# fgcallari/skeres

Hardware: AMD Instinct MI355X
Metric: LM iterations/sec (higher is better)
Workload: dtype f64

## Files before the change

### skeres_amd/csrc/bal_kernels.hip

```cpp
#include <hip/hip_runtime.h>

#include <algorithm>

#include "functors.hpp"
#include "bal_kernels.hpp"

namespace sk {

static constexpr int kBlock = 256;

__device__ __forceinline__ double wave_sum(double v) {
#pragma unroll
  for (int off = 32; off > 0; off >>= 1) v += __shfl_xor(v, off, 64);
  return v;
}

__device__ __forceinline__ int bal_part(const BalDev& d, int i) { return i >= d.cam_b ? 2 : ((i >= d.seg_lo && i < d.cam_a) ? 0 : 1); }
__device__ __forceinline__ int bal_pos(const BalDev& d, int i, int part) { return 9 * (i - (part == 0 ? d.seg_lo : (part == 1 ? d.cam_a : d.cam_b))); }
__device__ __forceinline__ double* bal_block(const BalDev& d, int i, int j, int* ld) {
  const int pj = bal_part(d, j), pi = bal_part(d, i);
  const BalDev::Front& f = d.front[pj];
  const int row = pi == pj ? bal_pos(d, i, pi) : f.border_row[i - d.cam_b];
  *ld = f.ld;
  return f.S + (size_t)row * f.ld + bal_pos(d, j, pj);
// ... 218 lines not shown
    acc[1] += m0 * (d.r[o] + m0 / 2.0) + m1 * (d.r[(size_t)d.N + o] + m1 / 2.0);
  }
  block_sum<2>(acc, d.partial, d.partial_stride);
}

template <bool kLoss>
__global__ __launch_bounds__(kBlock) void bal_host_jac_kernel(BalDev d, int partial_off) {
  double acc[1] = {0.0};
  for (int h = blockIdx.x * kBlock + threadIdx.x; h < d.num_host; h += gridDim.x * kBlock) {
    const int o = d.host_obs[h];
    const int ci = d.cam[o], pi = d.pt[o];
    const double* row = d.host_rows + (size_t)h * kHostRow;
    const double r0 = row[0], r1 = row[1];
    double j0[12], j1[12];
#pragma unroll
    for (int k = 0; k < 9; ++k) { j0[k] = row[2 + k]; j1[k] = row[11 + k]; }
#pragma unroll
    for (int k = 0; k < 3; ++k) { j0[9 + k] = row[20 + k]; j1[9 + k] = row[23 + k]; }
    if (kLoss) {
      const double sq = r0 * r0 + r1 * r1;
      double rho[3];
      bal_loss_eval(d, o, sq, rho);
      const LossCorrector lc(sq, rho);
      acc[0] += rho[0];
#pragma unroll
      for (int k = 0; k < 12; ++k) {
        const double a = j0[k], b = j1[k];
        const double rtj = lc.alpha_sq_norm * (r0 * a + r1 * b);
        j0[k] = lc.sqrt_rho1 * (a - r0 * rtj);
        j1[k] = lc.sqrt_rho1 * (b - r1 * rtj);
      }
      d.r[o] = r0 * lc.residual_scaling;
      d.r[(size_t)d.N + o] = r1 * lc.residual_scaling;
    } else {
      d.r[o] = r0;
      d.r[(size_t)d.N + o] = r1;
      acc[0] += r0 * r0 + r1 * r1;
    }
#pragma unroll
    for (int k = 0; k < 9; ++k) {
      const double s = d.scale_c[9 * (size_t)ci + k];
      d.F[(size_t)k * d.N + o] = j0[k] * s;
      d.F[(size_t)(9 + k) * d.N + o] = j1[k] * s;
    }
#pragma unroll
    for (int k = 0; k < 3; ++k) {
      const double s = d.scale_p[3 * (size_t)pi + k];
      d.E[(size_t)k * d.N + o] = j0[9 + k] * s;
      d.E[(size_t)(3 + k) * d.N + o] = j1[9 + k] * s;
    }
  }
  block_sum<1>(acc, d.partial + partial_off, d.partial_stride);
}

template <bool kLoss>
__global__ __launch_bounds__(kBlock) void bal_host_cost_kernel(BalDev d, int partial_off) {
  double acc[2] = {0.0, 0.0};
  for (int h = blockIdx.x * kBlock + threadIdx.x; h < d.num_host; h += gridDim.x * kBlock) {
    const int o = d.host_obs[h];
    const int ci = d.cam[o], pi = d.pt[o];
    const double n0 = d.host_rows[(size_t)h * kHostRow], n1 = d.host_rows[(size_t)h * kHostRow + 1];
    if (kLoss) {
      double rho[3];
      bal_loss_eval(d, o, n0 * n0 + n1 * n1, rho);
      acc[0] += rho[0];
    } else {
      acc[0] += n0 * n0 + n1 * n1;
    }
    double m0 = -d.u[3 * (size_t)d.N + o], m1 = -d.u[4 * (size_t)d.N + o];
#pragma unroll
    for (int k = 0; k < 3; ++k) {
      const double s = d.step_p[3 * (size_t)pi + k];
      m0 += d.E[(size_t)k * d.N + o] * s;
      m1 += d.E[(size_t)(3 + k) * d.N + o] * s;
    }
    acc[1] += m0 * (d.r[o] + m0 / 2.0) + m1 * (d.r[(size_t)d.N + o] + m1 / 2.0);
  }
  block_sum<2>(acc, d.partial + partial_off, d.partial_stride);
}

__global__ __launch_bounds__(kBlock) void bal_scale_jac_kernel(BalDev d) {
  for (int o = blockIdx.x * kBlock + threadIdx.x; o < d.N; o += gridDim.x * kBlock) {
    const int ci = d.cam[o], pi = d.pt[o];
#pragma unroll
    for (int k = 0; k < 9; ++k) {
      const double s = d.scale_c[9 * (size_t)ci + k];
      d.F[(size_t)k * d.N + o] *= s;
      d.F[(size_t)(9 + k) * d.N + o] *= s;
    }
#pragma unroll
    for (int k = 0; k < 3; ++k) {
      const double s = d.scale_p[3 * (size_t)pi + k];
      d.E[(size_t)k * d.N + o] *= s;
      d.E[(size_t)(3 + k) * d.N + o] *= s;
    }
  }
}

__global__ __launch_bounds__(kBlock) void bal_cam_records_kernel(BalDev d) {
  __shared__ __attribute__((aligned(16))) double stage[kBlock / 64][64 * kFcam];
  const int lane = threadIdx.x & 63, w = threadIdx.x >> 6;
  double* st = stage[w];
  const size_t N = d.N;
  for (long o0 = ((long)blockIdx.x * (kBlock / 64) + w) * 64; o0 < d.N; o0 += (long)gridDim.x * kBlock) {
    const long o = o0 + lane;
    const int my_slot = o < d.N ? d.obs_slot[o] : 0;
    if (o < d.N) {
#pragma unroll
      for (int k = 0; k < 18; ++k) st[lane * kFcam + k] = d.F[(size_t)k * N + o];
      st[lane * kFcam + 18] = d.r[o];
      st[lane * kFcam + 19] = d.r[N + o];
    }
    __builtin_amdgcn_wave_barrier();
    __builtin_amdgcn_s_waitcnt(0xC07F);
    __builtin_amdgcn_wave_barrier();
    const int nrec = (int)((d.N - o0) < 64 ? (d.N - o0) : 64);
#pragma unroll
    for (int i = 0; i < kFcam / 2; ++i) {
      const int e2 = i * 64 + lane, rr = e2 / (kFcam / 2), f2 = e2 - rr * (kFcam / 2);
      const int slot = __shfl(my_slot, rr, 64);
      if (rr < nrec) reinterpret_cast<double2*>(d.Fcam + (size_t)slot * kFcam)[f2] = reinterpret_cast<const double2*>(st)[e2];
    }
    __builtin_amdgcn_wave_barrier();
  }
}

__device__ __forceinline__ void bal_cam_reduce_body(const BalDev& d, int block) {
  const int wave = (block * kBlock + threadIdx.x) >> 6, lane = threadIdx.x & 63;
  if (wave >= d.C) return;
  double sq[9], g[9];
#pragma unroll
  for (int k = 0; k < 9; ++k) { sq[k] = 0.0; g[k] = 0.0; }
  for (int e = d.cam_start[wave] + lane; e < d.cam_start[wave + 1]; e += 64) {
    const double2* rec = reinterpret_cast<const double2*>(d.Fcam + (size_t)e * kFcam);
    double v[kFcam];
#pragma unroll
    for (int k = 0; k < kFcam / 2; ++k) { const double2 t = rec[k]; v[2 * k] = t.x; v[2 * k + 1] = t.y; }
    const double r0 = v[18], r1 = v[19];
#pragma unroll
    for (int k = 0; k < 9; ++k) {
      const double f0 = v[k], f1 = v[9 + k];
      sq[k] += f0 * f0 + f1 * f1;
      g[k] += f0 * r0 + f1 * r1;
    }
  }
#pragma unroll
  for (int k = 0; k < 9; ++k) { sq[k] = wave_sum(sq[k]); g[k] = wave_sum(g[k]); }
  if (lane == 0) {
#pragma unroll
    for (int k = 0; k < 9; ++k) { d.colsq_c[9 * (size_t)wave + k] = sq[k]; d.gs_c[9 * (size_t)wave + k] = g[k]; }
  }
}

__device__ __forceinline__ void bal_pt_reduce_body(const BalDev& d, int block) {
  const int gid = block * kBlock + threadIdx.x, sub = gid % kPointLanes;
  const int p = gid / kPointLanes;
  if (p >= d.P) return;
  double sq[3] = {0, 0, 0}, g[3] = {0, 0, 0};
  for (int o = d.pt_start[p] + sub; o < d.pt_start[p + 1]; o += kPointLanes) {
    const double r0 = d.r[o], r1 = d.r[(size_t)d.N + o];
#pragma unroll
    for (int k = 0; k < 3; ++k) {
      const double e0 = d.E[(size_t)k * d.N + o], e1 = d.E[(size_t)(3 + k) * d.N + o];
      sq[k] += e0 * e0 + e1 * e1;
      g[k] += e0 * r0 + e1 * r1;
    }
  }
#pragma unroll
  for (int k = 0; k < 3; ++k) { sq[k] = point_lanes_sum(sq[k]); g[k] = point_lanes_sum(g[k]); }
  if (sub == 0) {
#pragma unroll
    for (int k = 0; k < 3; ++k) { d.colsq_p[3 * (size_t)p + k] = sq[k]; d.gs_p[3 * (size_t)p + k] = g[k]; }
  }
}

__global__ __launch_bounds__(kBlock) void bal_reduce_kernel(BalDev d, int cam_blocks) {
  if ((int)blockIdx.x < cam_blocks) bal_cam_reduce_body(d, (int)blockIdx.x);
  else bal_pt_reduce_body(d, (int)blockIdx.x - cam_blocks);
}

__global__ void jacobi_scale_kernel(const double* colsq, double* scale, int n) {
  const int j = blockIdx.x * blockDim.x + threadIdx.x;
  if (j < n) scale[j] = scale[j] == 0.0 ? 0.0 : 1.0 / (1.0 + sqrt(colsq[j]));
}
__global__ void apply_scale_to_reductions_kernel(double* colsq, double* gs, const double* scale, int n) {
  const int j = blockIdx.x * blockDim.x + threadIdx.x;
  if (j < n) { const double s = scale[j]; colsq[j] = colsq[j] * s * s; gs[j] = gs[j] * s; }
}
__global__ void lm_diagonal_kernel(const double* colsq, double* D, int n, double lo, double hi, double radius) {
  const int j = blockIdx.x * blockDim.x + threadIdx.x;
  if (j < n) D[j] = sqrt(fmin(fmax(colsq[j], lo), hi) / radius);
}
__global__ __launch_bounds__(kBlock) void grad_max_xnorm_kernel(const double* gs, const double* scale, const double* x,
                                                                int n, double* partial, int stride) {
  double m = 0.0, s = 0.0;
  for (int j = blockIdx.x * kBlock + threadIdx.x; j < n; j += gridDim.x * kBlock) {
    if (scale[j] != 0.0) m = fmax(m, fabs(gs[j] / scale[j]));
    s += x[j] * x[j];
  }
  __shared__ double shm[kBlock / 64], shs[kBlock / 64];
#pragma unroll
  for (int off = 32; off > 0; off >>= 1) { m = fmax(m, __shfl_xor(m, off, 64)); s += __shfl_xor(s, off, 64); }
  if ((threadIdx.x & 63) == 0) { shm[threadIdx.x >> 6] = m; shs[threadIdx.x >> 6] = s; }
  __syncthreads();
  if (threadIdx.x == 0) {
    for (int i = 1; i < kBlock / 64; ++i) { m = fmax(m, shm[i]); s += shs[i]; }
    partial[blockIdx.x] = m;
    partial[stride + blockIdx.x] = s;
  }
}

__global__ __launch_bounds__(kBlock) void final_reduce_kernel(const double* partial, int stride, int count, int K, int maxmask, double* out) {
  __shared__ double sh[kBlock];
  const int k = blockIdx.x;
  const bool is_max = ((maxmask >> k) & 1) != 0;
  double a = 0.0;
  for (int i = threadIdx.x; i < count; i += kBlock) {
    const double v = partial[(size_t)k * stride + i];
    a = is_max ? fmax(a, v) : a + v;
  }
  sh[threadIdx.x] = a;
  __syncthreads();
  for (int w = kBlock / 2; w > 0; w >>= 1) {
    if ((int)threadIdx.x < w) sh[threadIdx.x] = is_max ? fmax(sh[threadIdx.x], sh[threadIdx.x + w]) : sh[threadIdx.x] + sh[threadIdx.x + w];
    __syncthreads();
  }
  if (threadIdx.x == 0) out[k] = sh[0];
}

__global__ __launch_bounds__(kBlock) void bal_point_block_kernel(BalDev d) {
  const int gid = blockIdx.x * kBlock + threadIdx.x, sub = gid % kPointLanes;
  const int p = gid / kPointLanes;
  if (p >= d.P) return;
  double t00 = 0, t10 = 0, t11 = 0, t20 = 0, t21 = 0, t22 = 0;
  for (int o = d.pt_start[p] + sub; o < d.pt_start[p + 1]; o += kPointLanes) {
    const double a0 = d.E[o], a1 = d.E[(size_t)d.N + o], a2 = d.E[2 * (size_t)d.N + o];
    const double b0 = d.E[3 * (size_t)d.N + o], b1 = d.E[4 * (size_t)d.N + o], b2 = d.E[5 * (size_t)d.N + o];
    t00 += a0 * a0 + b0 * b0; t10 += a1 * a0 + b1 * b0; t11 += a1 * a1 + b1 * b1;
    t20 += a2 * a0 + b2 * b0; t21 += a2 * a1 + b2 * b1; t22 += a2 * a2 + b2 * b2;
  }
  t00 = point_lanes_sum(t00); t10 = point_lanes_sum(t10); t11 = point_lanes_sum(t11);
  t20 = point_lanes_sum(t20); t21 = point_lanes_sum(t21); t22 = point_lanes_sum(t22);
  if (sub != 0) return;
  const double d0 = bal_lm_diag(d, d.colsq_p[3 * (size_t)p]), d1 = bal_lm_diag(d, d.colsq_p[3 * (size_t)p + 1]), d2 = bal_lm_diag(d, d.colsq_p[3 * (size_t)p + 2]);
  t00 += d0 * d0; t11 += d1 * d1; t22 += d2 * d2;
  const double l00 = sqrt(t00);
  const double l10 = t10 / l00, l20 = t20 / l00;
  const double l11 = sqrt(t11 - l10 * l10);
  const double l21 = (t21 - l20 * l10) / l11;
  const double l22 = sqrt(t22 - l20 * l20 - l21 * l21);
  const double m00 = 1.0 / l00, m11 = 1.0 / l11, m22 = 1.0 / l22;
  const double m10 = -(l10 * m00) / l11;
  const double m21 = -(l21 * m11) / l22;
  const double m20 = -(l20 * m00 + l21 * m10) / l22;
  const size_t P = d.P;
  d.M[p] = m00; d.M[P + p] = m10; d.M[2 * P + p] = m11; d.M[3 * P + p] = m20; d.M[4 * P + p] = m21; d.M[5 * P + p] = m22;
  const double g0 = d.gs_p[3 * (size_t)p], g1 = d.gs_p[3 * (size_t)p + 1], g2 = d.gs_p[3 * (size_t)p + 2];
  const double u0 = m00 * g0, u1 = m10 * g0 + m11 * g1, u2 = m20 * g0 + m21 * g1 + m22 * g2;
  d.q[p] = m00 * u0 + m10 * u1 + m20 * u2;
  d.q[P + p] = m11 * u1 + m21 * u2;
  d.q[2 * P + p] = m22 * u2;
  if (!(l00 > 0.0) || !(l11 > 0.0) || !(l22 > 0.0)) *d.fail_flag = 1;
}

__global__ __launch_bounds__(kBlock) void bal_kept_points_kernel(BalDev d, int obs_blocks) {
  const size_t N = d.N, P = d.P;
  if ((int)blockIdx.x < obs_blocks) {
    const int e = blockIdx.x * kBlock + threadIdx.x;
    if (e >= d.num_kept_obs) return;
    const int o = d.kept_obs[e], k = d.kept_obs_slot[e];
    const int ic = d.kept_cam[k] / 3, t3 = 3 * (d.kept_cam[k] % 3);
    const int c = d.cam[o];
    const bool below = ic > c;
    if (!d.front[bal_part(d, below ? c : ic)].S) return;
    double ea[3], eb[3];
#pragma unroll
    for (int a = 0; a < 3; ++a) { ea[a] = d.E[(size_t)a * N + o]; eb[a] = d.E[(size_t)(3 + a) * N + o]; }
    int ld;
    double* blk = below ? bal_block(d, ic, c, &ld) : bal_block(d, c, ic, &ld);
#pragma unroll
    for (int b = 0; b < 9; ++b) {
      const double f0 = d.F[(size_t)b * N + o], f1 = d.F[(size_t)(9 + b) * N + o];
#pragma unroll
      for (int a = 0; a < 3; ++a) {
        const double v = ea[a] * f0 + eb[a] * f1;
        if (below) blk[(size_t)(t3 + a) * ld + b] = v; else blk[(size_t)b * ld + t3 + a] = v;
      }
    }
    return;
  }
  const int k = (((int)blockIdx.x - obs_blocks) * kBlock + threadIdx.x) >> 6, lane = threadIdx.x & 63;
  if (k >= d.num_kept) return;
  const int p = d.kept_pt[k], ic = d.kept_cam[k] / 3, t3 = 3 * (d.kept_cam[k] % 3);
  double t00 = 0, t10 = 0, t11 = 0, t20 = 0, t21 = 0, t22 = 0;
  for (int o = d.pt_start[p] + lane; o < d.pt_start[p + 1]; o += 64) {
    const double a0 = d.E[o], a1 = d.E[N + o], a2 = d.E[2 * N + o];
    const double b0 = d.E[3 * N + o], b1 = d.E[4 * N + o], b2 = d.E[5 * N + o];
    t00 += a0 * a0 + b0 * b0; t10 += a1 * a0 + b1 * b0; t11 += a1 * a1 + b1 * b1;
    t20 += a2 * a0 + b2 * b0; t21 += a2 * a1 + b2 * b1; t22 += a2 * a2 + b2 * b2;
  }
  t00 = wave_sum(t00); t10 = wave_sum(t10); t11 = wave_sum(t11); t20 = wave_sum(t20); t21 = wave_sum(t21); t22 = wave_sum(t22);
  if (lane != 0) return;
  d.M[p] = 0.0; d.M[P + p] = 0.0; d.M[2 * P + p] = 0.0; d.M[3 * P + p] = 0.0; d.M[4 * P + p] = 0.0; d.M[5 * P + p] = 0.0;
  d.q[p] = 0.0; d.q[P + p] = 0.0; d.q[2 * P + p] = 0.0;
  if (!d.front[bal_part(d, ic)].S) return;
  const bool home = !d.kept_home || d.kept_home[k] != 0;
  const double d0 = home ? bal_lm_diag(d, d.colsq_p[3 * (size_t)p]) : 0.0, d1 = home ? bal_lm_diag(d, d.colsq_p[3 * (size_t)p + 1]) : 0.0,
               d2 = home ? bal_lm_diag(d, d.colsq_p[3 * (size_t)p + 2]) : 0.0;
  int ld;
  double* blk = bal_block(d, ic, ic, &ld) + (size_t)t3 * ld + t3;
  blk[0] = t00 + d0 * d0;
  blk[ld] = t10; blk[ld + 1] = t11 + d1 * d1;
  blk[2 * (size_t)ld] = t20; blk[2 * (size_t)ld + 1] = t21; blk[2 * (size_t)ld + 2] = t22 + d2 * d2;
  double* rhs = bal_rhs(d, ic) + t3;
  rhs[0] = home ? d.gs_p[3 * (size_t)p] : 0.0; rhs[1] = home ? d.gs_p[3 * (size_t)p + 1] : 0.0; rhs[2] = home ? d.gs_p[3 * (size_t)p + 2] : 0.0;
}

__global__ __launch_bounds__(kBlock) void bal_kept_sums_kernel(BalDev d, double* buf, int K, int gather) {
  const int t = blockIdx.x * kBlock + threadIdx.x;
  if (t >= 3 * d.num_kept) return;
  const int k = t / 3, a = t - 3 * k;
  const size_t p = (size_t)d.kept_pt[k], g = (size_t)(d.kept_global ? d.kept_global[k] : k);
  if (gather) { buf[3 * g + a] = d.colsq_p[3 * p + a]; buf[3 * (size_t)K + 3 * g + a] = d.gs_p[3 * p + a]; }
  else { d.colsq_p[3 * p + a] = buf[3 * g + a]; d.gs_p[3 * p + a] = buf[3 * (size_t)K + 3 * g + a]; }
}

__global__ __launch_bounds__(kBlock, 4) void bal_obs_precompute_kernel(BalDev d) {
  constexpr int kLs = kWs + 2;
  __shared__ __attribute__((aligned(16))) double stage[kBlock / 64][32 * kLs];
  const size_t N = d.N, P = d.P;
  const int lane = threadIdx.x & 63, wave = threadIdx.x >> 6;
  double* mine = &stage[wave][0];
  for (long base = (long)(blockIdx.x * kBlock + wave * 64); base < (long)d.N; base += (long)gridDim.x * kBlock) {
    const long o = base + lane;
    const int my_slot = o < (long)d.N ? d.obs_slot[o] : 0;
    double w[27], rt[2];
    if (o < (long)d.N) {
      const int p = d.pt[o];
      const double m00 = d.M[p], m10 = d.M[P + p], m11 = d.M[2 * P + p], m20 = d.M[3 * P + p], m21 = d.M[4 * P + p], m22 = d.M[5 * P + p];
      const double q0 = d.q[p], q1 = d.q[P + p], q2 = d.q[2 * P + p];
      double eh[2][3];
#pragma unroll
      for (int r = 0; r < 2; ++r) {
        const double e0 = d.E[(3 * r) * N + o], e1 = d.E[(3 * r + 1) * N + o], e2 = d.E[(3 * r + 2) * N + o];
        eh[r][0] = e0 * m00;
        eh[r][1] = e0 * m10 + e1 * m11;
        eh[r][2] = e0 * m20 + e1 * m21 + e2 * m22;
        rt[r] = d.r[r * N + o] - (e0 * q0 + e1 * q1 + e2 * q2);
      }
#pragma unroll
      for (int c = 0; c < 9; ++c) {
        const double f0 = d.F[c * N + o], f1 = d.F[(9 + c) * N + o];
#pragma unroll
        for (int a = 0; a < 3; ++a) w[3 * c + a] = f0 * eh[0][a] + f1 * eh[1][a];
      }
    }
    const int nrec = (int)(((long)d.N - base) < 64 ? ((long)d.N - base) : 64);
    const int sub = lane >> 4, chunk = lane & 15;
#pragma unroll
    for (int half = 0; half < 2; ++half) {
      if ((lane >> 5) == half && o < (long)d.N) {
        double* rec = mine + (lane & 31) * kLs;
#pragma unroll
        for (int k = 0; k < 27; ++k) rec[k] = w[k];
        rec[27] = rt[0]; rec[28] = rt[1];
        rec[29] = 0.0; rec[30] = 0.0; rec[31] = 0.0;
      }
      __builtin_amdgcn_wave_barrier();
#pragma unroll 4
      for (int it = 0; it < 8; ++it) {
        const int rl = 4 * it + sub, rec = 32 * half + rl;
        const int slot = __shfl(my_slot, rec, 64);
        if (rec < nrec) {
          const double2 v = *reinterpret_cast<const double2*>(&mine[rl * kLs + 2 * chunk]);
          *reinterpret_cast<double2*>(d.What + (size_t)slot * kWs + 2 * chunk) = v;
        }
      }
      __builtin_amdgcn_wave_barrier();
    }
  }
}

__global__ __launch_bounds__(kBlock) void bal_cam_diag_kernel(BalDev d) {
  const int i = (blockIdx.x * kBlock + threadIdx.x) >> 6, lane = threadIdx.x & 63;
  if (i >= d.C) return;
  if (d.pseudo && d.pseudo[i]) return;
  double acc[45], rh[9];
#pragma unroll
  for (int k = 0; k < 45; ++k) acc[k] = 0.0;
#pragma unroll
  for (int k = 0; k < 9; ++k) rh[k] = 0.0;
  for (int e = d.cam_start[i] + lane; e < d.cam_start[i + 1]; e += 64) {
    double f0[9], f1[9], w[28];
    {
      const double2* rec = reinterpret_cast<const double2*>(d.Fcam + (size_t)e * kFcam);
#pragma unroll
      for (int k = 0; k < 9; ++k) {
        const double2 t = rec[k];
        if (2 * k < 9) f0[2 * k] = t.x; else f1[2 * k - 9] = t.x;
        if (2 * k + 1 < 9) f0[2 * k + 1] = t.y; else f1[2 * k + 1 - 9] = t.y;
      }
    }
    const double2* wrec = reinterpret_cast<const double2*>(d.What + (size_t)e * kWs);
#pragma unroll
    for (int k = 0; k < 14; ++k) { const double2 t = wrec[k]; w[2 * k] = t.x; w[2 * k + 1] = t.y; }
    const double r0 = w[27], r1 = wrec[14].x;
    int k = 0;
#pragma unroll
    for (int c = 0; c < 9; ++c) {
      rh[c] += f0[c] * r0 + f1[c] * r1;
#pragma unroll
      for (int e2 = 0; e2 <= c; ++e2, ++k)
        acc[k] += (f0[c] * f0[e2] + f1[c] * f1[e2]) - (w[3 * c] * w[3 * e2] + w[3 * c + 1] * w[3 * e2 + 1] + w[3 * c + 2] * w[3 * e2 + 2]);
    }
  }
#pragma unroll
  for (int k = 0; k < 45; ++k) acc[k] = wave_sum(acc[k]);
#pragma unroll
  for (int k = 0; k < 9; ++k) rh[k] = wave_sum(rh[k]);
  if (lane == 0 && d.front[bal_part(d, i)].S) {
    int k = 0, ld;
    double* blk = bal_block(d, i, i, &ld);
    double* rhs = bal_rhs(d, i);
#pragma unroll
    for (int c = 0; c < 9; ++c) {
      rhs[c] = rh[c];
#pragma unroll
      for (int e2 = 0; e2 <= c; ++e2, ++k) blk[(size_t)c * ld + e2] = acc[k];
    }
  }
}

__global__ __launch_bounds__(64) void bal_dup_diag_kernel(BalDev d) {
  const int first = blockIdx.x;
  const int i = d.dup_cam[first];
  if (first > 0 && d.dup_cam[first - 1] == i) return;
  if (!d.front[bal_part(d, i)].S) return;
  const int t = threadIdx.x;
  if (t >= 45) return;
  int c = 0, rem = t;
  while (rem > c) { rem -= c + 1; ++c; }
  const int e2 = rem;
  double acc = 0.0;
  for (int k = first; k < d.num_dup && d.dup_cam[k] == i; ++k) {
    const double* wa = d.What + (size_t)d.dup_a[k] * kWs;
    const double* wb = d.What + (size_t)d.dup_b[k] * kWs;
    acc += (wa[3 * c] * wb[3 * e2] + wa[3 * c + 1] * wb[3 * e2 + 1] + wa[3 * c + 2] * wb[3 * e2 + 2]) +
           (wb[3 * c] * wa[3 * e2] + wb[3 * c + 1] * wa[3 * e2 + 1] + wb[3 * c + 2] * wa[3 * e2 + 2]);
  }
  int ld;
  double* blk = bal_block(d, i, i, &ld);
  blk[(size_t)c * ld + e2] -= acc;
}

constexpr int kPairSlot = 34;
__device__ __forceinline__ void pair_accumulate(const BalDev& d, int e_begin, int e_end, int stride, int c, double* slot, double (&acc)[9]) {
  if (e_begin >= e_end) return;
  const int last = e_begin + (e_end - 1 - e_begin) / stride * stride;
  const double* wr = d.What + (size_t)d.pair_row_obs[e_begin] * kWs + 3 * c;
  const double* wc = d.What + (size_t)d.pair_col_obs[e_begin] * kWs + 3 * c;
  double y0 = wr[0], y1 = wr[1], y2 = wr[2], v0 = wc[0], v1 = wc[1], v2 = wc[2];
  int e1 = e_begin + stride <= last ? e_begin + stride : last;
  int ob1 = d.pair_row_obs[e1], oa1 = d.pair_col_obs[e1];
  for (int e = e_begin; e < e_end; e += stride) {
    slot[3 * c] = v0; slot[3 * c + 1] = v1; slot[3 * c + 2] = v2;
    __builtin_amdgcn_wave_barrier();
    double w[kWu];
#pragma unroll
    for (int k = 0; k < kWu / 2; ++k) { const double2 t = reinterpret_cast<const double2*>(slot)[k]; w[2 * k] = t.x; w[2 * k + 1] = t.y; }
    __builtin_amdgcn_wave_barrier();
    const double* wrn = d.What + (size_t)ob1 * kWs + 3 * c;
    const double* wcn = d.What + (size_t)oa1 * kWs + 3 * c;
    const double yn0 = wrn[0], yn1 = wrn[1], yn2 = wrn[2], vn0 = wcn[0], vn1 = wcn[1], vn2 = wcn[2];
    const int e2 = e + 2 * stride <= last ? e + 2 * stride : last;
    const int ob2 = d.pair_row_obs[e2], oa2 = d.pair_col_obs[e2];
#pragma unroll
    for (int k = 0; k < 9; ++k) acc[k] += y0 * w[3 * k] + y1 * w[3 * k + 1] + y2 * w[3 * k + 2];
    y0 = yn0; y1 = yn1; y2 = yn2; v0 = vn0; v1 = vn1; v2 = vn2;
    ob1 = ob2; oa1 = oa2;
  }
}

__device__ __forceinline__ int xcd_grouped_block(int w, int group) {
  if (group <= 0) return w;
  const int x = w & 7, q = w >> 3;
  return ((q / group) * 8 + x) * group + q % group;
}

__global__ __launch_bounds__(kBlock) void bal_pair_kernel(BalDev d, int xcd_group) {
  const int lane = threadIdx.x & 63;
  const int wave = (xcd_grouped_block((int)blockIdx.x, xcd_group) * kBlock + threadIdx.x) >> 6;
  __shared__ __attribute__((aligned(16))) double share[kBlock / 64][7][kPairSlot];
  const int sub = lane / 9, c = lane - 9 * sub;
  const int slot = wave * 7 + sub;
  if (sub >= 7 || slot >= d.num_short_segments) return;
  const int seg = d.short_segments[slot];
  double acc[9];
#pragma unroll
  for (int k = 0; k < 9; ++k) acc[k] = 0.0;
  pair_accumulate(d, d.seg_start[seg], d.seg_start[seg + 1], 1, c, share[threadIdx.x >> 6][sub], acc);
  const int i = d.seg_row[seg], j = d.seg_col[seg];
  int ld;
  double* out = bal_block(d, i, j, &ld) + (size_t)c * ld;
#pragma unroll
  for (int k = 0; k < 9; ++k) out[k] = -acc[k];
}

__global__ __launch_bounds__(kBlock) void bal_pair_long_kernel(BalDev d, int xcd_group) {
  __shared__ double red[kBlock / 64][7][81];
  __shared__ __attribute__((aligned(16))) double share[kBlock / 64][7][kPairSlot];
  const int lane = threadIdx.x & 63, w = threadIdx.x >> 6;
  const int slot = (xcd_grouped_block((int)blockIdx.x, xcd_group) * kBlock + threadIdx.x) >> 6;
  if (slot >= d.num_long_segments) return;
  const int seg = d.long_segments[slot];
  const int sub = lane / 9, c = lane - 9 * sub;
  double acc[9];
#pragma unroll
  for (int k = 0; k < 9; ++k) acc[k] = 0.0;
  if (sub < 7) {
    pair_accumulate(d, d.seg_start[seg] + sub, d.seg_start[seg + 1], 7, c, share[w][sub], acc);
#pragma unroll
    for (int k = 0; k < 9; ++k) red[w][sub][9 * c + k] = acc[k];
  }
  __builtin_amdgcn_wave_barrier();
  __builtin_amdgcn_s_waitcnt(0xC07F);
  __builtin_amdgcn_wave_barrier();
  const int i = d.seg_row[seg], j = d.seg_col[seg];
  int ld;
  double* blk = bal_block(d, i, j, &ld);
  for (int e = lane; e < 81; e += 64) {
    double s = 0.0;
#pragma unroll
    for (int g = 0; g < 7; ++g) s += red[w][g][e];
    blk[(size_t)(e / 9) * ld + e % 9] = -s;
  }
}

__global__ void finish_normal_matrix_kernel(double* S, int ld, int n, int npad, int rhs_row, const double* D) {
  const int j = blockIdx.x * blockDim.x + threadIdx.x;
  if (j >= npad) return;
  if (j < n) S[(size_t)j * ld + j] += D[j] * D[j];
  else if (j == rhs_row) S[(size_t)j * ld + j] = 1e300;
  else S[(size_t)j * ld + j] = 1.0;
}
__global__ void bal_finish_S_kernel(BalDev d, int parts) {
  const int j = blockIdx.x * blockDim.x + threadIdx.x;
  if (j >= 9 * d.C) return;
  const int i = j / 9, c = j - 9 * i, part = bal_part(d, i);
  if (!((parts >> part) & 1) || !d.front[part].S) return;
  if (d.pseudo && d.pseudo[i]) return;
  int ld;
  double* blk = bal_block(d, i, i, &ld);
  const double D = bal_lm_diag(d, d.colsq_c[j]);
  blk[(size_t)c * ld + c] += D * D;
}
__global__ void set_diagonal_kernel(double* S, int ld, int from, int to, double value) {
  const int j = from + blockIdx.x * blockDim.x + threadIdx.x;
  if (j < to) S[(size_t)j * ld + j] = value;
}

__global__ __launch_bounds__(kBlock) void bal_obs_backsub_kernel(BalDev d) {
  const size_t N = d.N;
  for (int o = blockIdx.x * kBlock + threadIdx.x; o < d.N; o += gridDim.x * kBlock) {
    const double* yc = d.y_c + 9 * (size_t)d.cam[o];
    double f0 = 0.0, f1 = 0.0;
#pragma unroll
    for (int c = 0; c < 9; ++c) { f0 += d.F[c * N + o] * yc[c]; f1 += d.F[(9 + c) * N + o] * yc[c]; }
    d.u[o] = d.E[o] * f0 + d.E[3 * N + o] * f1;
    d.u[N + o] = d.E[N + o] * f0 + d.E[4 * N + o] * f1;
    d.u[2 * N + o] = d.E[2 * N + o] * f0 + d.E[5 * N + o] * f1;
    d.u[3 * N + o] = f0;
    d.u[4 * N + o] = f1;
  }
}

__global__ __launch_bounds__(kBlock) void bal_point_backsub_kernel(BalDev d) {
  const int gid = blockIdx.x * kBlock + threadIdx.x, sub = gid % kPointLanes;
  const int p = gid / kPointLanes;
  double acc[1] = {0.0};
  double w0 = 0.0, w1 = 0.0, w2 = 0.0;
  if (p < d.P) {
    for (int o = d.pt_start[p] + sub; o < d.pt_start[p + 1]; o += kPointLanes) {
      w0 += d.u[o];
      w1 += d.u[(size_t)d.N + o];
      w2 += d.u[2 * (size_t)d.N + o];
    }
  }
  w0 = point_lanes_sum(w0); w1 = point_lanes_sum(w1); w2 = point_lanes_sum(w2);
  if (p < d.P && sub == 0) {
    const size_t P = d.P;
    const double t0 = d.gs_p[3 * (size_t)p] - w0, t1 = d.gs_p[3 * (size_t)p + 1] - w1, t2 = d.gs_p[3 * (size_t)p + 2] - w2;
    const double m00 = d.M[p], m10 = d.M[P + p], m11 = d.M[2 * P + p], m20 = d.M[3 * P + p], m21 = d.M[4 * P + p], m22 = d.M[5 * P + p];
    const double u0 = m00 * t0, u1 = m10 * t0 + m11 * t1, u2 = m20 * t0 + m21 * t1 + m22 * t2;
    const double y[3] = {m00 * u0 + m10 * u1 + m20 * u2, m11 * u1 + m21 * u2, m22 * u2};
#pragma unroll
    for (int k = 0; k < 3; ++k) {
      const double st = -y[k];
      const double dl = st * d.scale_p[3 * (size_t)p + k];
      d.step_p[3 * (size_t)p + k] = st;
      const double xo = d.xp[3 * (size_t)p + k];
      const double xn = xo + dl;
      d.xp_new[3 * (size_t)p + k] = xn;
      const double df = xo - xn;
      acc[0] += df * df;
    }
  }
  block_sum<1>(acc, d.partial + d.partial_stride, d.partial_stride);
}

__global__ __launch_bounds__(kBlock) void bal_kept_step_kernel(BalDev d, int slot) {
  double acc[1] = {0.0};
  for (int k = threadIdx.x; k < d.num_kept; k += kBlock) {
    const int p = d.kept_pt[k], ic = d.kept_cam[k] / 3, t3 = 3 * (d.kept_cam[k] % 3);
    const bool home = !d.kept_home || d.kept_home[k] != 0;
#pragma unroll
    for (int a = 0; a < 3; ++a) {
      const double st = -d.y_c[9 * (size_t)ic + t3 + a];
      d.step_p[3 * (size_t)p + a] = st;
      const double xo = d.xp[3 * (size_t)p + a];
      const double xn = xo + st * d.scale_p[3 * (size_t)p + a];
      d.xp_new[3 * (size_t)p + a] = xn;
      const double df = xo - xn;
      if (home) acc[0] += df * df;
    }
  }
  block_sum<1>(acc, d.partial + d.partial_stride + slot, d.partial_stride);
}

__global__ __launch_bounds__(kBlock) void bal_cam_step_kernel(BalDev d, int norm_lo, int norm_hi, int norm_lo2, int norm_hi2) {
  double acc[1] = {0.0};
  const int n = 9 * d.C;
  const int j = blockIdx.x * kBlock + threadIdx.x;
  if (j < n) {
    const int i = j / 9, c = j - 9 * i, part = bal_part(d, i);
    const double y = d.front[part].S ? d.y_front[part][bal_pos(d, i, part) + c] : 0.0;
    d.y_c[j] = y;
    const double st = -y;
    d.step_c[j] = st;
    const double xo = d.xc[j];
    const double xn = xo + st * d.scale_c[j];
    d.xc_new[j] = xn;
    const double df = xo - xn;
    if ((j >= norm_lo && j < norm_hi) || (j >= norm_lo2 && j < norm_hi2)) acc[0] += df * df;
  }
  block_sum<1>(acc, d.partial, d.partial_stride);
}
__global__ __launch_bounds__(1024) void final_reduce_rows_kernel(const double* partial, int stride, ReduceRows rows) {
  __shared__ double sh[1024];
  const int k = blockIdx.x, count = rows.count[k];
  const bool is_max = rows.is_max[k] != 0;
  const double* src = partial + (size_t)rows.row[k] * stride;
  double a = 0.0;
  for (int i = threadIdx.x; i < count; i += 1024) a = is_max ? fmax(a, src[i]) : a + src[i];
  sh[threadIdx.x] = a;
  __syncthreads();
  for (int w = 512; w > 0; w >>= 1) {
    if ((int)threadIdx.x < w) sh[threadIdx.x] = is_max ? fmax(sh[threadIdx.x], sh[threadIdx.x + w]) : sh[threadIdx.x] + sh[threadIdx.x + w];
    __syncthreads();
  }
  if (threadIdx.x == 0) *rows.out[k] = sh[0];
}
void launch_final_reduce_rows(const double* partial, int stride, const ReduceRows& rows, hipStream_t s) {
  if (rows.n > 0) hipLaunchKernelGGL(final_reduce_rows_kernel, dim3(rows.n), dim3(1024), 0, s, partial, stride, rows);
}

__global__ __launch_bounds__(256) void tri_pack_kernel(double* S, int ld, double* packed, const int* __restrict__ col0, const long long* __restrict__ off,
                                                       int to_packed) {
  const int kb = blockIdx.y;
  const size_t c0 = (size_t)col0[kb] * 128, width = (size_t)(kb + 1) * 128 - c0;
  double* pk = packed + off[kb];
  const size_t n2 = 128 * width / 2;
  for (size_t i = (size_t)blockIdx.x * 256 + threadIdx.x; i < n2; i += (size_t)gridDim.x * 256) {
    const size_t e = 2 * i, r = e / width, c = e % width;
    double2* a = reinterpret_cast<double2*>(S + ((size_t)kb * 128 + r) * ld + c0 + c);
    double2* b = reinterpret_cast<double2*>(pk + e);
    if (to_packed) *b = *a; else *a = *b;
  }
}

static inline int grid_for(int n, int cap = 2048) {
  int g = (n + kBlock - 1) / kBlock;
  return g < 1 ? 1 : (g > cap ? cap : g);
}

__global__ __launch_bounds__(256) void zero_envelope_kernel(double* S, int ld, const int* col0) {
  const int kb = blockIdx.y;
  const size_t c0 = (size_t)col0[kb] * 128, width = (size_t)(kb + 1) * 128 - c0;
  const size_t n2 = 128 * width / 2;
  for (size_t i = (size_t)blockIdx.x * 256 + threadIdx.x; i < n2; i += (size_t)gridDim.x * 256) {
    const size_t e = 2 * i, r = e / width, c = e % width;
    *reinterpret_cast<double2*>(S + ((size_t)kb * 128 + r) * ld + c0 + c) = make_double2(0.0, 0.0);
  }
}
void launch_zero_envelope(double* S, int ld, const int* col0, int nblk, hipStream_t s) {
  if (nblk > 0) hipLaunchKernelGGL(zero_envelope_kernel, dim3(32, nblk), dim3(256), 0, s, S, ld, col0);
}

int bal_partial_blocks(int N) { return grid_for(N); }
size_t tri_packed_elems(int nblk) { return (size_t)128 * 128 * ((size_t)nblk * (nblk + 1) / 2); }
void launch_tri_pack(double* S, int ld, double* packed, int nblk, const int* col0, const long long* off, bool to_packed, hipStream_t s) {
  if (nblk > 0) hipLaunchKernelGGL(tri_pack_kernel, dim3(64, nblk), dim3(256), 0, s, S, ld, packed, col0, off, to_packed ? 1 : 0);
}

void launch_bal_eval_jac(const BalDev& d, hipStream_t s) {
  if (d.loss_root >= 0) hipLaunchKernelGGL(bal_eval_jac_kernel<true>, dim3(grid_for(d.N)), dim3(kBlock), 0, s, d);
  else hipLaunchKernelGGL(bal_eval_jac_kernel<false>, dim3(grid_for(d.N)), dim3(kBlock), 0, s, d);
}
void launch_bal_eval_cost(const BalDev& d, hipStream_t s) {
  if (d.loss_root >= 0) hipLaunchKernelGGL(bal_eval_cost_kernel<true>, dim3(grid_for(d.N)), dim3(kBlock), 0, s, d);
  else hipLaunchKernelGGL(bal_eval_cost_kernel<false>, dim3(grid_for(d.N)), dim3(kBlock), 0, s, d);
}
int bal_tape_width(const Tape& t) { return t.num_obs_consts > kTapeMaxObs ? 0 : tape_pick_width(t, kBlock); }
template <class K> static void bal_tape_allow_lds(K kernel, size_t bytes) {
  if (bytes > 48 * 1024) (void)hipFuncSetAttribute(reinterpret_cast<const void*>(kernel), hipFuncAttributeMaxDynamicSharedMemorySize, (int)bytes);
}
void launch_bal_eval_jac_tape(const BalDev& d, const TapeDevBuffers& tb, hipStream_t s) {
  const int W = bal_tape_width(tb.host), nobs = tb.host.num_obs_consts;
  const size_t lds = tape_lds_bytes(tb.host, W, kBlock);
  const dim3 g(grid_for(d.N)), b(kBlock);
#define SK_TAPE_JAC(LOSS, WW) { bal_tape_allow_lds(bal_eval_jac_tape_kernel<LOSS, WW>, lds); hipLaunchKernelGGL((bal_eval_jac_tape_kernel<LOSS, WW>), g, b, lds, s, d, tb.view, nobs); }
  if (d.loss_root >= 0) { if (W == 3) SK_TAPE_JAC(true, 3) else if (W == 2) SK_TAPE_JAC(true, 2) else SK_TAPE_JAC(true, 1) }
  else { if (W == 3) SK_TAPE_JAC(false, 3) else if (W == 2) SK_TAPE_JAC(false, 2) else SK_TAPE_JAC(false, 1) }
#undef SK_TAPE_JAC
}
void launch_bal_eval_cost_tape(const BalDev& d, const TapeDevBuffers& tb, hipStream_t s) {
  const size_t lds = tape_lds_bytes(tb.host, 0, kBlock);
  const int nobs = tb.host.num_obs_consts;
  if (d.loss_root >= 0) { bal_tape_allow_lds(bal_eval_cost_tape_kernel<true>, lds); hipLaunchKernelGGL(bal_eval_cost_tape_kernel<true>, dim3(grid_for(d.N)), dim3(kBlock), lds, s, d, tb.view, nobs); }
  else { bal_tape_allow_lds(bal_eval_cost_tape_kernel<false>, lds); hipLaunchKernelGGL(bal_eval_cost_tape_kernel<false>, dim3(grid_for(d.N)), dim3(kBlock), lds, s, d, tb.view, nobs); }
}
int launch_bal_host_jac(const BalDev& d, int partial_off, hipStream_t s) {
  if (d.num_host <= 0) return 0;
  const int g = grid_for(d.num_host);
  if (d.loss_root >= 0) hipLaunchKernelGGL(bal_host_jac_kernel<true>, dim3(g), dim3(kBlock), 0, s, d, partial_off);
  else hipLaunchKernelGGL(bal_host_jac_kernel<false>, dim3(g), dim3(kBlock), 0, s, d, partial_off);
  return g;
}
int launch_bal_host_cost(const BalDev& d, int partial_off, hipStream_t s) {
  if (d.num_host <= 0) return 0;
  const int g = grid_for(d.num_host);
  if (d.loss_root >= 0) hipLaunchKernelGGL(bal_host_cost_kernel<true>, dim3(g), dim3(kBlock), 0, s, d, partial_off);
  else hipLaunchKernelGGL(bal_host_cost_kernel<false>, dim3(g), dim3(kBlock), 0, s, d, partial_off);
  return g;
}
void launch_bal_scale_jac(const BalDev& d, hipStream_t s) { hipLaunchKernelGGL(bal_scale_jac_kernel, dim3(grid_for(d.N)), dim3(kBlock), 0, s, d); }
void launch_bal_cam_records(const BalDev& d, hipStream_t s) { hipLaunchKernelGGL(bal_cam_records_kernel, dim3(grid_for((d.N + 63) / 64 * 64)), dim3(kBlock), 0, s, d); }
void launch_bal_reduce(const BalDev& d, hipStream_t s) {
  const int cam_blocks = (d.C * 64 + kBlock - 1) / kBlock, pt_blocks = d.P > 0 ? (int)(((long)d.P * kPointLanes + kBlock - 1) / kBlock) : 0;
  hipLaunchKernelGGL(bal_reduce_kernel, dim3(cam_blocks + pt_blocks), dim3(kBlock), 0, s, d, cam_blocks);
}
static int point_grid(int P) { return (int)(((long)P * kPointLanes + kBlock - 1) / kBlock); }
int bal_point_blocks(int P) { return P > 0 ? point_grid(P) : 1; }
void launch_jacobi_scale(const double* colsq, double* scale, int n, hipStream_t s) { if (n > 0) hipLaunchKernelGGL(jacobi_scale_kernel, dim3((n + 255) / 256), dim3(256), 0, s, colsq, scale, n); }
void launch_apply_scale_to_reductions(double* colsq, double* gs, const double* scale, int n, hipStream_t s) { if (n > 0) hipLaunchKernelGGL(apply_scale_to_reductions_kernel, dim3((n + 255) / 256), dim3(256), 0, s, colsq, gs, scale, n); }
void launch_lm_diagonal(const double* colsq, double* D, int n, double lo, double hi, double radius, hipStream_t s) { if (n > 0) hipLaunchKernelGGL(lm_diagonal_kernel, dim3((n + 255) / 256), dim3(256), 0, s, colsq, D, n, lo, hi, radius); }
int launch_grad_max_xnorm(const double* gs, const double* scale, const double* x, int n, double* partial, int stride, hipStream_t s) {
  const int g = grid_for(n, 256);
  hipLaunchKernelGGL(grad_max_xnorm_kernel, dim3(g), dim3(kBlock), 0, s, gs, scale, x, n, partial, stride);
  return g;
}
__global__ void bal_pack_rank_scalars_kernel(const double* __restrict__ scal, double* __restrict__ table, int rank, int world, int mode, int segmented) {
  const int K = mode == 0 ? 3 : 4;
  for (int i = threadIdx.x; i < world * K; i += blockDim.x) table[i] = 0.0;
  __syncthreads();
  if (threadIdx.x != 0) return;
  double* t = table + (size_t)rank * K;
  if (mode == 0) {
    t[0] = scal[4];
    t[1] = segmented ? fmax(scal[2], scal[0]) : scal[2];
    t[2] = scal[3] + (segmented ? scal[1] : 0.0);
  } else {
    const int fail = *reinterpret_cast<const int*>(scal + 14), info = *reinterpret_cast<const int*>(scal + 15);
    t[0] = scal[0]; t[1] = scal[1];
    t[2] = scal[9] + (segmented ? scal[8] : 0.0);
    t[3] = (double)(fail | info);
  }
}
void launch_bal_pack_rank_scalars(const double* scal, double* table, int rank, int world, int mode, bool segmented, hipStream_t s) {
  hipLaunchKernelGGL(bal_pack_rank_scalars_kernel, dim3(1), dim3(64), 0, s, scal, table, rank, world, mode, segmented ? 1 : 0);
}
void launch_final_reduce(const double* partial, int stride, int count, int K, int maxmask, double* out, hipStream_t s) { hipLaunchKernelGGL(final_reduce_kernel, dim3(K), dim3(kBlock), 0, s, partial, stride, count, K, maxmask, out); }
void launch_bal_point_block(const BalDev& d, hipStream_t s) { if (d.P > 0) hipLaunchKernelGGL(bal_point_block_kernel, dim3(point_grid(d.P)), dim3(kBlock), 0, s, d); }
void launch_bal_kept_points(const BalDev& d, hipStream_t s) {
  if (d.num_kept <= 0) return;
  const int obs_blocks = (d.num_kept_obs + kBlock - 1) / kBlock;
  hipLaunchKernelGGL(bal_kept_points_kernel, dim3(obs_blocks + (d.num_kept * 64 + kBlock - 1) / kBlock), dim3(kBlock), 0, s, d, obs_blocks);
}
void launch_bal_obs_precompute(const BalDev& d, hipStream_t s) { hipLaunchKernelGGL(bal_obs_precompute_kernel, dim3(grid_for(d.N)), dim3(kBlock), 0, s, d); }
void launch_bal_kept_sums(const BalDev& d, double* buf, int K, bool gather, hipStream_t s) {
  if (d.num_kept > 0) hipLaunchKernelGGL(bal_kept_sums_kernel, dim3((3 * d.num_kept + kBlock - 1) / kBlock), dim3(kBlock), 0, s, d, buf, K, gather ? 1 : 0);
}
void launch_bal_cam_diag(const BalDev& d, hipStream_t s) {
  hipLaunchKernelGGL(bal_cam_diag_kernel, dim3((d.C * 64 + kBlock - 1) / kBlock), dim3(kBlock), 0, s, d);
  if (d.num_dup > 0) hipLaunchKernelGGL(bal_dup_diag_kernel, dim3(d.num_dup), dim3(64), 0, s, d);
}
void launch_bal_pair(const BalDev& d, hipStream_t s) {
  const int group_long = dev_knobs().schedule_plain ? 0 : 8, group_short = group_long;
  auto grid = [](int blocks, int group) { return group > 0 ? (blocks + 8 * group - 1) / (8 * group) * (8 * group) : blocks; };
  if (d.num_long_segments > 0)
    hipLaunchKernelGGL(bal_pair_long_kernel, dim3(grid((d.num_long_segments * 64 + kBlock - 1) / kBlock, group_long)), dim3(kBlock), 0, s, d, group_long);
  if (d.num_short_segments > 0) {
    const int waves = (d.num_short_segments + 6) / 7;
    hipLaunchKernelGGL(bal_pair_kernel, dim3(grid((waves * 64 + kBlock - 1) / kBlock, group_short)), dim3(kBlock), 0, s, d, group_short);
  }
}
void launch_finish_normal_matrix(double* S, int ld, int n, int npad, int rhs_row, const double* D, hipStream_t s) { hipLaunchKernelGGL(finish_normal_matrix_kernel, dim3((npad + 255) / 256), dim3(256), 0, s, S, ld, n, npad, rhs_row, D); }
__global__ void bal_finish_all_kernel(BalDev d, BalFinishRanges r, int jmax) {
  const int j = blockIdx.x * blockDim.x + threadIdx.x;
  if (j >= jmax) return;
  if (j < 9 * d.C) {
    const int i = j / 9, c = j - 9 * i, part = bal_part(d, i);
    if (d.front[part].S && !(d.pseudo && d.pseudo[i])) {
      int ld;
      double* blk = bal_block(d, i, i, &ld);
      const double D = bal_lm_diag(d, d.colsq_c[j]);
      blk[(size_t)c * ld + c] += D * D;
    }
  }
#pragma unroll
  for (int k = 0; k < 4; ++k)
    if (r.S[k] && j >= r.from[k] && j < r.to[k]) r.S[k][(size_t)j * r.ld[k] + j] = r.value[k];
}
void launch_bal_finish_all(const BalDev& d, const BalFinishRanges& r, hipStream_t s) {
  int jmax = 9 * d.C;
  for (int k = 0; k < 4; ++k) if (r.S[k] && r.to[k] > jmax) jmax = r.to[k];
  hipLaunchKernelGGL(bal_finish_all_kernel, dim3((jmax + 255) / 256), dim3(256), 0, s, d, r, jmax);
}
void launch_bal_finish_S(const BalDev& d, int parts, hipStream_t s) { hipLaunchKernelGGL(bal_finish_S_kernel, dim3((9 * d.C + 255) / 256), dim3(256), 0, s, d, parts); }
void launch_set_diagonal(double* S, int ld, int from, int to, double value, hipStream_t s) {
  if (to > from) hipLaunchKernelGGL(set_diagonal_kernel, dim3((to - from + 255) / 256), dim3(256), 0, s, S, ld, from, to, value);
}
void launch_bal_backsub(const BalDev& d, double* out, int norm_lo, int norm_hi, int norm_lo2, int norm_hi2, hipStream_t s) {
  const int gc = (9 * d.C + kBlock - 1) / kBlock, gp = bal_point_blocks(d.P);
  hipLaunchKernelGGL(bal_cam_step_kernel, dim3(gc), dim3(kBlock), 0, s, d, norm_lo, norm_hi, norm_lo2, norm_hi2);
  hipLaunchKernelGGL(bal_obs_backsub_kernel, dim3(grid_for(d.N)), dim3(kBlock), 0, s, d);
  hipLaunchKernelGGL(bal_point_backsub_kernel, dim3(gp), dim3(kBlock), 0, s, d);
  if (d.num_kept > 0) hipLaunchKernelGGL(bal_kept_step_kernel, dim3(1), dim3(kBlock), 0, s, d, gp);
  ReduceRows rows;
  rows.n = 2;
  rows.row[0] = 0; rows.count[0] = gc; rows.out[0] = out;
  rows.row[1] = 1; rows.count[1] = d.P > 0 ? gp + (d.num_kept > 0 ? 1 : 0) : 0; rows.out[1] = out + 1;
  launch_final_reduce_rows(d.partial, d.partial_stride, rows, s);
}

__global__ __launch_bounds__(kBlock) void dogleg_vector_norms_kernel(BalDev d, DoglegDev q) {
  double acc[3] = {0.0, 0.0, 0.0};
  const int nc = 9 * d.C, n = nc + 3 * d.P;
  for (int j = blockIdx.x * kBlock + threadIdx.x; j < n; j += gridDim.x * kBlock) {
    double sj = 0.0, gj = 0.0;
    if (!(j < nc && d.pseudo && d.pseudo[j / 9])) {
      const double diag = sqrt(fmin(fmax(d.colsq_c[j], d.lm_lo), d.lm_hi));
      const double gh = d.gs_c[j] / diag;
      gj = d.step_c[j];
      const double p = diag * gj;
      sj = -gh / diag;
      acc[0] += gh * gh; acc[1] += gh * p; acc[2] += p * p;
    }
    q.s[j] = sj; q.g[j] = gj;
  }
  block_sum<3>(acc, q.partial + 5 * (size_t)q.stride, q.stride);
}

__global__ __launch_bounds__(kBlock) void bal_dogleg_products_kernel(BalDev d, DoglegDev q) {
  double acc[5] = {0.0, 0.0, 0.0, 0.0, 0.0};
  const size_t N = d.N;
  const double* sp = q.s + 9 * (size_t)d.C;
  const double* gp = q.g + 9 * (size_t)d.C;
  for (int o = blockIdx.x * kBlock + threadIdx.x; o < d.N; o += gridDim.x * kBlock) {
    const size_t ci = 9 * (size_t)d.cam[o], pi = 3 * (size_t)d.pt[o];
    double w0 = 0.0, w1 = 0.0, m0 = 0.0, m1 = 0.0;
#pragma unroll
    for (int k = 0; k < 9; ++k) {
      const double f0 = d.F[k * N + o], f1 = d.F[(9 + k) * N + o], sk_ = q.s[ci + k], gk = q.g[ci + k];
      w0 += f0 * sk_; w1 += f1 * sk_; m0 += f0 * gk; m1 += f1 * gk;
    }
#pragma unroll
    for (int k = 0; k < 3; ++k) {
      const double e0 = d.E[k * N + o], e1 = d.E[(3 + k) * N + o], sk_ = sp[pi + k], gk = gp[pi + k];
      w0 += e0 * sk_; w1 += e1 * sk_; m0 += e0 * gk; m1 += e1 * gk;
    }
    const double r0 = d.r[o], r1 = d.r[N + o];
    acc[0] += w0 * r0 + w1 * r1; acc[1] += m0 * r0 + m1 * r1;
    acc[2] += w0 * w0 + w1 * w1; acc[3] += w0 * m0 + w1 * m1; acc[4] += m0 * m0 + m1 * m1;
  }
  block_sum<5>(acc, q.partial, q.stride);
}

__global__ __launch_bounds__(kBlock) void bal_dogleg_combine_kernel(BalDev d, DoglegDev q, double a, double b) {
  double acc[1] = {0.0};
  const int n = 9 * d.C + 3 * d.P;
  for (int j = blockIdx.x * kBlock + threadIdx.x; j < n; j += gridDim.x * kBlock) {
    const double st = a * q.s[j] + b * q.g[j];
    d.step_c[j] = st;
    const double xo = d.xc[j];
    const double xn = xo + st * d.scale_c[j];
    d.xc_new[j] = xn;
    const double df = xo - xn;
    acc[0] += df * df;
  }
  block_sum<1>(acc, q.partial + 8 * (size_t)q.stride, q.stride);
}

int dogleg_partial_stride(const BalDev& d) { return std::max(grid_for(d.N), grid_for(9 * d.C + 3 * d.P)); }
void launch_dogleg_vector_norms(const BalDev& d, const DoglegDev& q, hipStream_t s) {
  hipLaunchKernelGGL(dogleg_vector_norms_kernel, dim3(grid_for(9 * d.C + 3 * d.P)), dim3(kBlock), 0, s, d, q);
}
void launch_bal_dogleg_products(const BalDev& d, const DoglegDev& q, hipStream_t s) {
  hipLaunchKernelGGL(bal_dogleg_products_kernel, dim3(grid_for(d.N)), dim3(kBlock), 0, s, d, q);
}
void launch_dogleg_reduce_scalars(const DoglegDev& q, hipStream_t s) { launch_final_reduce(q.partial, q.stride, q.stride, 8, 0, q.scal, s); }
void launch_bal_dogleg_combine(const BalDev& d, const DoglegDev& q, double a, double b, hipStream_t s) {
  const int g = grid_for(9 * d.C + 3 * d.P);
  hipLaunchKernelGGL(bal_dogleg_combine_kernel, dim3(g), dim3(kBlock), 0, s, d, q, a, b);
  launch_final_reduce(q.partial + 8 * (size_t)q.stride, q.stride, g, 1, 0, q.scal + 8, s);
}

__global__ void box_project_kernel(double* x, const double* __restrict__ lo, const double* __restrict__ hi, int n) {
  const int j = blockIdx.x * blockDim.x + threadIdx.x;
  if (j < n) x[j] = fmin(fmax(x[j], lo[j]), hi[j]);
}

__global__ __launch_bounds__(kBlock) void bounded_grad_max_xnorm_kernel(const double* __restrict__ gs, const double* __restrict__ scale, const double* __restrict__ x,
                                                                        int n, BoundsDev q) {
  double m = 0.0;
  double acc[2] = {0.0, 0.0};
  for (int j = blockIdx.x * kBlock + threadIdx.x; j < n; j += gridDim.x * kBlock) {
    const double xj = x[j], lo = q.lo[j], hi = q.hi[j];
    if (scale[j] != 0.0) m = fmax(m, fabs(xj - fmin(fmax(xj - gs[j] / scale[j], lo), hi)));
    acc[0] += xj * xj;
    acc[1] += (xj == lo || xj == hi) ? 1.0 : 0.0;
  }
  __shared__ double shm[kBlock / 64];
#pragma unroll
  for (int off = 32; off > 0; off >>= 1) m = fmax(m, __shfl_xor(m, off, 64));
  if ((threadIdx.x & 63) == 0) shm[threadIdx.x >> 6] = m;
  __syncthreads();
  if (threadIdx.x == 0) {
    for (int i = 1; i < kBlock / 64; ++i) m = fmax(m, shm[i]);
    q.partial[3 * (size_t)q.stride + blockIdx.x] = m;
  }
  block_sum<2>(acc, q.partial + 4 * (size_t)q.stride, q.stride);
}

__global__ __launch_bounds__(kBlock) void bal_directional_derivative_kernel(BalDev d, BoundsDev q) {
  double m = 0.0;
  double acc[1] = {0.0};
  const int nc = 9 * d.C, n = nc + 3 * d.P;
  for (int j = blockIdx.x * kBlock + threadIdx.x; j < n; j += gridDim.x * kBlock) {
    if (j < nc && d.pseudo && d.pseudo[j / 9]) continue;
    const double st = d.step_c[j];
    acc[0] += d.gs_c[j] * st;
    m = fmax(m, fabs(st * d.scale_c[j]));
  }
  __shared__ double shm[kBlock / 64];
#pragma unroll
  for (int off = 32; off > 0; off >>= 1) m = fmax(m, __shfl_xor(m, off, 64));
  if ((threadIdx.x & 63) == 0) shm[threadIdx.x >> 6] = m;
  __syncthreads();
  if (threadIdx.x == 0) {
    for (int i = 1; i < kBlock / 64; ++i) m = fmax(m, shm[i]);
    q.partial[2 * (size_t)q.stride + blockIdx.x] = m;
  }
  block_sum<1>(acc, q.partial + q.stride, q.stride);
}

__global__ __launch_bounds__(kBlock) void bal_bounded_candidate_kernel(BalDev d, BoundsDev q, double alpha) {
  double acc[1] = {0.0};
  const int nc = 9 * d.C, n = nc + 3 * d.P;
  for (int j = blockIdx.x * kBlock + threadIdx.x; j < n; j += gridDim.x * kBlock) {
    const double xo = d.xc[j];
    double xn = xo;
    if (!(j < nc && d.pseudo && d.pseudo[j / 9])) xn = fmin(fmax(xo + (alpha * d.step_c[j]) * d.scale_c[j], q.lo[j]), q.hi[j]);
    d.xc_new[j] = xn;
    const double df = xo - xn;
    acc[0] += df * df;
  }
  block_sum<1>(acc, q.partial, q.stride);
}

int bounds_partial_stride(int n) { return grid_for(n); }
void launch_box_project(double* x, const double* lo, const double* hi, int n, hipStream_t s) {
  if (n > 0) hipLaunchKernelGGL(box_project_kernel, dim3((n + 255) / 256), dim3(256), 0, s, x, lo, hi, n);
}
void launch_bounded_grad_max_xnorm(const double* gs, const double* scale, const double* x, int n, const BoundsDev& q, hipStream_t s) {
  const int g = grid_for(n);
  hipLaunchKernelGGL(bounded_grad_max_xnorm_kernel, dim3(g), dim3(kBlock), 0, s, gs, scale, x, n, q);
  launch_final_reduce(q.partial + 3 * (size_t)q.stride, q.stride, g, 3, 1, q.scal + 3, s);
}
void launch_bal_directional_derivative(const BalDev& d, const BoundsDev& q, hipStream_t s) {
  const int g = grid_for(9 * d.C + 3 * d.P);
// ... 11 lines not shown
```

### skeres_amd/csrc/bal_kernels.hpp

```cpp
#pragma once
#include <hip/hip_runtime.h>

#include "common.hpp"
#include "loss.hpp"

namespace sk {

constexpr int kLongSegment = 32;
constexpr int kWs = 32;
constexpr int kWu = 28;
struct BalDev {
  int C, P, N;
  int res_size, cam_size, pt_size;
  const int* cam;
  const int* pt;
  const double* obs;
  const int* pt_start;
  const int* cam_start;
  const int* cam_obs;
  int num_segments;
  const int* seg_start;
  const int* seg_row;
  const int* seg_col;
  int num_short_segments, num_long_segments;
  const int* short_segments;
  const int* long_segments;
  const int* pair_row_obs;
  const int* pair_col_obs;
  int num_kept;
  const int* kept_pt;  const int* kept_cam;
  int num_kept_obs;  const int* kept_obs;  const int* kept_obs_slot;
  const unsigned char* pseudo;
  const int* kept_home;  const int* kept_global;
  int num_dup;  const int* dup_a;  const int* dup_b;  const int* dup_cam;
  double* xc;  double* xp;
  double* xc_new;  double* xp_new;
  double* scale_c;  double* scale_p;
  double* colsq_c;  double* colsq_p;
  double* gs_c;  double* gs_p;
  double lm_lo, lm_hi, lm_radius;  const double* lm_radius_dev;
  double* step_c;  double* step_p;
  double* y_c;
  double* r;  double* F;  double* E;  double* What;  double* u;
  double* Fcam;  const int* obs_slot;
  double* M;  double* q;
  struct Front { double* S; int ld; int interior; int rhs_row; const int* border_row; };
  Front front[3];
  int seg_lo, cam_a, cam_b;
  const double* y_front[3];
  double* S;  int ld;  int rhs_row;
  double* partial;  int partial_stride;
  int* fail_flag;
  const LossNode* loss_nodes;  int loss_root;  const int* loss_of_obs;
  const unsigned char* is_host;
  int num_host;
  const int* host_obs;
  const double* host_rows;
};
constexpr int kHostRow = 26;
constexpr int kFcam = 20;

int bal_partial_blocks(int N);
int bal_point_blocks(int P);
void launch_zero_envelope(double* S, int ld, const int* col0, int nblk, hipStream_t s);
size_t tri_packed_elems(int nblk);
void launch_tri_pack(double* S, int ld, double* packed, int nblk, const int* col0, const long long* off, bool to_packed, hipStream_t s);
void launch_bal_eval_jac(const BalDev& d, hipStream_t s);
void launch_bal_eval_cost(const BalDev& d, hipStream_t s);
void launch_bal_eval_jac_tape(const BalDev& d, const TapeDevBuffers& tb, hipStream_t s);
void launch_bal_eval_cost_tape(const BalDev& d, const TapeDevBuffers& tb, hipStream_t s);
int launch_bal_host_jac(const BalDev& d, int partial_off, hipStream_t s);
int launch_bal_host_cost(const BalDev& d, int partial_off, hipStream_t s);
void launch_bal_scale_jac(const BalDev& d, hipStream_t s);
void launch_bal_cam_records(const BalDev& d, hipStream_t s);
void launch_bal_reduce(const BalDev& d, hipStream_t s);
void launch_jacobi_scale(const double* colsq, double* scale, int n, hipStream_t s);
void launch_apply_scale_to_reductions(double* colsq, double* gs, const double* scale, int n, hipStream_t s);
void launch_lm_diagonal(const double* colsq, double* D, int n, double lo, double hi, double radius, hipStream_t s);
int launch_grad_max_xnorm(const double* gs, const double* scale, const double* x, int n, double* partial, int stride, hipStream_t s);
void launch_final_reduce(const double* partial, int stride, int count, int K, int maxmask, double* out, hipStream_t s);
void launch_bal_pack_rank_scalars(const double* scal, double* table, int rank, int world, int mode, bool segmented, hipStream_t s);
struct ReduceRows { int n = 0; int row[4] = {0, 0, 0, 0}, count[4] = {0, 0, 0, 0}, is_max[4] = {0, 0, 0, 0}; double* out[4] = {nullptr, nullptr, nullptr, nullptr}; };
void launch_final_reduce_rows(const double* partial, int stride, const ReduceRows& rows, hipStream_t s);
void launch_bal_point_block(const BalDev& d, hipStream_t s);
void launch_bal_kept_points(const BalDev& d, hipStream_t s);
void launch_bal_kept_sums(const BalDev& d, double* buf, int K, bool gather, hipStream_t s);
void launch_bal_obs_precompute(const BalDev& d, hipStream_t s);
void launch_bal_cam_diag(const BalDev& d, hipStream_t s);
void launch_bal_pair(const BalDev& d, hipStream_t s);
void launch_finish_normal_matrix(double* S, int ld, int n, int npad, int rhs_row, const double* D, hipStream_t s);
void launch_bal_finish_S(const BalDev& d, int parts, hipStream_t s);
struct BalFinishRanges { double* S[4] = {nullptr, nullptr, nullptr, nullptr}; int ld[4] = {0, 0, 0, 0}, from[4] = {0, 0, 0, 0}, to[4] = {0, 0, 0, 0}; double value[4] = {0, 0, 0, 0}; };
void launch_bal_finish_all(const BalDev& d, const BalFinishRanges& r, hipStream_t s);
void launch_set_diagonal(double* S, int ld, int from, int to, double value, hipStream_t s);
void launch_bal_backsub(const BalDev& d, double* out, int norm_lo, int norm_hi, int norm_lo2, int norm_hi2, hipStream_t s);

struct DoglegDev { double* s; double* g; double* partial; int stride; double* scal; };
int dogleg_partial_stride(const BalDev& d);
void launch_dogleg_vector_norms(const BalDev& d, const DoglegDev& q, hipStream_t s);
void launch_bal_dogleg_products(const BalDev& d, const DoglegDev& q, hipStream_t s);
void launch_dogleg_reduce_scalars(const DoglegDev& q, hipStream_t s);
void launch_bal_dogleg_combine(const BalDev& d, const DoglegDev& q, double a, double b, hipStream_t s);

struct BoundsDev { const double* lo; const double* hi; double* partial; int stride; double* scal; };
int bounds_partial_stride(int n);
void launch_box_project(double* x, const double* lo, const double* hi, int n, hipStream_t s);
void launch_bounded_grad_max_xnorm(const double* gs, const double* scale, const double* x, int n, const BoundsDev& q, hipStream_t s);
void launch_bal_directional_derivative(const BalDev& d, const BoundsDev& q, hipStream_t s);
void launch_bal_bounded_candidate(const BalDev& d, const BoundsDev& q, double alpha, hipStream_t s);

}
```

### skeres_amd/csrc/bal_solver.hip

```cpp
#include <algorithm>
#include <cmath>
#include <limits>

#include "bal_kernels.hpp"
#include "bal_plan.hpp"
#include "solver.hpp"

namespace sk {

namespace {

struct CaptureGuard {
  hipStream_t s; bool active; bool* graph_mode;
  CaptureGuard(hipStream_t st, bool on, bool* gm) : s(st), active(on), graph_mode(gm) {}
  void release() { active = false; }
  ~CaptureGuard() {
    if (!active) return;
    hipGraph_t g = nullptr;
    (void)hipStreamEndCapture(s, &g);
    if (g) (void)hipGraphDestroy(g);
    (void)hipGetLastError();
    *graph_mode = false;
  }
};
// ... 19 lines not shown
    SolverBase::set_kernel_timing(on);
    kt_b_.only(on == 2 ? "gemm_syrk" : ""); kt_b_.enable(on != 0);
  }
  KernelTimer::Stat kernel_stat(const std::string& name) override {
    KernelTimer::Stat a = kt_.get_stat(name), b = kt_b_.get_stat(name);
    a.seconds += b.seconds; a.launches += b.launches;
    return a;
  }
  bool stat(const std::string& name, double* value) const override {
    const int nblk = npad_ / 128;
    if (name == "envelope_fill") {
      double in = 0.0;
      for (int k = 0; k < 3; ++k) in += fr_[k].envelope().blocks();
      *value = in / (0.5 * nblk * (nblk + 1.0));
      return true;
    }
    if (name == "reduced_system_blocks") { *value = nblk; return true; }
    if (name == "camera_order") { *value = camera_order_; return true; }
    if (name == "cholesky_flops_full") { const double n = 9.0 * C_; *value = n * n * n / 3.0; return true; }
    if (name == "cholesky_flops_plan") {
      double f = 0.0;
      for (int k = 0; k < 3; ++k) if (fr_[k].nblk > 0) f += cholesky_plan_flops(fr_[k].nblk, fr_[k].env(), fr_[k].ncols, fr_[k].tail_rows, fr_[k].tl());
      *value = f;
      return true;
    }
    if (name == "cholesky_columns_resident") {
      int r = 0;
      for (int k = 0; k < 3; ++k) {
        if (fr_[k].nblk == 0) continue;
        const CholeskyPlan plan = cholesky_plan(fr_[k].nblk, group_, fr_[k].env(), chain_live() && (k != 1 || tail_chain()), fr_[k].ncols, fr_[k].tail_rows, fr_[k].tl());
        for (char c : plan.resident) r += c ? 1 : 0;
      }
      *value = r;
      return true;
    }
    if (name == "chain_steps") {
      *value = (dissected_ ? std::max(fr_[0].ncols, fr_[1].ncols) : 0) + fr_[2].ncols;
      return true;
    }
    if (name == "allreduce_bytes") { *value = (double)packed_elems_ * sizeof(double); return true; }
    if (name == "allreduce_bytes_full_triangle") { *value = (double)tri_packed_elems(nblk) * sizeof(double); return true; }
    if (name == "dissected") { *value = dissected_ ? 1.0 : 0.0; return true; }
    if (name == "pair_segments_short") { *value = d_.num_short_segments; return true; }
    if (name == "pair_segments_long") { *value = d_.num_long_segments; return true; }
    if (name == "graph_replay") { *value = graph_mode_ ? 1.0 : 0.0; return true; }
    if (name == "host_callback_blocks" || name == "tape_blocks") {
      const bool host = name == "host_callback_blocks";
      size_t c = 0;
      for (size_t b = 0; b < problem_->rb_functor.size(); ++b)
        c += host ? problem_->rb_functor[b] == SK_FUNCTOR_HOST_CALLBACK : problem_->tape_of_block(b) != nullptr;
      *value = (double)c;
      return true;
    }
    if (name == "tape_width") { *value = tape_mode_ ? bal_tape_width(tape_dev_.host) : 0; return true; }
    if (name == "tape_lds_bytes") { *value = tape_mode_ ? (double)tape_lds_bytes(tape_dev_.host, bal_tape_width(tape_dev_.host), 256) : 0.0; return true; }
    if (name == "retained_points") { *value = (double)retained_pts_.size(); return true; }
    if (name == "retained_model_us") { *value = retained_model_us_; return true; }
    if (name == "retained_model_us_without") { *value = retained_without_us_; return true; }
    if (name == "border_cameras") { *value = border_cams_; return true; }
    if (name == "border_gap") { *value = border_gap_; return true; }
    if (name == "border_model_us") { *value = border_model_us_; return true; }
    if (name == "border_model_us_plain") { *value = border_plain_us_; return true; }
    if (name == "segments") { *value = segmented_ ? segments_ : (dissected_ ? 2 : 1); return true; }
    if (name == "segment_cameras") { *value = segmented_ ? my_hi_ - my_lo_ : C_; return true; }
    if (name.rfind("model_us_segments_", 0) == 0) { const int k = atoi(name.c_str() + 18); if (k < 1 || k > 8) return false; *value = cut_model_.model_us[k]; return true; }
    if (name == "dissection_head_cameras") { *value = cam_a_; return true; }
    if (name == "dissection_tail_cameras") { *value = cam_b_ - cam_a_; return true; }
    if (name == "dissection_separator_cameras") { *value = dissected_ ? C_ - cam_b_ : 0; return true; }
    if (name == "dissection_model_us_plain") { *value = cut_model_.t_plain; return true; }
    if (name == "dissection_model_us") { *value = cut_model_.t_model; return true; }
    if (name == "model_us_two_segments_with_members") { *value = cut_model_.two_segments_members_us; return true; }
    return strategy_stat(name, value);
  }
  bool chain_ok() const { return opt_.cholesky_group == 0 && opt_.lookahead && chol_ctx_.server != nullptr; }
  bool chain_live() const { return chain_ok() && cholesky_chain_enabled(&chol_ctx_); }
  bool tail_chain() const { return chol_ctx_b_.server != nullptr; }
  int distribution(double* allreduce_s, double* saved_s) const override {
    if (allreduce_s) *allreduce_s = est_allreduce_s_;
    if (saved_s) *saved_s = est_saved_s_;
    return distribution_;
  }

 protected:
  int setup() override;
  int evaluate_with_jacobian(bool first) override;
  int linear_solve(double radius, LinearSolve* out) override;
  int dogleg_trial(double a, double b, double* cost, double* step_norm) override;
  int bounded_trial(double alpha, double* cost, double* step_norm) override;
  bool supports_dogleg() const override { return true; }
  int solve_once(double radius, LinearSolve* out, bool* chain_lost);
  struct Backsolve { int resident; bool zero_after; };
  int enqueue_schur_assembly(const Backsolve& bs, bool graph);
  int enqueue_factor_backsolve(const Backsolve& bs, bool graph);
  int enqueue_point_backsub(bool graph);
  int enqueue_candidate_cost(int rows, bool* failed);
  int trial_cost(const double* step_sq_dev, int step_sq_slot, double* cost, double* step_norm);
  const char* refuses_bounds() const override {
    for (int f : problem_->rb_functor)
      if (f == SK_FUNCTOR_HOST_CALLBACK) return "parameter bounds with host-evaluated (director) residual blocks under DENSE_SCHUR are not supported";
    return nullptr;
  }
  int upload_bounds();
  BoundsDev bd_{};
  DevBuf<double> b_bd_box_, b_bd_partial_, b_bd_scal_;
  DoglegDev dl_{};
  DevBuf<double> b_dl_vec_, b_dl_partial_, b_dl_scal_;
  void accept_candidate() override { std::swap(d_.xc, d_.xc_new); std::swap(d_.xp, d_.xp_new); parity_ ^= 1; }
  int write_back() override;
  void describe(Summary* s) override {
    s->num_parameter_blocks = (int)problem_->block_size.size();
    s->num_parameters = problem_->num_parameters();
    s->num_residual_blocks = (int)problem_->rb_functor.size();
    s->num_residuals = problem_->num_residuals;
    s->num_e_blocks = P_total_; s->num_f_blocks = C_ - pseudo_cams_;
  }

 private:
  int gather_rank_scalars(double* vals, int K, const int* ops);
  int host_callbacks(const double* x_dev, bool jac, bool* failed);
  std::vector<int> host_obs_;
  std::vector<const CostFunction*> host_cf_;
  std::vector<double> host_x_, host_rows_h_;
  DevBuf<unsigned char> b_is_host_;
  DevBuf<int> b_host_obs_;
  DevBuf<double> b_host_rows_;
  std::vector<int> h_cam_, h_pt_;
  int gather_rank_scalars_signed(double* vals, int K);
  bool rank_table_on_device(int K) const;
  int enqueue_rank_table(int mode, int K);
  int fold_rank_table(const double* table, double* vals, int K, const int* ops);
  int exchange_rank_table(const double* vals, int K, std::vector<double>* table);

  int C_ = 0, P_total_ = 0, P_ = 0, N_ = 0;
  int res_size_ = 2, cam_size_ = 9, pt_size_ = 3;
  int n_ = 0, npad_ = 0, rhs_row_ = 0;
  std::vector<int> cam_block_, pt_block_;
  std::vector<int> local_pt_;
  BalDev d_{};
  DevBuf<LossNode> b_loss_nodes_;
  DevBuf<int> b_loss_of_obs_;
  DevBuf<int> b_cam_, b_pt_, b_pt_start_, b_cam_start_, b_cam_obs_, b_obs_slot_, b_seg_start_, b_seg_row_, b_seg_col_, b_pair_row_, b_pair_col_, b_short_segs_, b_long_segs_;
  int *fail_p_ = nullptr, *info_p_ = nullptr;
  DevBuf<double> b_obs_, b_xc_, b_xp_, b_xc_new_, b_xp_new_, b_scale_, b_colsq_, b_gs_, b_step_, b_y_,
      b_r_, b_F_, b_Fcam_, b_E_, b_W_, b_rt_, b_M_, b_q_, b_S_, b_Linv_, b_partial_, b_scal_, b_small_;
  std::vector<int> env_last_;
  std::vector<int> env_tail_;
  std::vector<int> retained_pts_, retained_cam_;
  int pseudo_cams_ = 0;
  int border_members_ = 0;
  double retained_model_us_ = 0.0, retained_without_us_ = 0.0;
  std::vector<int> struct_ocam_, struct_opt_;
  int struct_P_ = 0;
  DevBuf<int> b_kept_pt_, b_kept_cam_, b_kept_obs_, b_kept_obs_slot_;
  int P_own_ = 0;
  DevBuf<int> b_kept_home_, b_kept_global_;
  DevBuf<int> b_dup_a_, b_dup_b_, b_dup_cam_;
  int num_dup_ = 0;
  int num_kept_obs_ = 0;
  DevBuf<unsigned char> b_pseudo_;
  int border_cams_ = 0, border_gap_ = 0;
  double border_model_us_ = 0.0, border_plain_us_ = 0.0;
  FrontHost fr_[3];
  bool dissected_ = false;
  bool segmented_ = false;
  int segments_ = 0, role_ = 0, my_lo_ = 0, my_hi_ = 0;
  bool replica_ = false;
  int fold_world_ = 0;
  int cam_a_ = 0, cam_b_ = 0, border_blocks_ = 0;
  std::vector<int> seg_off_;
  std::vector<int> sep_first_;
  std::vector<int> root_last_, root_tail_;
  FrontView leaf_;
  DevBuf<int> b_border_row_[2], b_leaf_map_, b_leaf_gmap_;
  CutModel cut_model_;
  DissectedSystem ds_;
  CholeskyContext chol_ctx_b_;
  KernelTimer kt_b_;
  bool tape_mode_ = false;
  TapeDevBuffers tape_dev_;
  bool graph_mode_ = false;
  int parity_ = 0;
  hipGraphExec_t g_step_[2] = {nullptr, nullptr}, g_eval_[2] = {nullptr, nullptr};
  bool graph_ok() const { return graph_mode_ && !kt_.enabled(); }
  int finish_capture(hipStream_t s, hipGraphExec_t* exec);
  DevBuf<int> b_zero_col0_f_[3], b_mapB_;
  bool mapB_involution_ = false;
  DevBuf<double> b_yf_, b_wf_, b_ybB_;
  double order_hash_ = 0.0;
  int camera_order_ = 0;
  int group_ = 3;
  DevBuf<double> b_pack_;
  size_t packed_elems_ = 0;
  std::vector<int> pack_col0_h_;
  std::vector<long long> pack_off_h_;
  DevBuf<int> b_pack_col0_;
  DevBuf<long long> b_pack_off_;
  int distribution_ = SK_DISTRIBUTION_SHARDED;
  double est_allreduce_s_ = 0.0, est_saved_s_ = 0.0;
  int choose_distribution(const std::vector<int>& opt);
  struct Structure {
    std::vector<int> ocam, opt;
    std::vector<int> band_ocam, band_opt;
    std::vector<int> env_for_model;
    int Creal = 0;
  };
  int init_queues();
  int plan_layout(Structure* st);
  void plan_pack();
  int prepare_pack();
  int shard_or_replicate(const std::vector<int>& opt);
  int cut_camera_sequence(Structure* st);
  void adopt_cuts(const CutPlan& cuts, int Cband, bool multi, Structure* st);
  int upload_structure(const LocalStructure& ls);
  int allocate_fronts(const FrontLayout& lay);
  int bind_device_view(const LocalStructure& ls);
  int agree_with_ranks();
  bool distribution_decided_ = false;
  std::chrono::steady_clock::time_point setup_t0_, stage_last_;
  void stage(const char* what) {
    if (!dev_knobs().debug_setup) return;
    const auto now = std::chrono::steady_clock::now();
    std::fprintf(stderr, "[skeres_amd] set-up: %-40s %8.1f ms (at %.1f ms)\n", what, std::chrono::duration<double, std::milli>(now - stage_last_).count(),
                 std::chrono::duration<double, std::milli>(now - setup_t0_).count());
    stage_last_ = now;
  }
  CholeskyContext chol_ctx_;
  enum Slot {
    kGradMaxCam = 0, kXSqCam, kGradMaxPt, kXSqPt, kSumSq,
    kEvalFirst = kGradMaxCam, kEvalLast = kSumSq,
    kCandSumSq = 0, kModel,
    kStepSqCam = 8, kStepSqPt,
    kRadiusDev = 12,
    kFail = 14, kInfo,
    kStepFirst = kCandSumSq, kStepLast = kInfo,
    kDevSlots = kStepLast + 1,
    kRadius = kDevSlots,
    kDogleg,
    kBounds = kDogleg + kDlScalCount,
    kRankTable = kBounds + kBdScalCount,
    kRankTableSlots = 24,
    kHostSlots = kRankTable + kRankTableSlots
  };
  static_assert(kEvalLast < kStepSqCam && kModel < kStepSqCam && kStepSqPt < kRadiusDev && kRadiusDev < kFail, "b_scal_'s slots are distinct");
  static_assert(kStepLast < kRadius && kRadius < kDogleg && kDogleg + kDlScalCount <= kBounds && kBounds + kBdScalCount <= kRankTable, "h_scal_'s regions do not overlap");
  double* h_scal_ = nullptr;
  int host_flag(int slot) const { int v = 0; std::memcpy(&v, h_scal_ + slot, sizeof(int)); return v; }
  double* rank_table_dev() const { return b_small_.p + 2 * 9 * (size_t)C_ + 6 * retained_pts_.size() + 64; }
  int partial_stride_ = 0;
  bool zero_by_backsolve_ = false;
  bool need_full_zero_ = false;
  DevBuf<int> b_zero_min_f_[3];
  bool pair_claimed_ = false;
 public:
  ~BalSolver() override {
    if (pair_claimed_) cholesky_release_pair_servers(&chol_ctx_);
    for (hipGraphExec_t g : {g_step_[0], g_step_[1], g_eval_[0], g_eval_[1]}) if (g) (void)hipGraphExecDestroy(g);
    if (h_scal_) (void)hipHostFree(h_scal_);
  }
};

int BalSolver::choose_distribution(const std::vector<int>& opt) {
  const int W = opt_.world;
  distribution_ = SK_DISTRIBUTION_SHARDED;
  if (W <= 1 || opt_.distribution_mode == SK_DISTRIBUTION_SHARDED) return SK_OK;
  if (opt_.distribution_mode != SK_DISTRIBUTION_REPLICATED) {
    const double per_iter = chain_model::shardable_work_s(chain_model::pair_entries(opt, P_total_), (double)opt.size());
    est_saved_s_ = per_iter * (1.0 - 1.0 / W);
    int rc = allreduce(b_pack_.p, packed_elems_);
    if (rc) return rc;
    SK_HIP_TRY(hipStreamSynchronize(stream_));
    const auto t0 = std::chrono::steady_clock::now();
    for (int rep = 0; rep < 2; ++rep) { rc = allreduce(b_pack_.p, packed_elems_); if (rc) return rc; }
    SK_HIP_TRY(hipStreamSynchronize(stream_));
    double mine = std::chrono::duration<double>(std::chrono::steady_clock::now() - t0).count() / 2.0;
    double vals[1] = {mine};
    const int ops[1] = {0};
    SK_HIP_TRY(b_small_.alloc(2 * 9 * (size_t)C_ + 6 * retained_pts_.size() + 64 + 16 * (size_t)W));
    rc = gather_rank_scalars(vals, 1, ops);
    if (rc) return rc;
    est_allreduce_s_ = vals[0] / W;
    collect_allreduce_time(true);
    phase_[5] = 0.0;
    if (est_allreduce_s_ <= est_saved_s_) return SK_OK;
  }
  distribution_ = SK_DISTRIBUTION_REPLICATED;
  opt_.allreduce = nullptr; opt_.world = 1; opt_.rank = 0;
  b_pack_.release();
  return SK_OK;
}

int BalSolver::setup() {
  setup_t0_ = stage_last_ = std::chrono::steady_clock::now();
  std::string why;
  if (!problem_is_bal_shaped(*problem_, &why)) { set_error("%s", why.c_str()); return SK_ERR_UNSUPPORTED; }
  const Problem& p = *problem_;
  int rc = SK_OK;
  Structure st;
  (void)bal_block_shape(p, &res_size_, &cam_size_, &pt_size_);
  bal_index_problem(p, &cam_block_, &pt_block_, &st.ocam, &st.opt);
  C_ = (int)cam_block_.size(); P_total_ = (int)pt_block_.size();
  st.Creal = C_;
  n_ = 9 * C_; rhs_row_ = n_; npad_ = ((n_ + 1 + 127) / 128) * 128;
  if ((rc = init_queues())) return rc;
  if ((rc = plan_layout(&st))) return rc;
  stage("camera order applied");
  plan_pack();
// ... 125 lines not shown
}

static void pack_rows(int nblk, const std::vector<int>& last, const std::vector<int>& tail, std::vector<int>* col0, std::vector<long long>* off) {
  col0->assign(nblk, 0);
  off->assign(nblk + 1, 0);
  if (!last.empty()) *col0 = cholesky_row_first_cols(nblk, last.data(), tail.empty() ? nullptr : tail.data());
  for (int kb = 0; kb < nblk; ++kb) (*off)[kb + 1] = (*off)[kb] + (long long)128 * 128 * (kb + 1 - (*col0)[kb]);
}
void BalSolver::plan_pack() {
  pack_rows(npad_ / 128, env_last_, env_tail_, &pack_col0_h_, &pack_off_h_);
  packed_elems_ = (size_t)pack_off_h_.back();
}
int BalSolver::prepare_pack() {
  if (opt_.reduce_buffer) {
    if (opt_.reduce_buffer_bytes < packed_elems_ * sizeof(double)) { set_error("reduce buffer too small: need %zu bytes", packed_elems_ * sizeof(double)); return SK_ERR_INVALID_ARGUMENT; }
    b_pack_.adopt(static_cast<double*>(opt_.reduce_buffer), packed_elems_);
  } else {
    SK_HIP_TRY(b_pack_.alloc(packed_elems_));
  }
  SK_HIP_TRY(b_pack_.zero(stream_));
  return SK_OK;
}
int BalSolver::shard_or_replicate(const std::vector<int>& opt) {
  int rc = prepare_pack();
  if (rc) return rc;
  rc = choose_distribution(opt);
  if (rc) return rc;
  distribution_decided_ = true;
  return SK_OK;
}

int BalSolver::cut_camera_sequence(Structure* st) {
  const bool seg_modes = opt_.distribution_mode == SK_DISTRIBUTION_AUTO || opt_.distribution_mode == SK_DISTRIBUTION_SEGMENTED;
  if (opt_.allreduce && opt_.world > 1 && pseudo_cams_ > 0 && !seg_modes) {
    int rc = shard_or_replicate(st->opt);
    if (rc) return rc;
  }
  for (int pass = 0; pass < 2; ++pass) {
    const bool multi = opt_.allreduce != nullptr && opt_.world >= 2;
    border_members_ = env_tail_.empty() ? 0 : border_cams_ + pseudo_cams_;
    const BandStructure band{&st->ocam, &st->opt, C_, P_total_, &st->band_ocam, &st->band_opt, &struct_ocam_, &struct_opt_, struct_P_,
                             &st->env_for_model, &env_tail_, npad_ / 128, pseudo_cams_, border_members_};
    const bool band_chain_bound = band_is_chain_bound(band);
    const bool two_seg_try = multi && pseudo_cams_ > 0 && seg_modes && !distribution_decided_;
    const bool pseudo_border = border_members_ > 0 && (!multi || two_seg_try) && (pseudo_cams_ > 0 || band_chain_bound);
    const int Cband = C_ - (pseudo_border ? border_members_ : 0);
    const bool plan_ok = opt_.dissection != SK_DISSECTION_OFF && opt_.envelope && opt_.lookahead && opt_.cholesky_group == 0 && (env_tail_.empty() || pseudo_border);
    bool may_dissect = plan_ok && (multi ? ((pseudo_cams_ == 0 || two_seg_try) && seg_modes)
                                         : (!opt_.allreduce && chol_ctx_b_.init_secondary(chol_ctx_) == hipSuccess));
    if (!may_dissect) (void)hipGetLastError();
    if (!plan_ok && opt_.distribution_mode == SK_DISTRIBUTION_SEGMENTED) {
      set_error("the segmented distribution needs the library's own factorisation plan (envelope, look-ahead, no explicit group); not supported with these options");
      return SK_ERR_UNSUPPORTED;
    }
    CutPlan cuts;
    if (may_dissect) {
      const bool lockstep_cut = !multi && opt_.dissection == SK_DISSECTION_AUTO && opt_.resident_kernels && cholesky_chain_enabled(&chol_ctx_);
      const CutFlags flags{multi, two_seg_try, lockstep_cut, pseudo_border, opt_.dissection, opt_.distribution_mode, opt_.max_segments, opt_.world, dev_knobs().dissect_at};
      cuts = plan_cuts(band, flags, &cut_model_);
      if (cuts.needs_pair_claim) {
        if (!pair_claimed_) pair_claimed_ = cholesky_claim_pair_servers(&chol_ctx_);
        if (!pair_claimed_ && cuts.drop_without_claim) { cuts.a.clear(); cuts.b.clear(); }
      }
    }
    if (two_seg_try && cuts.a.empty() && opt_.distribution_mode != SK_DISTRIBUTION_SEGMENTED) {
      int rc = shard_or_replicate(st->opt);
      if (rc) return rc;
      continue;
    }
    if (multi && opt_.distribution_mode == SK_DISTRIBUTION_SEGMENTED && cuts.a.empty()) {
      set_error("the segmented distribution needs a separator in the camera sequence (no point seen from both ends); not supported for this problem");
      return SK_ERR_UNSUPPORTED;
    }
    if (!cuts.a.empty()) adopt_cuts(cuts, Cband, multi, st);
    break;
  }
  return SK_OK;
}

void BalSolver::adopt_cuts(const CutPlan& cuts, int Cband, bool multi, Structure* st) {
  dissected_ = true;
  segmented_ = multi;
  const CutNumbering num = apply_cuts(cuts, Cband, C_);
  seg_off_ = num.seg_off; sep_first_ = num.sep_first;
  const std::vector<int>& fin = num.fin;
  segments_ = (int)cuts.a.size() + 1;
  cam_b_ = seg_off_[segments_];
  std::vector<int> cb2(C_);
  for (int c = 0; c < C_; ++c) cb2[fin[c]] = cam_block_[c];
  cam_block_.swap(cb2);
  for (int& c : st->ocam) c = fin[c];
  for (int& c : struct_ocam_) c = fin[c];
  for (int& c : retained_cam_) c = fin[c];
  env_tail_.clear();
  cam_a_ = seg_off_[1];
  if (!segmented_) return;
  distribution_ = SK_DISTRIBUTION_SEGMENTED;
  role_ = opt_.rank % segments_;
  replica_ = opt_.rank >= segments_;
  fold_world_ = segments_;
  my_lo_ = seg_off_[role_]; my_hi_ = seg_off_[role_ + 1];
  std::vector<int> sep_off;
  for (int f : sep_first_) sep_off.push_back(9 * (std::min(f, C_ - border_members_) - cam_b_));
  root_tail_.clear();
  root_last_ = root_envelope(sep_off, 9 * border_members_, &root_tail_);
  pack_rows((9 * (C_ - cam_b_) + 1 + 127) / 128, root_last_, root_tail_, &pack_col0_h_, &pack_off_h_);
  packed_elems_ = (size_t)pack_off_h_.back();
}

int BalSolver::upload_structure(const LocalStructure& ls) {
  const Problem& p = *problem_;
  hipStream_t s = stream_;
  SK_HIP_TRY(b_cam_.upload(ls.cam, s)); SK_HIP_TRY(b_pt_.upload(ls.pt, s)); SK_HIP_TRY(b_obs_.upload(ls.obs, s));
  if (ls.tape) { tape_mode_ = true; SK_HIP_TRY(tape_dev_.upload(*ls.tape, s)); }
  SK_HIP_TRY(b_pt_start_.upload(ls.pt_start, s)); SK_HIP_TRY(b_cam_start_.upload(ls.cam_start, s)); SK_HIP_TRY(b_cam_obs_.upload(ls.cam_obs, s));
  SK_HIP_TRY(b_obs_slot_.upload(ls.slot, s));
  if (!ls.dup_cam.empty()) { SK_HIP_TRY(b_dup_a_.upload(ls.dup_a, s)); SK_HIP_TRY(b_dup_b_.upload(ls.dup_b, s)); SK_HIP_TRY(b_dup_cam_.upload(ls.dup_cam, s)); }
  num_dup_ = (int)ls.dup_cam.size();
  SK_HIP_TRY(b_seg_start_.upload(ls.seg_start, s)); SK_HIP_TRY(b_seg_row_.upload(ls.seg_row, s)); SK_HIP_TRY(b_seg_col_.upload(ls.seg_col, s));
  SK_HIP_TRY(b_pair_row_.upload(ls.pair_row, s)); SK_HIP_TRY(b_pair_col_.upload(ls.pair_col, s));
  SK_HIP_TRY(b_short_segs_.upload(ls.short_segs, s)); SK_HIP_TRY(b_long_segs_.upload(ls.long_segs, s));
  d_.num_short_segments = (int)ls.short_segs.size(); d_.num_long_segments = (int)ls.long_segs.size();
  const size_t nc = 9 * (size_t)C_, np = 3 * (size_t)P_, nx = nc + np;
  std::vector<double> x(nx, 0.0);
  for (int i = 0; i < C_; ++i) if (cam_block_[i] >= 0) std::memcpy(&x[9 * (size_t)i], p.block_ptr[cam_block_[i]], cam_size_ * sizeof(double));
  for (int q = 0; q < P_; ++q) std::memcpy(&x[nc + 3 * (size_t)q], p.block_ptr[pt_block_[local_pt_[q]]], pt_size_ * sizeof(double));
  SK_HIP_TRY(b_xc_.upload(x, s)); SK_HIP_TRY(b_xc_new_.alloc(nx));
  SK_HIP_TRY(b_scale_.alloc(nx)); SK_HIP_TRY(b_colsq_.alloc(nx)); SK_HIP_TRY(b_gs_.alloc(nx)); SK_HIP_TRY(b_step_.alloc(nx));
  {
    std::vector<double> free_mask(nx, 1.0);
    auto mask_block = [&](int block, size_t off, int size, int padded) {
      for (int k = size; k < padded; ++k) free_mask[off + k] = 0.0;
      if ((size_t)block < p.block_constant.size() && p.block_constant[block]) { for (int k = 0; k < size; ++k) free_mask[off + k] = 0.0; return; }
      const int pi = (size_t)block < p.block_param.size() ? p.block_param[block] : -1;
      if (pi < 0) return;
      const LocalParameterization& lp = p.params[pi];
      if (lp.type == kParamSubset) for (int k = 0; k < size; ++k) if ((lp.constant_mask >> k) & 1u) free_mask[off + k] = 0.0;
    };
    for (int i = 0; i < C_; ++i) {
      if (cam_block_[i] >= 0) mask_block(cam_block_[i], 9 * (size_t)i, cam_size_, 9);
      else for (int k = 0; k < 9; ++k) free_mask[9 * (size_t)i + k] = 0.0;
    }
    for (int q = 0; q < P_; ++q) mask_block(pt_block_[local_pt_[q]], nc + 3 * (size_t)q, pt_size_, 3);
    SK_HIP_TRY(hipMemcpyAsync(b_scale_.p, free_mask.data(), nx * sizeof(double), hipMemcpyHostToDevice, s));
    SK_HIP_TRY(hipStreamSynchronize(s));
  }
  SK_HIP_TRY(b_y_.alloc(npad_ + 128));
  SK_HIP_TRY(b_r_.alloc(2 * (size_t)N_)); SK_HIP_TRY(b_F_.alloc(18 * (size_t)N_)); SK_HIP_TRY(b_Fcam_.alloc(kFcam * (size_t)N_)); SK_HIP_TRY(b_E_.alloc(6 * (size_t)N_));
  SK_HIP_TRY(b_W_.alloc(kWs * (size_t)N_)); SK_HIP_TRY(b_rt_.alloc(5 * (size_t)N_));
  if (res_size_ < 2 || cam_size_ < 9 || pt_size_ < 3) {
    SK_HIP_TRY(b_r_.zero(s)); SK_HIP_TRY(b_F_.zero(s)); SK_HIP_TRY(b_E_.zero(s));
  }
  SK_HIP_TRY(b_M_.alloc(6 * (size_t)P_)); SK_HIP_TRY(b_q_.alloc(3 * (size_t)P_));
  if (pseudo_cams_ > 0) {
    std::vector<unsigned char> pseudo(C_, 0);
    for (int i = 0; i < C_; ++i) pseudo[i] = cam_block_[i] < 0 ? 1 : 0;
    SK_HIP_TRY(b_pseudo_.upload(pseudo, s));
    SK_HIP_TRY(b_kept_pt_.upload(ls.kept_pt, s)); SK_HIP_TRY(b_kept_cam_.upload(ls.kept_cam, s));
    if (segmented_) { SK_HIP_TRY(b_kept_home_.upload(ls.kept_home, s)); SK_HIP_TRY(b_kept_global_.upload(ls.kept_global, s)); }
    SK_HIP_TRY(b_kept_obs_.upload(ls.kept_obs, s)); SK_HIP_TRY(b_kept_obs_slot_.upload(ls.kept_obs_slot, s));
    num_kept_obs_ = (int)ls.kept_obs.size();
  }
  return SK_OK;
}

int BalSolver::allocate_fronts(const FrontLayout& lay) {
  hipStream_t s = stream_;
  for (int f = 0; f < 3; ++f) fr_[f] = lay.fr[f];
  border_blocks_ = lay.border_blocks;
  {
    const FrontHost& e = fr_[2];
    SK_HIP_TRY(b_S_.alloc(e.s_off + e.dim * e.dim));
    SK_HIP_TRY(b_Linv_.alloc(e.linv_off + (size_t)e.ncols * 128 * 128)); SK_HIP_TRY(b_Linv_.zero(s));
    const size_t y_end = e.y_off + e.dim;
    SK_HIP_TRY(b_yf_.alloc(y_end)); SK_HIP_TRY(b_yf_.zero(s)); SK_HIP_TRY(b_wf_.alloc(y_end)); SK_HIP_TRY(b_ybB_.alloc((size_t)std::max(1, border_blocks_) * 128));
  }
  if (opt_.allreduce) { SK_HIP_TRY(b_pack_col0_.upload(pack_col0_h_, s)); SK_HIP_TRY(b_pack_off_.upload(pack_off_h_, s)); }
  cholesky_prepare(&chol_ctx_, s);
  if (dissected_ && !segmented_) SK_HIP_TRY(chol_ctx_b_.init_secondary(chol_ctx_));
  SK_HIP_TRY(b_S_.zero(s));
  for (int f = 0; f < 3; ++f) {
    const FrontHost& F = fr_[f];
    if (F.nblk == 0) continue;
    std::vector<int> col0(F.nblk, 0);
    const bool chain_here = chain_ok() && (f != 1 || tail_chain());
    const int widen = F.last.empty() ? 1 : std::max(group_, cholesky_plan_max_group(cholesky_plan(F.nblk, group_, F.last.data(), chain_here, F.ncols, F.tail_rows, F.tl())));
    if (!F.last.empty()) {
      const std::vector<int> first = cholesky_row_first_cols(F.nblk, F.last.data(), F.tl(), F.tail_rows);
      for (int i = 0; i < F.nblk; ++i) col0[i] = std::max(0, first[i] - (widen - 1));
    }
    SK_HIP_TRY(b_zero_col0_f_[f].upload(col0, s));
    std::vector<int> col_min(F.nblk);
    for (int i = 0; i < F.nblk; ++i) col_min[i] = i < F.ncols ? i : F.ncols;
    SK_HIP_TRY(b_zero_min_f_[f].upload(col_min, s));
  }
  for (int f = 0; f < 2; ++f) if (!lay.border_row_h[f].empty()) SK_HIP_TRY(b_border_row_[f].upload(lay.border_row_h[f], s));
  if (segmented_) { SK_HIP_TRY(b_leaf_map_.upload(lay.leaf_map_h, s)); SK_HIP_TRY(b_leaf_gmap_.upload(lay.leaf_gmap_h, s)); }
  if (dissected_ && !segmented_) { SK_HIP_TRY(b_mapB_.upload(lay.mapB, s)); mapB_involution_ = lay.mapB_involution; }
  partial_stride_ = std::max(std::max(std::max(bal_partial_blocks(N_), bal_point_blocks(P_) + 1), (9 * C_ + 255) / 256), 256) + bal_partial_blocks((int)host_obs_.size());
  SK_HIP_TRY(b_partial_.alloc(4 * (size_t)partial_stride_));
  SK_HIP_TRY(b_scal_.alloc(kDevSlots)); SK_HIP_TRY(b_scal_.zero(s)); SK_HIP_TRY(b_small_.alloc(2 * 9 * (size_t)C_ + 6 * retained_pts_.size() + 64 + 16 * (size_t)opt_.world));
  fail_p_ = reinterpret_cast<int*>(b_scal_.p + kFail); info_p_ = reinterpret_cast<int*>(b_scal_.p + kInfo);
  SK_HIP_TRY(hipHostMalloc(reinterpret_cast<void**>(&h_scal_), kHostSlots * sizeof(double), hipHostMallocDefault));
  if (dogleg()) {
    BalDev shape{}; shape.C = C_; shape.P = P_; shape.N = N_;
    const size_t nx = 9 * (size_t)C_ + 3 * (size_t)P_;
    dl_.stride = dogleg_partial_stride(shape);
    SK_HIP_TRY(b_dl_vec_.alloc(2 * nx)); SK_HIP_TRY(b_dl_vec_.zero(s));
    SK_HIP_TRY(b_dl_partial_.alloc(9 * (size_t)dl_.stride)); SK_HIP_TRY(b_dl_partial_.zero(s));
    SK_HIP_TRY(b_dl_scal_.alloc(16)); SK_HIP_TRY(b_dl_scal_.zero(s));
    dl_.s = b_dl_vec_.p; dl_.g = b_dl_vec_.p + nx; dl_.partial = b_dl_partial_.p; dl_.scal = b_dl_scal_.p;
  }
  return SK_OK;
}

int BalSolver::bind_device_view(const LocalStructure& ls) {
  const Problem& p = *problem_;
  hipStream_t s = stream_;
  const size_t nc = 9 * (size_t)C_, nx = nc + 3 * (size_t)P_;
  d_.C = C_; d_.P = P_; d_.N = N_;
  d_.pseudo = pseudo_cams_ > 0 ? b_pseudo_.p : nullptr; d_.num_kept = pseudo_cams_ > 0 ? (int)ls.kept_pt.size() : 0; d_.kept_pt = b_kept_pt_.p; d_.kept_cam = b_kept_cam_.p;
  d_.num_kept_obs = pseudo_cams_ > 0 ? num_kept_obs_ : 0; d_.kept_obs = b_kept_obs_.p; d_.kept_obs_slot = b_kept_obs_slot_.p;
  d_.kept_home = segmented_ && pseudo_cams_ > 0 ? b_kept_home_.p : nullptr; d_.kept_global = segmented_ && pseudo_cams_ > 0 ? b_kept_global_.p : nullptr;
  d_.num_dup = num_dup_; d_.dup_a = b_dup_a_.p; d_.dup_b = b_dup_b_.p; d_.dup_cam = b_dup_cam_.p;
  d_.res_size = res_size_; d_.cam_size = cam_size_; d_.pt_size = pt_size_;
  d_.cam = b_cam_.p; d_.pt = b_pt_.p; d_.obs = b_obs_.p; d_.pt_start = b_pt_start_.p; d_.cam_start = b_cam_start_.p; d_.cam_obs = b_cam_obs_.p; d_.obs_slot = b_obs_slot_.p;
  d_.num_segments = (int)ls.seg_row.size(); d_.seg_start = b_seg_start_.p; d_.seg_row = b_seg_row_.p; d_.seg_col = b_seg_col_.p;
  d_.short_segments = b_short_segs_.p; d_.long_segments = b_long_segs_.p;
  d_.pair_row_obs = b_pair_row_.p; d_.pair_col_obs = b_pair_col_.p;
  d_.xc = b_xc_.p; d_.xp = b_xc_.p + nc; d_.xc_new = b_xc_new_.p; d_.xp_new = b_xc_new_.p + nc;
  d_.scale_c = b_scale_.p; d_.scale_p = b_scale_.p + nc; d_.colsq_c = b_colsq_.p; d_.colsq_p = b_colsq_.p + nc;
  d_.gs_c = b_gs_.p; d_.gs_p = b_gs_.p + nc; d_.step_c = b_step_.p; d_.step_p = b_step_.p + nc;
  d_.y_c = b_y_.p; d_.r = b_r_.p; d_.F = b_F_.p; d_.Fcam = b_Fcam_.p; d_.E = b_E_.p; d_.What = b_W_.p; d_.u = b_rt_.p; d_.M = b_M_.p; d_.q = b_q_.p;
  for (int f = 0; f < 3; ++f) {
    d_.front[f].S = fr_[f].nblk > 0 ? b_S_.p + fr_[f].s_off : nullptr; d_.front[f].ld = (int)fr_[f].dim; d_.front[f].interior = fr_[f].ncols * 128;
    d_.front[f].rhs_row = fr_[f].rhs_row; d_.front[f].border_row = f < 2 ? b_border_row_[f].p : nullptr;
    d_.y_front[f] = b_yf_.p + fr_[f].y_off;
  }
  d_.seg_lo = segmented_ ? my_lo_ : 0; d_.cam_a = segmented_ ? my_hi_ : cam_a_; d_.cam_b = cam_b_;
  d_.S = d_.front[2].S; d_.ld = d_.front[2].ld; d_.rhs_row = fr_[2].rhs_row;
  if (segmented_) {
    const FrontHost& F = fr_[0];
    leaf_.S = d_.front[0].S; leaf_.ld = (long)F.dim; leaf_.nblk = F.nblk; leaf_.ncols = F.ncols; leaf_.last = F.env();
    leaf_.Linv = b_Linv_.p + F.linv_off; leaf_.rhs_row = F.rhs_row; leaf_.tail_rows = F.tail_rows; leaf_.spike = role_ > 0 && role_ + 1 < segments_;
    leaf_.tail = F.tl();
  }
  if (dissected_ && !segmented_) {
    auto view = [&](int f) {
      FrontView v;
      v.S = d_.front[f].S; v.ld = (long)fr_[f].dim; v.nblk = fr_[f].nblk; v.ncols = fr_[f].ncols; v.last = fr_[f].env();
      v.Linv = b_Linv_.p + fr_[f].linv_off; v.rhs_row = fr_[f].rhs_row; v.tail = fr_[f].tl();
      return v;
    };
    ds_.A = view(0); ds_.B = view(1); ds_.R = view(2); ds_.border_blocks = border_blocks_; ds_.mapB = b_mapB_.p; ds_.mapB_involution = mapB_involution_;
  }
  d_.partial = b_partial_.p; d_.partial_stride = partial_stride_; d_.fail_flag = fail_p_;
  d_.loss_nodes = nullptr; d_.loss_root = p.rb_loss.empty() ? -1 : p.rb_loss[0]; d_.loss_of_obs = nullptr;
  {
    bool mixed = false;
    int any_root = -1;
    for (size_t b = 0; b < p.rb_loss.size(); ++b) { mixed = mixed || p.rb_loss[b] != p.rb_loss[0]; any_root = std::max(any_root, p.rb_loss[b]); }
    if (mixed) {
      std::vector<int> roots(N_);
      for (int o = 0; o < N_; ++o) roots[o] = p.rb_loss[ls.order[o]];
      SK_HIP_TRY(b_loss_of_obs_.upload(roots, s));
      d_.loss_of_obs = b_loss_of_obs_.p; d_.loss_root = any_root;
    }
  }
  if (d_.loss_root >= 0) { SK_HIP_TRY(b_loss_nodes_.upload(p.loss_nodes, s)); d_.loss_nodes = b_loss_nodes_.p; }
  d_.is_host = nullptr; d_.num_host = (int)host_obs_.size(); d_.host_obs = nullptr; d_.host_rows = nullptr;
  if (!host_obs_.empty()) {
    std::vector<unsigned char> flag(N_, 0);
    for (int o : host_obs_) flag[o] = 1;
    SK_HIP_TRY(b_is_host_.upload(flag, s)); SK_HIP_TRY(b_host_obs_.upload(host_obs_, s));
    SK_HIP_TRY(b_host_rows_.alloc(host_obs_.size() * (size_t)kHostRow));
    d_.is_host = b_is_host_.p; d_.host_obs = b_host_obs_.p; d_.host_rows = b_host_rows_.p;
    h_cam_ = ls.cam; h_pt_ = ls.pt;
    host_x_.resize(nx); host_rows_h_.resize(host_obs_.size() * (size_t)kHostRow);
  }
  graph_mode_ = graph_mode_ && host_obs_.empty() && !dissected_ && !tape_mode_;
  zero_by_backsolve_ = !graph_mode_ && !dev_knobs().schedule_plain && opt_.resident_kernels;
  for (int f = 0; f < 3; ++f) if (fr_[f].nblk > 0 && !cholesky_backsolve_resident(fr_[f].nblk)) zero_by_backsolve_ = false;
  SK_HIP_TRY(hipStreamSynchronize(s));
  return SK_OK;
}

int BalSolver::upload_bounds() {
  const Problem& p = *problem_;
  hipStream_t s = stream_;
  const size_t nc = 9 * (size_t)C_, nx = nc + 3 * (size_t)P_;
  const double inf = std::numeric_limits<double>::infinity();
  std::vector<double> box(2 * nx);
  std::fill(box.begin(), box.begin() + (long)nx, -inf); std::fill(box.begin() + (long)nx, box.end(), inf);
  auto fill = [&](int block, size_t off, int size) {
    for (int k = 0; k < size; ++k) { box[off + k] = p.lower_bound((size_t)block, k); box[nx + off + k] = p.upper_bound((size_t)block, k); }
  };
  for (int i = 0; i < C_; ++i) if (cam_block_[i] >= 0) fill(cam_block_[i], 9 * (size_t)i, cam_size_);
  for (int q = 0; q < P_; ++q) fill(pt_block_[local_pt_[q]], nc + 3 * (size_t)q, pt_size_);
  SK_HIP_TRY(b_bd_box_.upload(box, s));
  bd_.stride = bounds_partial_stride((int)nx);
  SK_HIP_TRY(b_bd_partial_.alloc(6 * (size_t)bd_.stride)); SK_HIP_TRY(b_bd_partial_.zero(s));
  SK_HIP_TRY(b_bd_scal_.alloc(8)); SK_HIP_TRY(b_bd_scal_.zero(s));
  bd_.lo = b_bd_box_.p; bd_.hi = b_bd_box_.p + nx; bd_.partial = b_bd_partial_.p; bd_.scal = b_bd_scal_.p;
  launch_box_project(d_.xc, bd_.lo, bd_.hi, (int)nx, s);
  SK_HIP_TRY(hipStreamSynchronize(s));
  return SK_OK;
}

int BalSolver::agree_with_ranks() {
  if (!opt_.allreduce) return SK_OK;
  double v[2] = {order_hash_, -order_hash_};
  int rc = gather_rank_scalars_signed(v, 2);
  if (rc) return rc;
  if (v[0] != order_hash_ || v[1] != -order_hash_) {
    set_error("the ranks derived different camera orders for the reduced system (are the residual blocks added in the same order on every rank?)");
    return SK_ERR_COMM;
  }
  double off[1] = {chain_ok() && !chain_live() ? 1.0 : 0.0};
  rc = gather_rank_scalars_signed(off, 1);
  if (rc) return rc;
  if (off[0] > 0.0) cholesky_disable_chain(&chol_ctx_);
  return SK_OK;
}
bool BalSolver::rank_table_on_device(int K) const { return opt_.allreduce != nullptr && opt_.world > 1 && opt_.world * K <= kRankTableSlots; }
int BalSolver::enqueue_rank_table(int mode, int K) {
  double* dev = rank_table_dev();
  launch_bal_pack_rank_scalars(b_scal_.p, dev, opt_.rank, opt_.world, mode, segmented_, stream_);
  int rc = allreduce(dev, (size_t)opt_.world * K);
  if (rc) return rc;
  SK_HIP_TRY(hipMemcpyAsync(h_scal_ + kRankTable, dev, (size_t)opt_.world * K * sizeof(double), hipMemcpyDeviceToHost, stream_));
  return SK_OK;
}
int BalSolver::fold_rank_table(const double* table, double* vals, int K, const int* ops) {
  const int W = opt_.world;
  const int fold = fold_world_ > 0 ? std::min(fold_world_, W) : W;
  for (int k = 0; k < K; ++k) {
    double a = 0.0;
    for (int r = 0; r < fold; ++r) a = ops[k] ? std::max(a, table[(size_t)r * K + k]) : a + table[(size_t)r * K + k];
    vals[k] = a;
  }
  return SK_OK;
}
int BalSolver::exchange_rank_table(const double* vals, int K, std::vector<double>* table) {
  table->assign((size_t)opt_.world * K, 0.0);
  for (int k = 0; k < K; ++k) (*table)[(size_t)opt_.rank * K + k] = vals[k];
  double* dev = rank_table_dev();
  SK_HIP_TRY(hipMemcpyAsync(dev, table->data(), table->size() * sizeof(double), hipMemcpyHostToDevice, stream_));
  int rc = allreduce(dev, table->size());
  if (rc) return rc;
  SK_HIP_TRY(hipMemcpyAsync(table->data(), dev, table->size() * sizeof(double), hipMemcpyDeviceToHost, stream_));
  SK_HIP_TRY(hipStreamSynchronize(stream_));
  return SK_OK;
}
int BalSolver::gather_rank_scalars_signed(double* vals, int K) {
  std::vector<double> table;
  int rc = exchange_rank_table(vals, K, &table);
  if (rc) return rc;
  for (int k = 0; k < K; ++k) {
    double a = table[k];
    for (int r = 1; r < opt_.world; ++r) a = std::max(a, table[(size_t)r * K + k]);
    vals[k] = a;
  }
  return SK_OK;
}
int BalSolver::gather_rank_scalars(double* vals, int K, const int* ops) {
  if (!opt_.allreduce) return SK_OK;
  std::vector<double> table;
  int rc = exchange_rank_table(vals, K, &table);
  return rc ? rc : fold_rank_table(table.data(), vals, K, ops);
}

int BalSolver::evaluate_with_jacobian(bool first) {
  hipStream_t s = stream_;
  const size_t nc = 9 * (size_t)C_, np = 3 * (size_t)P_;
  SK_HIP_TRY(hipEventRecord(ev_[kEvBegin], s));
  const bool graph = graph_ok() && !first;
  const bool replay = graph && g_eval_[parity_] != nullptr;
  if (graph && !replay && hipStreamBeginCapture(s, hipStreamCaptureModeThreadLocal) != hipSuccess) { (void)hipGetLastError(); graph_mode_ = false; return evaluate_with_jacobian(first); }
  CaptureGuard capture(s, graph && !replay, &graph_mode_);
  if (!replay) {
  kt_.begin("bal_eval_jac", s);
  if (tape_mode_) launch_bal_eval_jac_tape(d_, tape_dev_, s); else launch_bal_eval_jac(d_, s);
  kt_.end("bal_eval_jac", s);
  int nb = bal_partial_blocks(N_);
  if (d_.num_host > 0) {
    bool failed = false;
    int rc = host_callbacks(d_.xc, true, &failed);
    if (rc) return rc;
    if (failed) return SK_ERR_EVALUATION_FAILED;
    nb += launch_bal_host_jac(d_, nb, s);
  }
  kt_.begin("bal_cam_records", s); launch_bal_cam_records(d_, s); kt_.end("bal_cam_records", s);
  kt_.begin("bal_reduce", s); launch_bal_reduce(d_, s); kt_.end("bal_reduce", s);
  if (opt_.allreduce) {
    double* buf = b_small_.p;
    const size_t nk = segmented_ && pseudo_cams_ > 0 ? 6 * retained_pts_.size() : 0;
    if (nk) SK_HIP_TRY(hipMemsetAsync(buf + 2 * nc, 0, nk * sizeof(double), s));
    if (replica_) {
      SK_HIP_TRY(hipMemsetAsync(buf, 0, 2 * nc * sizeof(double), s));
    } else {
      SK_HIP_TRY(hipMemcpyAsync(buf, d_.colsq_c, nc * sizeof(double), hipMemcpyDeviceToDevice, s));
      SK_HIP_TRY(hipMemcpyAsync(buf + nc, d_.gs_c, nc * sizeof(double), hipMemcpyDeviceToDevice, s));
      if (nk) launch_bal_kept_sums(d_, buf + 2 * nc, (int)retained_pts_.size(), true, s);
    }
    int rc = allreduce(buf, 2 * nc + nk);
    if (rc) return rc;
    SK_HIP_TRY(hipMemcpyAsync(d_.colsq_c, buf, nc * sizeof(double), hipMemcpyDeviceToDevice, s));
    SK_HIP_TRY(hipMemcpyAsync(d_.gs_c, buf + nc, nc * sizeof(double), hipMemcpyDeviceToDevice, s));
    if (nk) launch_bal_kept_sums(d_, buf + 2 * nc, (int)retained_pts_.size(), false, s);
  }
  if (first && opt_.jacobi_scaling) {
    launch_jacobi_scale(b_colsq_.p, b_scale_.p, (int)(nc + np), s);
    launch_bal_scale_jac(d_, s);
    launch_bal_cam_records(d_, s);
    launch_apply_scale_to_reductions(b_colsq_.p, b_gs_.p, b_scale_.p, (int)(nc + np), s);
  }
  if (!opt_.allreduce) {
    const int g = launch_grad_max_xnorm(b_gs_.p, b_scale_.p, d_.xc, (int)(nc + np), b_partial_.p + (size_t)partial_stride_, partial_stride_, s);
    ReduceRows rows;
    rows.n = 3;
    rows.row[0] = 0; rows.count[0] = nb; rows.out[0] = b_scal_.p + kSumSq;
    rows.row[1] = 1; rows.count[1] = g; rows.is_max[1] = 1; rows.out[1] = b_scal_.p + kGradMaxCam;
    rows.row[2] = 2; rows.count[2] = g; rows.out[2] = b_scal_.p + kXSqCam;
    launch_final_reduce_rows(b_partial_.p, partial_stride_, rows, s);
  } else {
  launch_final_reduce(b_partial_.p, partial_stride_, nb, 1, 0, b_scal_.p + kSumSq, s);
  int c_lo = 0, c_n = (int)nc;
  if (segmented_) { c_lo = 9 * my_lo_; c_n = 9 * (my_hi_ - my_lo_); }
  int gc = launch_grad_max_xnorm(d_.gs_c + c_lo, d_.scale_c + c_lo, d_.xc + c_lo, c_n, b_partial_.p, partial_stride_, s);
  if (segmented_ && role_ == 0) {
    const int lo2 = 9 * cam_b_, n2 = (int)nc - lo2;
    gc += launch_grad_max_xnorm(d_.gs_c + lo2, d_.scale_c + lo2, d_.xc + lo2, n2, b_partial_.p + gc, partial_stride_, s);
  }
  launch_final_reduce(b_partial_.p, partial_stride_, gc, 2, 1, b_scal_.p + kGradMaxCam, s);
  const int np_own = 3 * P_own_;
  const int gp = launch_grad_max_xnorm(d_.gs_p, d_.scale_p, d_.xp, np_own, b_partial_.p + 2 * (size_t)partial_stride_, partial_stride_, s);
  launch_final_reduce(b_partial_.p + 2 * (size_t)partial_stride_, partial_stride_, np_own ? gp : 0, 2, 1, b_scal_.p + kGradMaxPt, s);
  }
  SK_HIP_TRY(hipMemcpyAsync(h_scal_ + kEvalFirst, b_scal_.p + kEvalFirst, (kEvalLast + 1 - kEvalFirst) * sizeof(double), hipMemcpyDeviceToHost, s));
  if (bounded_) {
    kt_.begin("bounded_grad_max_xnorm", s); launch_bounded_grad_max_xnorm(b_gs_.p, b_scale_.p, d_.xc, (int)(nc + np), bd_, s); kt_.end("bounded_grad_max_xnorm", s);
    SK_HIP_TRY(hipMemcpyAsync(h_scal_ + kBounds + kBdGradMax, bd_.scal + kBdGradMax, (kBdActive + 1 - kBdGradMax) * sizeof(double), hipMemcpyDeviceToHost, s));
  }
  }
  if (graph) {
    if (!replay) { capture.release(); int rc = finish_capture(s, &g_eval_[parity_]); if (rc) return rc; if (!graph_mode_) return evaluate_with_jacobian(first); }
    SK_HIP_TRY(hipGraphLaunch(g_eval_[parity_], s));
  }
  SK_HIP_TRY(hipEventRecord(ev_[kEvJac], s));
  const bool dev_gather = rank_table_on_device(3) && !graph;
  if (dev_gather) { int rc = enqueue_rank_table(0, 3); if (rc) return rc; }
  SK_HIP_TRY(hipStreamSynchronize(s));
  const double sumsq = h_scal_[kSumSq];
  const double gmax_c = h_scal_[kGradMaxCam], x2_c = h_scal_[kXSqCam];
  double loc[3] = {sumsq, segmented_ ? std::max(h_scal_[kGradMaxPt], gmax_c) : h_scal_[kGradMaxPt], h_scal_[kXSqPt] + (segmented_ ? x2_c : 0.0)};
  const int ops3[3] = {0, 1, 0};
  int rc = dev_gather ? fold_rank_table(h_scal_ + kRankTable, loc, 3, ops3) : gather_rank_scalars(loc, 3, ops3);
  if (rc) return rc;
  add_phases(0, 0);
  cost_ = 0.5 * loc[0];
  gmax_ = segmented_ ? loc[1] : std::max(gmax_c, loc[1]);
  xnorm_ = std::sqrt((segmented_ ? 0.0 : x2_c) + loc[2]);
  if (bounded_) { gmax_ = h_scal_[kBounds + kBdGradMax]; active_bounds_ = (long)h_scal_[kBounds + kBdActive]; }
  if (!std::isfinite(cost_)) return SK_ERR_EVALUATION_FAILED;
  return SK_OK;
}

int BalSolver::linear_solve(double radius, LinearSolve* out) {
  bool chain_lost = false;
  int rc = solve_once(radius, out, &chain_lost);
  if (rc == SK_OK && chain_lost) rc = solve_once(radius, out, &chain_lost);
  return rc;
}

int BalSolver::solve_once(double radius, LinearSolve* out, bool* chain_lost) {
  hipStream_t s = stream_;
  *chain_lost = false;
  *out = LinearSolve();
  ++n_linear_solves_;
  SK_HIP_TRY(hipEventRecord(ev_[kEvBegin], s));
  const bool graph = graph_ok();
  const bool replay = graph && g_step_[parity_] != nullptr;
  bool candidate_failed = false;
  if (graph) {
    h_scal_[kRadius] = radius;
    if (!replay && hipStreamBeginCapture(s, hipStreamCaptureModeThreadLocal) != hipSuccess) { (void)hipGetLastError(); graph_mode_ = false; return solve_once(radius, out, chain_lost); }
  }
  CaptureGuard capture(s, graph && !replay, &graph_mode_);
  if (!replay) {
    d_.lm_lo = opt_.min_lm_diagonal; d_.lm_hi = opt_.max_lm_diagonal; d_.lm_radius = radius; d_.lm_radius_dev = nullptr;
    if (graph) {
      SK_HIP_TRY(hipMemcpyAsync(b_scal_.p + kRadiusDev, h_scal_ + kRadius, sizeof(double), hipMemcpyHostToDevice, s));
      d_.lm_radius_dev = b_scal_.p + kRadiusDev;
    }
    Backsolve bs;
    bs.resident = opt_.resident_kernels && cholesky_backsolve_resident(npad_ / 128) ? 1 : 0;
    bs.zero_after = zero_by_backsolve_ && bs.resident;
    int rc = enqueue_schur_assembly(bs, graph);
    if (rc == SK_OK) rc = enqueue_factor_backsolve(bs, graph);
    if (rc == SK_OK) rc = enqueue_point_backsub(graph);
    if (rc == SK_OK && !dogleg()) rc = enqueue_candidate_cost(2, &candidate_failed);
    if (rc) return rc;
    if (!graph) SK_HIP_TRY(hipEventRecord(ev_[kEvCost], s));
    SK_HIP_TRY(hipMemcpyAsync(h_scal_ + kStepFirst, b_scal_.p + kStepFirst, (kStepLast + 1 - kStepFirst) * sizeof(double), hipMemcpyDeviceToHost, s));
  }
  const bool dev_gather = rank_table_on_device(4) && !graph;
  if (dev_gather) { int rc = enqueue_rank_table(1, 4); if (rc) return rc; }
  if (graph) {
    if (!replay) { capture.release(); int rc = finish_capture(s, &g_step_[parity_]); if (rc) return rc; if (!graph_mode_) return solve_once(radius, out, chain_lost); }
    SK_HIP_TRY(hipGraphLaunch(g_step_[parity_], s));
    SK_HIP_TRY(hipEventRecord(ev_[kEvCost], s));
  }
  SK_HIP_TRY(hipStreamSynchronize(s));
  if (graph) {
    add_phase(2, ev_[kEvBegin], ev_[kEvCost]);
  } else {
    add_phases(1, 4);
  }
  const int fail = host_flag(kFail), info = host_flag(kInfo);
  if (info != 0) need_full_zero_ = true;
  if (cholesky_note_info(opt_.lookahead ? &chol_ctx_ : nullptr, info) && !opt_.allreduce) {
    if (graph_mode_) {
      for (hipGraphExec_t* g : {&g_step_[0], &g_step_[1], &g_eval_[0], &g_eval_[1]}) if (*g) { (void)hipGraphExecDestroy(*g); *g = nullptr; }
      graph_mode_ = false;
    }
    *chain_lost = true;
    return SK_OK;
  }
  if (dogleg()) {
    out->valid = (fail | info) == 0;
    out->dl = dogleg::Scalars::from(h_scal_ + kDogleg + kDlScalars);
    return SK_OK;
  }
  double loc[4] = {h_scal_[kCandSumSq], h_scal_[kModel], h_scal_[kStepSqPt] + (segmented_ ? h_scal_[kStepSqCam] : 0.0), (double)(fail | info)};
  const int ops4[4] = {0, 0, 0, 1};
  int rc = dev_gather ? fold_rank_table(h_scal_ + kRankTable, loc, 4, ops4) : gather_rank_scalars(loc, 4, ops4);
  if (rc) return rc;
  if (opt_.allreduce && loc[3] >= 2.0) cholesky_disable_chain(&chol_ctx_);
  const double step_sq = (segmented_ ? 0.0 : h_scal_[kStepSqCam]) + loc[2];
  if (loc[3] != 0.0 || !std::isfinite(step_sq) || !std::isfinite(loc[1])) return SK_OK;
  out->valid = true;
  out->model_cost_change = -loc[1];
  out->cost = candidate_failed ? std::numeric_limits<double>::max() : 0.5 * loc[0];
  out->step_norm = std::sqrt(bounded_ ? h_scal_[kBounds + kBdStepSq] : step_sq);
  out->g_delta = h_scal_[kBounds + kBdGDelta]; out->max_delta = h_scal_[kBounds + kBdMaxDelta];
  return SK_OK;
}

int BalSolver::enqueue_schur_assembly(const Backsolve& bs, bool graph) {
  hipStream_t s = stream_;
  kt_.begin("memset_S", s);
  for (int f = 0; f < 3; ++f)
    if (fr_[f].nblk > 0) launch_zero_envelope(d_.front[f].S, (int)fr_[f].dim, (zero_by_backsolve_ && !need_full_zero_) ? b_zero_min_f_[f].p : b_zero_col0_f_[f].p, fr_[f].nblk, s);
  kt_.end("memset_S", s);
  need_full_zero_ = !bs.zero_after;
  SK_HIP_TRY(hipMemsetAsync(b_scal_.p + kFail, 0, (kInfo + 1 - kFail) * sizeof(double), s));
  launch_bal_point_block(d_, s);
  launch_bal_kept_points(d_, s);
  launch_bal_obs_precompute(d_, s);
  kt_.begin("bal_cam_diag", s); launch_bal_cam_diag(d_, s); kt_.end("bal_cam_diag", s);
  kt_.begin("bal_pair", s); launch_bal_pair(d_, s); kt_.end("bal_pair", s);
  if (opt_.allreduce && !segmented_) {
    launch_tri_pack(d_.S, npad_, b_pack_.p, npad_ / 128, b_pack_col0_.p, b_pack_off_.p, true, s);
    int rc = allreduce(b_pack_.p, packed_elems_);
    if (rc) return rc;
    launch_tri_pack(d_.S, npad_, b_pack_.p, npad_ / 128, b_pack_col0_.p, b_pack_off_.p, false, s);
  }
  if (!segmented_) {
    BalFinishRanges r;
    int k = 0;
    for (int f = 0; f < 2; ++f)
      if (fr_[f].nblk > 0 && fr_[f].ncols * 128 > 9 * fr_[f].cams) { r.S[k] = d_.front[f].S; r.ld[k] = (int)fr_[f].dim; r.from[k] = 9 * fr_[f].cams; r.to[k] = fr_[f].ncols * 128; r.value[k] = 1.0; ++k; }
    r.S[k] = d_.front[2].S; r.ld[k] = (int)fr_[2].dim; r.from[k] = fr_[2].rhs_row; r.to[k] = fr_[2].rhs_row + 1; r.value[k] = 1e300; ++k;
    if ((int)fr_[2].dim > fr_[2].rhs_row + 1) { r.S[k] = d_.front[2].S; r.ld[k] = (int)fr_[2].dim; r.from[k] = fr_[2].rhs_row + 1; r.to[k] = (int)fr_[2].dim; r.value[k] = 1.0; ++k; }
    launch_bal_finish_all(d_, r, s);
  } else {
    launch_bal_finish_S(d_, 3, s);
    for (int f = 0; f < 2; ++f)
      if (fr_[f].nblk > 0) launch_set_diagonal(d_.front[f].S, (int)fr_[f].dim, 9 * fr_[f].cams, fr_[f].ncols * 128, 1.0, s);
  }
  if (!graph) SK_HIP_TRY(hipEventRecord(ev_[kEvAssemble], s));
  return SK_OK;
}

int BalSolver::enqueue_factor_backsolve(const Backsolve& bs, bool graph) {
  hipStream_t s = stream_;
  CholeskyContext* ctx = opt_.lookahead ? &chol_ctx_ : nullptr;
  int* bs_info = bs.resident ? info_p_ : nullptr;
  double* yf[3] = {b_yf_.p + fr_[0].y_off, b_yf_.p + fr_[1].y_off, b_yf_.p + fr_[2].y_off};
  double* wf[3] = {b_wf_.p + fr_[0].y_off, b_wf_.p + fr_[1].y_off, b_wf_.p + fr_[2].y_off};
  const bool prefilled = bs.resident != 0;
  if (prefilled) SK_HIP_TRY(hipMemsetAsync(b_yf_.p, 0xff, (fr_[0].dim + fr_[1].dim + fr_[2].dim) * sizeof(double), s));
  if (segmented_) {
    const FrontView& L = leaf_;
    const FrontHost& R = fr_[2];
    double* Rs = d_.front[2].S;
    double* RLinv = b_Linv_.p + R.linv_off;
    if (L.ncols > 0) {
      cholesky_factor(L.S, L.ld, L.nblk * 128, L.Linv, info_p_, group_, s, ctx, &kt_, L.last, chain_ok(), L.ncols, L.tail_rows, nullptr, L.tail);
      cholesky_border_add(Rs, (long)R.dim, L.S, L.ld, L.ncols, L.nblk - L.ncols, b_leaf_map_.p, s);
    }
    if (replica_) SK_HIP_TRY(hipMemsetAsync(b_pack_.p, 0, packed_elems_ * sizeof(double), s));
    else launch_tri_pack(Rs, (int)R.dim, b_pack_.p, R.nblk, b_pack_col0_.p, b_pack_off_.p, true, s);
    int rc = allreduce(b_pack_.p, packed_elems_);
    if (rc) return rc;
    launch_tri_pack(Rs, (int)R.dim, b_pack_.p, R.nblk, b_pack_col0_.p, b_pack_off_.p, false, s);
    launch_bal_finish_S(d_, 4, s);
    launch_set_diagonal(Rs, (int)R.dim, R.rhs_row, R.rhs_row + 1, 1e300, s);
    launch_set_diagonal(Rs, (int)R.dim, R.rhs_row + 1, (int)R.dim, 1.0, s);
    cholesky_factor(Rs, (long)R.dim, (int)R.dim, RLinv, info_p_, group_, s, ctx, &kt_, R.env(), chain_ok(), -1, 1, nullptr, R.tl());
    cholesky_backsolve(Rs, (long)R.dim, 9 * R.cams, (int)R.dim, R.rhs_row, RLinv, wf[2], yf[2], s, &kt_, R.env(), bs_info, R.tl(), bs.zero_after, bs.resident, prefilled);
    if (L.ncols > 0) {
      cholesky_gather_map(yf[2], b_leaf_gmap_.p, b_ybB_.p, (L.nblk - L.ncols) * 128, s);
      cholesky_backsolve_front(L.S, L.ld, L.nblk, L.ncols, L.rhs_row, L.Linv, b_ybB_.p, wf[0], yf[0], s, L.last, L.spike, L.tail_rows, bs_info, bs.zero_after, L.tail, nullptr, bs.resident, prefilled);
    }
  } else if (dissected_) {
    cholesky_dissected_factor(ds_, info_p_, group_, s, ctx, &chol_ctx_b_, &kt_, &kt_b_, chain_ok());
    cholesky_dissected_backsolve(ds_, 9 * fr_[2].cams, wf[2], yf[2], wf[0], yf[0], wf[1], yf[1], b_ybB_.p, s, &chol_ctx_b_, &kt_, bs_info, bs.zero_after, bs.resident, prefilled);
  } else {
    const FrontHost& R = fr_[2];
    cholesky_factor(d_.front[2].S, (long)R.dim, (int)R.dim, b_Linv_.p, info_p_, group_, s, ctx, &kt_, R.env(), chain_ok(), -1, 1, nullptr, R.tl());
    cholesky_backsolve(d_.front[2].S, (long)R.dim, n_, (int)R.dim, R.rhs_row, b_Linv_.p, wf[2], yf[2], s, &kt_, R.env(), bs_info, R.tl(), bs.zero_after, bs.resident, prefilled);
  }
  if (!graph) SK_HIP_TRY(hipEventRecord(ev_[kEvChol], s));
  return SK_OK;
}

int BalSolver::enqueue_point_backsub(bool graph) {
  hipStream_t s = stream_;
  int lo = 0, hi = 9 * C_, lo2 = 0, hi2 = 0;
  if (segmented_) {
    lo = 9 * my_lo_; hi = 9 * my_hi_;
    if (role_ == 0) { lo2 = 9 * cam_b_; hi2 = 9 * C_; }
  }
  launch_bal_backsub(d_, b_scal_.p + kStepSqCam, lo, hi, lo2, hi2, s);
  if (dogleg()) {
    kt_.begin("dogleg_vector_norms", s); launch_dogleg_vector_norms(d_, dl_, s); kt_.end("dogleg_vector_norms", s);
    kt_.begin("bal_dogleg_products", s); launch_bal_dogleg_products(d_, dl_, s); kt_.end("bal_dogleg_products", s);
    launch_dogleg_reduce_scalars(dl_, s);
    SK_HIP_TRY(hipMemcpyAsync(h_scal_ + kDogleg + kDlScalars, dl_.scal + kDlScalars, (kDlStepSq - kDlScalars) * sizeof(double), hipMemcpyDeviceToHost, s));
  }
  if (bounded_) {
    kt_.begin("bal_directional_derivative", s); launch_bal_directional_derivative(d_, bd_, s); kt_.end("bal_directional_derivative", s);
    kt_.begin("bal_bounded_candidate", s); launch_bal_bounded_candidate(d_, bd_, 1.0, s); kt_.end("bal_bounded_candidate", s);
    SK_HIP_TRY(hipMemcpyAsync(h_scal_ + kBounds + kBdStepSq, bd_.scal + kBdStepSq, (kBdMaxDelta + 1 - kBdStepSq) * sizeof(double), hipMemcpyDeviceToHost, s));
  }
  if (!graph) SK_HIP_TRY(hipEventRecord(ev_[kEvBacksub], s));
  return SK_OK;
}

int BalSolver::enqueue_candidate_cost(int rows, bool* failed) {
  hipStream_t s = stream_;
  kt_.begin("bal_eval_cost", s);
  if (tape_mode_) launch_bal_eval_cost_tape(d_, tape_dev_, s); else launch_bal_eval_cost(d_, s);
  kt_.end("bal_eval_cost", s);
  int nb_cost = bal_partial_blocks(N_);
  if (d_.num_host > 0) {
    int rc = host_callbacks(d_.xc_new, false, failed);
    if (rc) return rc;
    nb_cost += launch_bal_host_cost(d_, nb_cost, s);
  }
  launch_final_reduce(b_partial_.p, partial_stride_, nb_cost, rows, 0, b_scal_.p + kCandSumSq, s);
  return SK_OK;
}

int BalSolver::trial_cost(const double* step_sq_dev, int step_sq_slot, double* cost, double* step_norm) {
  hipStream_t s = stream_;
  SK_HIP_TRY(hipEventRecord(ev_[kEvBacksub], s));
  bool failed = false;
  int rc = enqueue_candidate_cost(1, &failed);
  if (rc) return rc;
  SK_HIP_TRY(hipEventRecord(ev_[kEvCost], s));
  SK_HIP_TRY(hipMemcpyAsync(h_scal_ + kCandSumSq, b_scal_.p + kCandSumSq, sizeof(double), hipMemcpyDeviceToHost, s));
  SK_HIP_TRY(hipMemcpyAsync(h_scal_ + step_sq_slot, step_sq_dev, sizeof(double), hipMemcpyDeviceToHost, s));
  SK_HIP_TRY(hipStreamSynchronize(s));
  add_phases(3, 4);
  *cost = failed ? std::numeric_limits<double>::max() : 0.5 * h_scal_[kCandSumSq];
  *step_norm = std::sqrt(h_scal_[step_sq_slot]);
  return SK_OK;
}

int BalSolver::bounded_trial(double alpha, double* cost, double* step_norm) {
  SK_HIP_TRY(hipEventRecord(ev_[kEvBegin], stream_));
  kt_.begin("bal_bounded_candidate", stream_); launch_bal_bounded_candidate(d_, bd_, alpha, stream_); kt_.end("bal_bounded_candidate", stream_);
  return trial_cost(bd_.scal + kBdStepSq, kBounds + kBdStepSq, cost, step_norm);
}

int BalSolver::dogleg_trial(double a, double b, double* cost, double* step_norm) {
  SK_HIP_TRY(hipEventRecord(ev_[kEvBegin], stream_));
  kt_.begin("bal_dogleg_combine", stream_); launch_bal_dogleg_combine(d_, dl_, a, b, stream_); kt_.end("bal_dogleg_combine", stream_);
  return trial_cost(dl_.scal + kDlStepSq, kDogleg + kDlStepSq, cost, step_norm);
}

int BalSolver::finish_capture(hipStream_t s, hipGraphExec_t* exec) {
  hipGraph_t g = nullptr;
  hipError_t e = hipStreamEndCapture(s, &g);
  if (e == hipSuccess && g) e = hipGraphInstantiate(exec, g, nullptr, nullptr, 0);
  if (g) (void)hipGraphDestroy(g);
  if (e != hipSuccess || !*exec) {
    (void)hipGetLastError();
    *exec = nullptr;
    graph_mode_ = false;
    std::fprintf(stderr, "[skeres_amd] hipGraph capture of the iteration failed (%s): launches are enqueued one by one\n", hipGetErrorString(e));
  }
  return SK_OK;
}

int BalSolver::host_callbacks(const double* x_dev, bool jac, bool* failed) {
  *failed = false;
  const size_t nc = 9 * (size_t)C_, np = 3 * (size_t)P_;
  SK_HIP_TRY(hipMemcpyAsync(host_x_.data(), x_dev, (nc + np) * sizeof(double), hipMemcpyDeviceToHost, stream_));
  SK_HIP_TRY(hipStreamSynchronize(stream_));
  for (size_t h = 0; h < host_obs_.size(); ++h) {
    const int o = host_obs_[h];
    const CostFunction* cf = host_cf_[h];
    const double* params[2] = {&host_x_[9 * (size_t)h_cam_[o]], &host_x_[nc + 3 * (size_t)h_pt_[o]]};
    double* row = &host_rows_h_[h * (size_t)kHostRow];
    for (int k = 0; k < kHostRow; ++k) row[k] = 0.0;
    if (res_size_ == 2 && cam_size_ == 9 && pt_size_ == 3) {
      double* jptr[2] = {row + 2, row + 20};
      if (!cf->callback(cf->user, params, row, jac ? jptr : nullptr)) { *failed = true; return SK_OK; }
    } else {
      double res[2] = {0.0, 0.0}, jc[2 * 9], jq[2 * 3];
      double* jptr[2] = {jc, jq};
      if (!cf->callback(cf->user, params, res, jac ? jptr : nullptr)) { *failed = true; return SK_OK; }
      for (int r = 0; r < res_size_; ++r) {
        row[r] = res[r];
        if (jac) {
          for (int k = 0; k < cam_size_; ++k) row[2 + 9 * r + k] = jc[r * cam_size_ + k];
          for (int k = 0; k < pt_size_; ++k) row[20 + 3 * r + k] = jq[r * pt_size_ + k];
        }
      }
    }
  }
  SK_HIP_TRY(hipMemcpyAsync(b_host_rows_.p, host_rows_h_.data(), host_rows_h_.size() * sizeof(double), hipMemcpyHostToDevice, stream_));
  SK_HIP_TRY(hipStreamSynchronize(stream_));
  return SK_OK;
}

int BalSolver::write_back() {
  const size_t nc = 9 * (size_t)C_, np = 3 * (size_t)P_;
  std::vector<double> x(nc + np);
  SK_HIP_TRY(hipMemcpyAsync(x.data(), d_.xc, (nc + np) * sizeof(double), hipMemcpyDeviceToHost, stream_));
  SK_HIP_TRY(hipStreamSynchronize(stream_));
  if (segmented_) {
    std::vector<double> cams(nc, 0.0);
    if (!replica_) {
      const size_t lo = 9 * (size_t)my_lo_, hi = 9 * (size_t)my_hi_;
      std::memcpy(&cams[lo], &x[lo], (hi - lo) * sizeof(double));
      if (role_ == 0) std::memcpy(&cams[9 * (size_t)cam_b_], &x[9 * (size_t)cam_b_], (nc - 9 * (size_t)cam_b_) * sizeof(double));
    }
    DevBuf<double> tmpc;
    SK_HIP_TRY(tmpc.upload(cams, stream_));
    int rc = allreduce(tmpc.p, cams.size());
    if (rc) return rc;
    SK_HIP_TRY(hipMemcpyAsync(x.data(), tmpc.p, nc * sizeof(double), hipMemcpyDeviceToHost, stream_));
    SK_HIP_TRY(hipStreamSynchronize(stream_));
  }
  for (int i = 0; i < C_; ++i) if (cam_block_[i] >= 0) std::memcpy(problem_->block_ptr[cam_block_[i]], &x[9 * (size_t)i], cam_size_ * sizeof(double));
  if (!opt_.allreduce) {
    for (int q = 0; q < P_; ++q) std::memcpy(problem_->block_ptr[pt_block_[local_pt_[q]]], &x[nc + 3 * (size_t)q], pt_size_ * sizeof(double));
    return SK_OK;
  }
  std::vector<double> all(3 * (size_t)P_total_, 0.0);
  if (!replica_)
    for (int q = 0; q < P_own_; ++q) std::memcpy(&all[3 * (size_t)local_pt_[q]], &x[nc + 3 * (size_t)q], 3 * sizeof(double));
  DevBuf<double> tmp;
  SK_HIP_TRY(tmp.upload(all, stream_));
  int rc = allreduce(tmp.p, all.size());
  if (rc) return rc;
  SK_HIP_TRY(hipMemcpyAsync(all.data(), tmp.p, all.size() * sizeof(double), hipMemcpyDeviceToHost, stream_));
  SK_HIP_TRY(hipStreamSynchronize(stream_));
  for (int q = 0; q < P_total_; ++q) std::memcpy(problem_->block_ptr[pt_block_[q]], &all[3 * (size_t)q], pt_size_ * sizeof(double));
  return SK_OK;
}

}

std::unique_ptr<SolverBase> make_bal_solver(const Options& o, Problem* p) { return std::unique_ptr<SolverBase>(new BalSolver(o, p)); }

}
```

### skeres_amd/csrc/chol_kernels.hip

```cpp
#include <hip/hip_runtime.h>
#include <algorithm>
#include <atomic>
#include <chrono>
#include <hip/hip_ext.h>
#include <math.h>
#include <stdlib.h>
#include <string.h>
#include <memory>
#include "chol_kernels.hpp"
#include "device_table.hpp"

namespace sk {

typedef double d4 __attribute__((ext_vector_type(4)));

constexpr int gemm_lds_doubles(int kBKT, int kTM, int kTN) { return 2 * (kTM + kTN) * (kBKT + 2); }
#define SK_GEMM_LDS(kBKT, kTM, kTN) __shared__ __attribute__((aligned(16))) double sh[gemm_lds_doubles(kBKT, kTM, kTN)];
template <int kMode, int kShape, int kBKT, int kPF, int kTM, int kTN>
__device__ __forceinline__ void gemm_nt_f64_body(double* shp, double* C, long ldc, const double* A, long lda, const double* B, long ldb, int K,
                                                 int tiles_m, int skip, int main_t = 0x7fffffff, int jump_t = 0, int main_n = 0x7fffffff,
                                                 int jump_n = 0, int block_id = -1, int* first_column_done = nullptr, int count_cols = 1,
                                                 int* diag_done = nullptr) {
  constexpr int mode = kMode;
  constexpr int kLdT = kBKT + 2;
// ... 2175 lines not shown
void cholesky_backsolve(double* S, long ld, int n, int npad, int rhs_row, const double* Linv, double* w, double* y,
                        hipStream_t s, KernelTimer* kt, const int* last, int* info, const int* tail, bool zero_after, int resident, bool prefilled) {
  const int nblk = npad / 128;
  if (info && (resident < 0 ? g_bs_resident.load() != 0 : resident != 0) && nblk <= kBsMaxBlocks) {
    BsTop env;
    for (int c = 0; c < nblk; ++c) {
      env.top[c] = (unsigned short)(last ? std::min(std::max(last[c], c), nblk - 1) : nblk - 1);
      env.tail[c] = (unsigned short)(tail ? std::min(std::max(tail[c], 0), nblk - 1) : nblk - 1);
    }
    if (kt) kt->begin("backsolve", s);
    if (!prefilled) (void)hipMemsetAsync(y, 0xff, sizeof(double) * (size_t)npad, s);
    const char* bs_stamps = dev_knobs().bs_stamps;
    if (bs_stamps) { static bool on = false; if (!on) { const int one = 1; (void)hipMemcpyToSymbol(HIP_SYMBOL(g_bs_stamps_on), &one, sizeof(int)); on = true; } }
    const bool spread = zero_after && dev_knobs().bs_spread != 0;
    const int janitors = zero_after ? bs_janitors(nblk) : 0;
#ifdef SK_TESTING
    if (janitors > 0) { int want = 1; if (g_test_janitor_giveup.compare_exchange_strong(want, 0)) { const int one = 1; (void)hipMemcpyToSymbolAsync(HIP_SYMBOL(g_bs_test_janitor_giveup), &one, sizeof(int), 0, hipMemcpyHostToDevice, s); (void)hipStreamSynchronize(s); } }
#endif
    hipLaunchKernelGGL(bs_resident_kernel, dim3(spread ? 8 * nblk : nblk + janitors), dim3(1024), 0, s, Linv, S, ld, (const double*)(S + (long)rhs_row * ld), n, y, nblk, env, info, nblk,
                       (const double*)nullptr, spread ? -1 : janitors, (const int*)nullptr);
    if (kt) kt->end("backsolve", s);
    if (bs_stamps) {
      (void)hipStreamSynchronize(s);
      std::vector<long long> st((size_t)1024 * 4);
      (void)hipMemcpyFromSymbol(st.data(), HIP_SYMBOL(g_bs_stamps), st.size() * sizeof(long long));
      if (FILE* f = fopen(bs_stamps, "w")) {
        for (int kb = nblk - 1; kb >= 0; --kb) fprintf(f, "%d %lld %lld %lld\n", kb, st[(size_t)kb * 4], st[(size_t)kb * 4 + 1], st[(size_t)kb * 4 + 2]);
        fclose(f);
      }
    }
    return;
  }
  hipLaunchKernelGGL(copy_row_kernel, dim3((npad + 255) / 256), dim3(256), 0, s, S + (long)rhs_row * ld, w, n, npad);
  if (kt) kt->begin("backsolve", s);
  const std::vector<int> first = cholesky_row_first_cols(nblk, last, tail);
  for (int kb = nblk - 1; kb >= 0; --kb) {
    const int ncols = kb * 128, col0 = first[kb] * 128;
    const int grid = ncols > col0 ? (ncols - col0 + 63) / 64 : 1;
    hipLaunchKernelGGL(bs_step_kernel, dim3(grid), dim3(1024), 0, s, Linv + (long)kb * 128 * 128, S + (long)kb * 128 * ld, ld, w, y, kb, col0, ncols);
  }
  if (kt) kt->end("backsolve", s);
}

__global__ __launch_bounds__(256) void border_add_kernel(double* __restrict__ root, long ld_r, const double* __restrict__ border, long ld_f, int m,
                                                         const int* __restrict__ map) {
  const long e = (long)blockIdx.x * 256 + threadIdx.x;
  if (e >= (long)m * m) return;
  const int i = (int)(e / m), j = (int)(e % m);
  if (j > i) return;
  int ri = i, rj = j;
  if (map) { ri = map[i]; rj = map[j]; }
  if (ri < 0 || rj < 0) return;
  const double v = border[(long)i * ld_f + j];
  if (v == 0.0) return;
  if (ri >= rj) root[(long)ri * ld_r + rj] += v;
  else root[(long)rj * ld_r + ri] += v;
}

__global__ __launch_bounds__(1024) void bs_border_kernel(const double* __restrict__ Lb, long ld, int m, const double* __restrict__ yb, double* __restrict__ w,
                                                          int col0, int ncols) {
  __shared__ double red[16 * 64];
  const int t = threadIdx.x, cl = t & 63, rg = t >> 6;
  const int col = col0 + blockIdx.x * 64 + cl;
  double acc = 0.0;
  if (col < ncols)
    for (int r = rg; r < m; r += 16) acc += Lb[(long)r * ld + col] * yb[r];
  red[rg * 64 + cl] = acc;
  __syncthreads();
  if (t < 64 && col < ncols) {
    double u = 0.0;
#pragma unroll
    for (int g = 0; g < 16; ++g) u += red[g * 64 + t];
    w[col] -= u;
  }
}

__global__ void gather_map_kernel(const double* __restrict__ src, const int* __restrict__ map, double* __restrict__ dst, int m) {
  const int i = blockIdx.x * blockDim.x + threadIdx.x;
  if (i < m) dst[i] = map ? (map[i] >= 0 ? src[map[i]] : 0.0) : src[i];
}

__global__ __launch_bounds__(256) void border_add2_kernel(double* __restrict__ root, long ld_r, const double* __restrict__ a, long ld_a, const double* __restrict__ b, long ld_b,
                                                          int m, const int* __restrict__ map) {
  const long e = (long)blockIdx.x * 256 + threadIdx.x;
  if (e >= (long)m * m) return;
  const int i = (int)(e / m), j = (int)(e % m);
  if (j > i) return;
  double v = root[(long)i * ld_r + j];
  bool touched = false;
  const double va = a[(long)i * ld_a + j];
  if (va != 0.0) { v += va; touched = true; }
  const int bi = map[i], bj = map[j];
  if (bi >= 0 && bj >= 0) {
    const double vb = bi >= bj ? b[(long)bi * ld_b + bj] : b[(long)bj * ld_b + bi];
    if (vb != 0.0) { v += vb; touched = true; }
  }
  if (touched) root[(long)i * ld_r + j] = v;
}
void cholesky_border_add(double* root, long ld_r, const double* front, long ld_f, int ncols, int border_blocks, const int* map, hipStream_t s) {
  const int m = border_blocks * 128;
  const long total = (long)m * m;
  hipLaunchKernelGGL(border_add_kernel, dim3((unsigned)((total + 255) / 256)), dim3(256), 0, s, root, ld_r, front + (long)ncols * 128 * ld_f + (long)ncols * 128, ld_f, m, map);
}

void cholesky_backsolve_front(double* S, long ld, int nblk, int ncols, int rhs_row, const double* Linv, const double* yb, double* w, double* y,
                              hipStream_t s, const int* last, bool spike, int tail_rows, int* info, bool zero_after, const int* tail, const int* yb_map, int resident,
                              bool prefilled) {
  const int ni = ncols * 128, m = (nblk - ncols) * 128;
  if (ncols <= 0) return;
  const bool res = info && (resident < 0 ? g_bs_resident.load() != 0 : resident != 0) && nblk <= kBsMaxBlocks;
  if (yb_map && !res) {
    std::fprintf(stderr, "[skeres_amd] internal: cholesky_backsolve_front got a border map without the resident launch\n");
    if (info) (void)hipMemsetAsync(info, 0x7f, sizeof(int), s);
    return;
  }
  if (res) {
    if (tail_rows < 1 || tail_rows > nblk - ncols) tail_rows = 1;
    BsTop env;
    for (int c = 0; c < nblk; ++c) {
      env.top[c] = (unsigned short)(last ? std::min(std::max(last[c], c), nblk - 1) : nblk - 1);
      env.tail[c] = (unsigned short)(tail ? std::min(std::max(tail[c], 0), nblk - 1) : nblk - tail_rows);
    }
    if (!prefilled) (void)hipMemsetAsync(y, 0xff, sizeof(double) * (size_t)ni, s);
    const bool spread = zero_after && dev_knobs().bs_spread != 0;
    const int janitors = zero_after ? bs_janitors(ncols) : 0;
    hipLaunchKernelGGL(bs_resident_kernel, dim3(spread ? 8 * ncols : ncols + janitors), dim3(1024), 0, s, Linv, S, ld, (const double*)(S + (long)rhs_row * ld), ni, y, nblk, env, info, ncols, yb,
                       spread ? -1 : janitors, yb_map);
    return;
  }
  hipLaunchKernelGGL(copy_row_kernel, dim3((ni + 255) / 256), dim3(256), 0, s, S + (long)rhs_row * ld, w, ni, ni);
  std::vector<int> first(nblk, 0);
  int c0 = 0;
  if (last)
    for (int kb = 0; kb < nblk - 1; ++kb) {
      while (c0 < kb && last[c0] < kb) ++c0;
      first[kb] = c0;
    }
  const int bfirst = first[ncols < nblk - 1 ? ncols : nblk - 1];
  const int bcol0 = (spike || tail) ? 0 : std::min(bfirst, ncols) * 128;
  if (ni > bcol0)
    hipLaunchKernelGGL(bs_border_kernel, dim3((ni - bcol0 + 63) / 64), dim3(1024), 0, s, S + (long)ncols * 128 * ld, ld, m, yb, w, bcol0, ni);
  for (int kb = ncols - 1; kb >= 0; --kb) {
    const int nc = kb * 128, col0 = first[kb] * 128;
    const int grid = nc > col0 ? (nc - col0 + 63) / 64 : 1;
    hipLaunchKernelGGL(bs_step_kernel, dim3(grid), dim3(1024), 0, s, Linv + (long)kb * 128 * 128, S + (long)kb * 128 * ld, ld, w, y, kb, col0, nc);
  }
}

static void fork_join_events(CholeskyContext* c) {
  if (!c->fork_ev) (void)hipEventCreateWithFlags(&c->fork_ev, g_event_flags);
  if (!c->join_ev) (void)hipEventCreateWithFlags(&c->join_ev, g_event_flags);
}

void cholesky_dissected_factor(const DissectedSystem& d, int* info, int group, hipStream_t s, CholeskyContext* ctxA, CholeskyContext* ctxB,
                               KernelTimer* kt, KernelTimer* ktB, bool allow_chain) {
  if (d.A.ncols > 0 && d.B.ncols > 0 && ctxA && ctxB && allow_chain) {
    CholeskyPartner pt{d.B.S, d.B.ld, d.B.nblk, d.B.ncols, 1, d.B.last, d.B.Linv, ctxB, d.B.tail};
    cholesky_factor(d.A.S, d.A.ld, d.A.nblk * 128, d.A.Linv, info, group, s, ctxA, kt, d.A.last, allow_chain, d.A.ncols, 1, &pt, d.A.tail);
    if (!pt.taken)
      cholesky_factor(d.B.S, d.B.ld, d.B.nblk * 128, d.B.Linv, info, group, s, ctxA, kt, d.B.last, allow_chain, d.B.ncols, 1, nullptr, d.B.tail);
    cholesky_border_add(d.R.S, d.R.ld, d.A.S, d.A.ld, d.A.ncols, d.border_blocks, nullptr, s);
    cholesky_border_add(d.R.S, d.R.ld, d.B.S, d.B.ld, d.B.ncols, d.border_blocks, d.mapB, s);
    cholesky_factor(d.R.S, d.R.ld, d.R.nblk * 128, d.R.Linv, info, group, s, ctxA, kt, d.R.last, allow_chain);
    return;
  }
  const bool side = d.B.ncols > 0 && ctxB && ctxB->fork;
  if (d.B.ncols > 0 && !side) {
    cholesky_factor(d.B.S, d.B.ld, d.B.nblk * 128, d.B.Linv, info, group, s, ctxA, kt, d.B.last, allow_chain && ctxB && ctxB->server, d.B.ncols, 1, nullptr, d.B.tail);
  } else if (side) {
    fork_join_events(ctxB);
    hipStream_t sB = ctxB->fork;
    (void)hipEventRecord(ctxB->fork_ev, s);
    (void)hipStreamWaitEvent(sB, ctxB->fork_ev, 0);
    const bool chainB = allow_chain && ctxB->server != nullptr;
    if (!ctxB->runner) ctxB->runner.reset(new AsyncRunner(ctxB->device));
    ctxB->runner->run([&d, info, group, ctxB, ktB, sB, chainB] {
      cholesky_factor(d.B.S, d.B.ld, d.B.nblk * 128, d.B.Linv, info, group, sB, ctxB, ktB, d.B.last, chainB, d.B.ncols, 1, nullptr, d.B.tail);
      (void)hipEventRecord(ctxB->join_ev, sB);
    });
  }
  if (d.A.ncols > 0) cholesky_factor(d.A.S, d.A.ld, d.A.nblk * 128, d.A.Linv, info, group, s, ctxA, kt, d.A.last, allow_chain, d.A.ncols, 1, nullptr, d.A.tail);
  if (side) {
    ctxB->runner->wait();
    (void)hipStreamWaitEvent(s, ctxB->join_ev, 0);
  }
  if (d.A.ncols > 0 && d.B.ncols > 0 && d.mapB && d.mapB_involution) {
    const int m = d.border_blocks * 128;
    hipLaunchKernelGGL(border_add2_kernel, dim3((unsigned)(((long)m * m + 255) / 256)), dim3(256), 0, s, d.R.S, d.R.ld,
                       (const double*)(d.A.S + (long)d.A.ncols * 128 * d.A.ld + (long)d.A.ncols * 128), d.A.ld,
                       (const double*)(d.B.S + (long)d.B.ncols * 128 * d.B.ld + (long)d.B.ncols * 128), d.B.ld, m, d.mapB);
  } else {
    if (d.A.ncols > 0) cholesky_border_add(d.R.S, d.R.ld, d.A.S, d.A.ld, d.A.ncols, d.border_blocks, nullptr, s);
    if (d.B.ncols > 0) cholesky_border_add(d.R.S, d.R.ld, d.B.S, d.B.ld, d.B.ncols, d.border_blocks, d.mapB, s);
  }
  cholesky_factor(d.R.S, d.R.ld, d.R.nblk * 128, d.R.Linv, info, group, s, ctxA, kt, d.R.last, allow_chain);
}

void cholesky_dissected_backsolve(const DissectedSystem& d, int n_root, double* wR, double* yR, double* wA, double* yA, double* wB, double* yB, double* ybB,
                                  hipStream_t s, CholeskyContext* ctxB, KernelTimer* kt, int* info, bool zero_after, int resident, bool prefilled) {
  if (resident < 0) resident = g_bs_resident.load() != 0 ? 1 : 0;
  cholesky_backsolve(d.R.S, d.R.ld, n_root, d.R.nblk * 128, d.R.rhs_row, d.R.Linv, wR, yR, s, nullptr, d.R.last, info, nullptr, zero_after, resident, prefilled);
  if (kt) kt->begin("backsolve", s);
  const int m = d.border_blocks * 128;
  const bool paired = dev_knobs().bs_pair != 0 && d.A.ncols > 0 && d.B.ncols > 0 && info && resident != 0 && d.A.nblk <= kBsPairMaxBlocks && d.B.nblk <= kBsPairMaxBlocks;
  const bool side = !paired && d.B.ncols > 0 && d.A.ncols > 0 && ctxB && ctxB->fork;
  hipStream_t sB = s;
  if (paired) {
    BsPair p;
    const bool spread = zero_after && dev_knobs().bs_spread != 0;
    const FrontView* fv[2] = {&d.A, &d.B};
    double* ys[2] = {yA, yB};
    int grid = 0, jan = 0;
    for (int f = 0; f < 2; ++f) {
      const FrontView& F = *fv[f];
      for (int c = 0; c < F.nblk; ++c) {
        p.env[f].top[c] = (unsigned short)(F.last ? std::min(std::max(F.last[c], c), F.nblk - 1) : F.nblk - 1);
        p.env[f].tail[c] = (unsigned short)(F.tail ? std::min(std::max(F.tail[c], 0), F.nblk - 1) : F.nblk - 1);
      }
      const int janitors = spread ? 3 * F.ncols : (zero_after ? bs_janitors(F.ncols) : 0);
      p.f[f] = BsArgs{F.Linv, F.S, F.ld, (const double*)(F.S + (long)F.rhs_row * F.ld), F.ncols * 128, ys[f], F.nblk, info, F.ncols, yR, janitors, f == 1 ? d.mapB : nullptr,
                      spread ? 3 : 0, spread ? 1 : 0};
      grid += F.ncols; jan += janitors;
    }
    if (spread) { grid = 8 * std::max(d.A.ncols, d.B.ncols); jan = 0; }
    const size_t nA = (size_t)d.A.ncols * 128, nB = (size_t)d.B.ncols * 128;
    if (prefilled) {}
    else if (yB >= yA + nA && (size_t)(yB - yA) <= nA + 4096) (void)hipMemsetAsync(yA, 0xff, sizeof(double) * ((size_t)(yB - yA) + nB), s);
    else { (void)hipMemsetAsync(yA, 0xff, sizeof(double) * nA, s); (void)hipMemsetAsync(yB, 0xff, sizeof(double) * nB, s); }
    hipLaunchKernelGGL(bs_resident_pair_kernel, dim3(grid + jan), dim3(1024), 0, s, p);
  } else {
  if (d.B.ncols > 0) {
    if (side) {
      fork_join_events(ctxB);
      (void)hipEventRecord(ctxB->fork_ev, s);
      (void)hipStreamWaitEvent(ctxB->fork, ctxB->fork_ev, 0);
      sB = ctxB->fork;
    }
    const bool mapped = info && resident != 0 && d.B.nblk <= kBsMaxBlocks;
    if (!mapped) cholesky_gather_map(yR, d.mapB, ybB, m, sB);
    cholesky_backsolve_front(d.B.S, d.B.ld, d.B.nblk, d.B.ncols, d.B.rhs_row, d.B.Linv, mapped ? yR : ybB, wB, yB, sB, d.B.last, false, 1, info, zero_after, d.B.tail,
                             mapped ? d.mapB : nullptr, resident, prefilled);
  }
  }
  if (!paired && d.A.ncols > 0) cholesky_backsolve_front(d.A.S, d.A.ld, d.A.nblk, d.A.ncols, d.A.rhs_row, d.A.Linv, yR, wA, yA, s, d.A.last, false, 1, info, zero_after, d.A.tail, nullptr, resident, prefilled);
  if (side) {
    (void)hipEventRecord(ctxB->join_ev, ctxB->fork);
    (void)hipStreamWaitEvent(s, ctxB->join_ev, 0);
  }
  if (kt) kt->end("backsolve", s);
}

void cholesky_gather_map(const double* src, const int* map, double* dst, int m, hipStream_t s) {
  hipLaunchKernelGGL(gather_map_kernel, dim3((m + 255) / 256), dim3(256), 0, s, src, map, dst, m);
}

void launch_syrk_gram(double* H, long ldh, const double* A, long lda, int Kc, int nslabs, double* slabs, int tiles, hipStream_t s,
                      KernelTimer* kt) {
  if (tiles <= 0) return;
  const size_t slab_stride = (size_t)tiles * 128 * ldh;
  if (kt) kt->begin("syrk_gram", s);
  hipLaunchKernelGGL(syrk_gram_f64_kernel, dim3(tiles * (tiles + 1) / 2, nslabs), dim3(256), 0, s, nslabs > 1 ? slabs : H, ldh, slab_stride, A, lda, Kc);
  if (kt) kt->end("syrk_gram", s);
  if (nslabs > 1) hipLaunchKernelGGL(gram_reduce_kernel, dim3(tiles * (tiles + 1) / 2), dim3(256), 0, s, H, slabs, slab_stride, ldh, nslabs);
}

double cholesky_syrk_flops(int npad, int group, const int* last, bool chain, double* c_tiles, int ncols, int tail_rows, const int* tail) {
  const int nblk = npad / 128;
  const BlockEnvelope env(nblk, last, tail, ncols, tail_rows);
  ncols = env.ncols;
  const CholeskyPlan plan = cholesky_plan(nblk, group, last, chain, ncols, env.tail_rows, tail);
  const std::vector<int>& gb = plan.bounds;
  double f = 0.0, tiles = 0.0;
  for (size_t g = 0; g + 2 < gb.size(); ++g) {
    if (gb[g] >= ncols) break;
    const int k0 = gb[g], k1 = gb[g + 1];
    const int na = (plan.paired[k0] == 1 && k1 - k0 == 2) ? 0 : (plan.resident[k0] ? 1 : gb[g + 2] - k1);
    const int Tb = env.active_rows(k1 - 1, k1 + na);
    f += 0.5 * Tb * (Tb + 1.0) * 2.0 * 128.0 * 128.0 * (double)((k1 - k0) * 128);
    tiles += 0.5 * Tb * (Tb + 1.0);
  }
  if (c_tiles) *c_tiles = tiles;
  return f;
}

}
```

Measured before the change: 257.2.

## Merge point reductions, zero/reset memsets and backsub launches into fewer kernels

Computes the per-point 3x3 normal-matrix sums inside the existing reduce kernel and stores them in a new tsum buffer, so the later point-block kernel only does the small Cholesky solve. The flag memset and the resident y 0xff prefill are folded into one zero-envelope kernel, and point backsub plus the kept-point step run in a single launch. The chained dissected factor path now uses the single-launch border add. This cuts kernel launches and rereads of E per LM iteration, at the cost of extra buffers, a kept-point mask and recomputing point sums after Jacobi scaling.

```diff
diff --git a/skeres_amd/csrc/bal_kernels.hip b/skeres_amd/csrc/bal_kernels.hip
--- a/skeres_amd/csrc/bal_kernels.hip
+++ b/skeres_amd/csrc/bal_kernels.hip
@@ -394,32 +394,52 @@
   }
 }
 
+template <bool kColumns, bool kSums>
 __device__ __forceinline__ void bal_pt_reduce_body(const BalDev& d, int block) {
   const int gid = block * kBlock + threadIdx.x, sub = gid % kPointLanes;
   const int p = gid / kPointLanes;
   if (p >= d.P) return;
   double sq[3] = {0, 0, 0}, g[3] = {0, 0, 0};
+  double t00 = 0, t10 = 0, t11 = 0, t20 = 0, t21 = 0, t22 = 0;
   for (int o = d.pt_start[p] + sub; o < d.pt_start[p + 1]; o += kPointLanes) {
-    const double r0 = d.r[o], r1 = d.r[(size_t)d.N + o];
-#pragma unroll
-    for (int k = 0; k < 3; ++k) {
-      const double e0 = d.E[(size_t)k * d.N + o], e1 = d.E[(size_t)(3 + k) * d.N + o];
-      sq[k] += e0 * e0 + e1 * e1;
-      g[k] += e0 * r0 + e1 * r1;
-    }
-  }
-#pragma unroll
-  for (int k = 0; k < 3; ++k) { sq[k] = point_lanes_sum(sq[k]); g[k] = point_lanes_sum(g[k]); }
-  if (sub == 0) {
-#pragma unroll
-    for (int k = 0; k < 3; ++k) { d.colsq_p[3 * (size_t)p + k] = sq[k]; d.gs_p[3 * (size_t)p + k] = g[k]; }
-  }
-}
-
+    if (kColumns) {
+      const double r0 = d.r[o], r1 = d.r[(size_t)d.N + o];
+#pragma unroll
+      for (int k = 0; k < 3; ++k) {
+        const double e0 = d.E[(size_t)k * d.N + o], e1 = d.E[(size_t)(3 + k) * d.N + o];
+        sq[k] += e0 * e0 + e1 * e1;
+        g[k] += e0 * r0 + e1 * r1;
+      }
+    }
+    if (kSums) {
+      const double a0 = d.E[o], a1 = d.E[(size_t)d.N + o], a2 = d.E[2 * (size_t)d.N + o];
+      const double b0 = d.E[3 * (size_t)d.N + o], b1 = d.E[4 * (size_t)d.N + o], b2 = d.E[5 * (size_t)d.N + o];
+      t00 += a0 * a0 + b0 * b0; t10 += a1 * a0 + b1 * b0; t11 += a1 * a1 + b1 * b1;
+      t20 += a2 * a0 + b2 * b0; t21 += a2 * a1 + b2 * b1; t22 += a2 * a2 + b2 * b2;
+    }
+  }
+  if (kColumns) {
+#pragma unroll
+    for (int k = 0; k < 3; ++k) { sq[k] = point_lanes_sum(sq[k]); g[k] = point_lanes_sum(g[k]); }
+    if (sub == 0) {
+#pragma unroll
+      for (int k = 0; k < 3; ++k) { d.colsq_p[3 * (size_t)p + k] = sq[k]; d.gs_p[3 * (size_t)p + k] = g[k]; }
+    }
+  }
+  if (kSums) {
+    t00 = point_lanes_sum(t00); t10 = point_lanes_sum(t10); t11 = point_lanes_sum(t11);
+    t20 = point_lanes_sum(t20); t21 = point_lanes_sum(t21); t22 = point_lanes_sum(t22);
+    const double v = sub == 0 ? t00 : (sub == 1 ? t10 : (sub == 2 ? t11 : (sub == 3 ? t20 : (sub == 4 ? t21 : t22))));
+    if (sub < 6) d.tsum[(size_t)sub * d.P + p] = v;
+  }
+}
+
+template <bool kSums>
 __global__ __launch_bounds__(kBlock) void bal_reduce_kernel(BalDev d, int cam_blocks) {
   if ((int)blockIdx.x < cam_blocks) bal_cam_reduce_body(d, (int)blockIdx.x);
-  else bal_pt_reduce_body(d, (int)blockIdx.x - cam_blocks);
-}
+  else bal_pt_reduce_body<true, kSums>(d, (int)blockIdx.x - cam_blocks);
+}
+__global__ __launch_bounds__(kBlock) void bal_point_sums_kernel(BalDev d) { bal_pt_reduce_body<false, true>(d, (int)blockIdx.x); }
 
 __global__ void jacobi_scale_kernel(const double* colsq, double* scale, int n) {
   const int j = blockIdx.x * blockDim.x + threadIdx.x;
@@ -470,20 +490,7 @@
   if (threadIdx.x == 0) out[k] = sh[0];
 }
 
-__global__ __launch_bounds__(kBlock) void bal_point_block_kernel(BalDev d) {
-  const int gid = blockIdx.x * kBlock + threadIdx.x, sub = gid % kPointLanes;
-  const int p = gid / kPointLanes;
-  if (p >= d.P) return;
-  double t00 = 0, t10 = 0, t11 = 0, t20 = 0, t21 = 0, t22 = 0;
-  for (int o = d.pt_start[p] + sub; o < d.pt_start[p + 1]; o += kPointLanes) {
-    const double a0 = d.E[o], a1 = d.E[(size_t)d.N + o], a2 = d.E[2 * (size_t)d.N + o];
-    const double b0 = d.E[3 * (size_t)d.N + o], b1 = d.E[4 * (size_t)d.N + o], b2 = d.E[5 * (size_t)d.N + o];
-    t00 += a0 * a0 + b0 * b0; t10 += a1 * a0 + b1 * b0; t11 += a1 * a1 + b1 * b1;
-    t20 += a2 * a0 + b2 * b0; t21 += a2 * a1 + b2 * b1; t22 += a2 * a2 + b2 * b2;
-  }
-  t00 = point_lanes_sum(t00); t10 = point_lanes_sum(t10); t11 = point_lanes_sum(t11);
-  t20 = point_lanes_sum(t20); t21 = point_lanes_sum(t21); t22 = point_lanes_sum(t22);
-  if (sub != 0) return;
+__device__ __forceinline__ void bal_point_solve(const BalDev& d, int p, double t00, double t10, double t11, double t20, double t21, double t22) {
   const double d0 = bal_lm_diag(d, d.colsq_p[3 * (size_t)p]), d1 = bal_lm_diag(d, d.colsq_p[3 * (size_t)p + 1]), d2 = bal_lm_diag(d, d.colsq_p[3 * (size_t)p + 2]);
   t00 += d0 * d0; t11 += d1 * d1; t22 += d2 * d2;
   const double l00 = sqrt(t00);
@@ -504,6 +511,22 @@
   d.q[2 * P + p] = m22 * u2;
   if (!(l00 > 0.0) || !(l11 > 0.0) || !(l22 > 0.0)) *d.fail_flag = 1;
 }
+__global__ __launch_bounds__(kBlock) void bal_point_block_kernel(BalDev d) {
+  const int gid = blockIdx.x * kBlock + threadIdx.x, sub = gid % kPointLanes;
+  const int p = gid / kPointLanes;
+  if (p >= d.P) return;
+  double t00 = 0, t10 = 0, t11 = 0, t20 = 0, t21 = 0, t22 = 0;
+  for (int o = d.pt_start[p] + sub; o < d.pt_start[p + 1]; o += kPointLanes) {
+    const double a0 = d.E[o], a1 = d.E[(size_t)d.N + o], a2 = d.E[2 * (size_t)d.N + o];
+    const double b0 = d.E[3 * (size_t)d.N + o], b1 = d.E[4 * (size_t)d.N + o], b2 = d.E[5 * (size_t)d.N + o];
+    t00 += a0 * a0 + b0 * b0; t10 += a1 * a0 + b1 * b0; t11 += a1 * a1 + b1 * b1;
+    t20 += a2 * a0 + b2 * b0; t21 += a2 * a1 + b2 * b1; t22 += a2 * a2 + b2 * b2;
+  }
+  t00 = point_lanes_sum(t00); t10 = point_lanes_sum(t10); t11 = point_lanes_sum(t11);
+  t20 = point_lanes_sum(t20); t21 = point_lanes_sum(t21); t22 = point_lanes_sum(t22);
+  if (sub != 0) return;
+  bal_point_solve(d, p, t00, t10, t11, t20, t21, t22);
+}
 
 __global__ __launch_bounds__(kBlock) void bal_kept_points_kernel(BalDev d, int obs_blocks) {
   const size_t N = d.N, P = d.P;
@@ -556,6 +579,13 @@
   blk[2 * (size_t)ld] = t20; blk[2 * (size_t)ld + 1] = t21; blk[2 * (size_t)ld + 2] = t22 + d2 * d2;
   double* rhs = bal_rhs(d, ic) + t3;
   rhs[0] = home ? d.gs_p[3 * (size_t)p] : 0.0; rhs[1] = home ? d.gs_p[3 * (size_t)p + 1] : 0.0; rhs[2] = home ? d.gs_p[3 * (size_t)p + 2] : 0.0;
+}
+
+__global__ __launch_bounds__(kBlock) void bal_points_kernel(BalDev d) {
+  const int p = blockIdx.x * kBlock + threadIdx.x;
+  if (p >= d.P) return;
+  const size_t P = d.P;
+  bal_point_solve(d, p, d.tsum[p], d.tsum[P + p], d.tsum[2 * P + p], d.tsum[3 * P + p], d.tsum[4 * P + p], d.tsum[5 * P + p]);
 }
 
 __global__ __launch_bounds__(kBlock) void bal_kept_sums_kernel(BalDev d, double* buf, int K, int gather) {
@@ -816,7 +846,8 @@
   }
 }
 
-__global__ __launch_bounds__(kBlock) void bal_point_backsub_kernel(BalDev d) {
+template <bool kSkipKept>
+__device__ __forceinline__ void bal_point_backsub_body(const BalDev& d) {
   const int gid = blockIdx.x * kBlock + threadIdx.x, sub = gid % kPointLanes;
   const int p = gid / kPointLanes;
   double acc[1] = {0.0};
@@ -829,7 +860,7 @@
     }
   }
   w0 = point_lanes_sum(w0); w1 = point_lanes_sum(w1); w2 = point_lanes_sum(w2);
-  if (p < d.P && sub == 0) {
+  if (p < d.P && sub == 0 && !(kSkipKept && d.pt_kept && d.pt_kept[p])) {
     const size_t P = d.P;
     const double t0 = d.gs_p[3 * (size_t)p] - w0, t1 = d.gs_p[3 * (size_t)p + 1] - w1, t2 = d.gs_p[3 * (size_t)p + 2] - w2;
     const double m00 = d.M[p], m10 = d.M[P + p], m11 = d.M[2 * P + p], m20 = d.M[3 * P + p], m21 = d.M[4 * P + p], m22 = d.M[5 * P + p];
@@ -849,8 +880,9 @@
   }
   block_sum<1>(acc, d.partial + d.partial_stride, d.partial_stride);
 }
-
-__global__ __launch_bounds__(kBlock) void bal_kept_step_kernel(BalDev d, int slot) {
+__global__ __launch_bounds__(kBlock) void bal_point_backsub_kernel(BalDev d) { bal_point_backsub_body<false>(d); }
+
+__device__ __forceinline__ void bal_kept_step_body(const BalDev& d, int slot) {
   double acc[1] = {0.0};
   for (int k = threadIdx.x; k < d.num_kept; k += kBlock) {
     const int p = d.kept_pt[k], ic = d.kept_cam[k] / 3, t3 = 3 * (d.kept_cam[k] % 3);
@@ -867,6 +899,10 @@
     }
   }
   block_sum<1>(acc, d.partial + d.partial_stride + slot, d.partial_stride);
+}
+__global__ __launch_bounds__(kBlock) void bal_kept_step_kernel(BalDev d, int slot) { bal_kept_step_body(d, slot); }
+__global__ __launch_bounds__(kBlock) void bal_point_step_kernel(BalDev d, int pt_blocks) {
+  if ((int)blockIdx.x < pt_blocks) bal_point_backsub_body<true>(d); else bal_kept_step_body(d, 0);
 }
 
 __global__ __launch_bounds__(kBlock) void bal_cam_step_kernel(BalDev d, int norm_lo, int norm_hi, int norm_lo2, int norm_hi2) {
@@ -925,8 +961,7 @@
   return g < 1 ? 1 : (g > cap ? cap : g);
 }
 
-__global__ __launch_bounds__(256) void zero_envelope_kernel(double* S, int ld, const int* col0) {
-  const int kb = blockIdx.y;
+__device__ __forceinline__ void zero_envelope_row(double* S, int ld, const int* col0, int kb) {
   const size_t c0 = (size_t)col0[kb] * 128, width = (size_t)(kb + 1) * 128 - c0;
   const size_t n2 = 128 * width / 2;
   for (size_t i = (size_t)blockIdx.x * 256 + threadIdx.x; i < n2; i += (size_t)gridDim.x * 256) {
@@ -934,8 +969,24 @@
     *reinterpret_cast<double2*>(S + ((size_t)kb * 128 + r) * ld + c0 + c) = make_double2(0.0, 0.0);
   }
 }
+__global__ __launch_bounds__(256) void zero_envelope_kernel(double* S, int ld, const int* col0) { zero_envelope_row(S, ld, col0, (int)blockIdx.y); }
 void launch_zero_envelope(double* S, int ld, const int* col0, int nblk, hipStream_t s) {
   if (nblk > 0) hipLaunchKernelGGL(zero_envelope_kernel, dim3(32, nblk), dim3(256), 0, s, S, ld, col0);
+}
+__global__ __launch_bounds__(256) void zero_reset_kernel(ZeroReset a) {
+  int kb = blockIdx.y;
+#pragma unroll
+  for (int f = 0; f < 3; ++f) {
+    if (kb < a.nblk[f]) { zero_envelope_row(a.S[f], a.ld[f], a.col0[f], kb); return; }
+    kb -= a.nblk[f];
+  }
+  const size_t t = (size_t)blockIdx.x * 256 + threadIdx.x;
+  if (t < (size_t)a.num_flags) a.flags[t] = 0.0;
+  unsigned long long* y = reinterpret_cast<unsigned long long*>(a.y);
+  for (size_t i = t; i < a.ny; i += (size_t)gridDim.x * 256) y[i] = ~0ull;
+}
+void launch_zero_reset(const ZeroReset& a, hipStream_t s) {
+  hipLaunchKernelGGL(zero_reset_kernel, dim3(32, a.nblk[0] + a.nblk[1] + a.nblk[2] + 1), dim3(256), 0, s, a);
 }
 
 int bal_partial_blocks(int N) { return grid_for(N); }
@@ -987,11 +1038,13 @@
 }
 void launch_bal_scale_jac(const BalDev& d, hipStream_t s) { hipLaunchKernelGGL(bal_scale_jac_kernel, dim3(grid_for(d.N)), dim3(kBlock), 0, s, d); }
 void launch_bal_cam_records(const BalDev& d, hipStream_t s) { hipLaunchKernelGGL(bal_cam_records_kernel, dim3(grid_for((d.N + 63) / 64 * 64)), dim3(kBlock), 0, s, d); }
-void launch_bal_reduce(const BalDev& d, hipStream_t s) {
+void launch_bal_reduce(const BalDev& d, bool point_sums, hipStream_t s) {
   const int cam_blocks = (d.C * 64 + kBlock - 1) / kBlock, pt_blocks = d.P > 0 ? (int)(((long)d.P * kPointLanes + kBlock - 1) / kBlock) : 0;
-  hipLaunchKernelGGL(bal_reduce_kernel, dim3(cam_blocks + pt_blocks), dim3(kBlock), 0, s, d, cam_blocks);
+  if (point_sums) hipLaunchKernelGGL(bal_reduce_kernel<true>, dim3(cam_blocks + pt_blocks), dim3(kBlock), 0, s, d, cam_blocks);
+  else hipLaunchKernelGGL(bal_reduce_kernel<false>, dim3(cam_blocks + pt_blocks), dim3(kBlock), 0, s, d, cam_blocks);
 }
 static int point_grid(int P) { return (int)(((long)P * kPointLanes + kBlock - 1) / kBlock); }
+void launch_bal_point_sums(const BalDev& d, hipStream_t s) { if (d.P > 0) hipLaunchKernelGGL(bal_point_sums_kernel, dim3(point_grid(d.P)), dim3(kBlock), 0, s, d); }
 int bal_point_blocks(int P) { return P > 0 ? point_grid(P) : 1; }
 void launch_jacobi_scale(const double* colsq, double* scale, int n, hipStream_t s) { if (n > 0) hipLaunchKernelGGL(jacobi_scale_kernel, dim3((n + 255) / 256), dim3(256), 0, s, colsq, scale, n); }
 void launch_apply_scale_to_reductions(double* colsq, double* gs, const double* scale, int n, hipStream_t s) { if (n > 0) hipLaunchKernelGGL(apply_scale_to_reductions_kernel, dim3((n + 255) / 256), dim3(256), 0, s, colsq, gs, scale, n); }
@@ -1028,6 +1081,7 @@
   const int obs_blocks = (d.num_kept_obs + kBlock - 1) / kBlock;
   hipLaunchKernelGGL(bal_kept_points_kernel, dim3(obs_blocks + (d.num_kept * 64 + kBlock - 1) / kBlock), dim3(kBlock), 0, s, d, obs_blocks);
 }
+void launch_bal_points(const BalDev& d, hipStream_t s) { if (d.P > 0) hipLaunchKernelGGL(bal_points_kernel, dim3((d.P + kBlock - 1) / kBlock), dim3(kBlock), 0, s, d); }
 void launch_bal_obs_precompute(const BalDev& d, hipStream_t s) { hipLaunchKernelGGL(bal_obs_precompute_kernel, dim3(grid_for(d.N)), dim3(kBlock), 0, s, d); }
 void launch_bal_kept_sums(const BalDev& d, double* buf, int K, bool gather, hipStream_t s) {
   if (d.num_kept > 0) hipLaunchKernelGGL(bal_kept_sums_kernel, dim3((3 * d.num_kept + kBlock - 1) / kBlock), dim3(kBlock), 0, s, d, buf, K, gather ? 1 : 0);
@@ -1072,12 +1126,16 @@
 void launch_set_diagonal(double* S, int ld, int from, int to, double value, hipStream_t s) {
   if (to > from) hipLaunchKernelGGL(set_diagonal_kernel, dim3((to - from + 255) / 256), dim3(256), 0, s, S, ld, from, to, value);
 }
-void launch_bal_backsub(const BalDev& d, double* out, int norm_lo, int norm_hi, int norm_lo2, int norm_hi2, hipStream_t s) {
+void launch_bal_backsub(const BalDev& d, double* out, int norm_lo, int norm_hi, int norm_lo2, int norm_hi2, bool one_point_launch, hipStream_t s) {
   const int gc = (9 * d.C + kBlock - 1) / kBlock, gp = bal_point_blocks(d.P);
   hipLaunchKernelGGL(bal_cam_step_kernel, dim3(gc), dim3(kBlock), 0, s, d, norm_lo, norm_hi, norm_lo2, norm_hi2);
   hipLaunchKernelGGL(bal_obs_backsub_kernel, dim3(grid_for(d.N)), dim3(kBlock), 0, s, d);
-  hipLaunchKernelGGL(bal_point_backsub_kernel, dim3(gp), dim3(kBlock), 0, s, d);
-  if (d.num_kept > 0) hipLaunchKernelGGL(bal_kept_step_kernel, dim3(1), dim3(kBlock), 0, s, d, gp);
+  if (one_point_launch && d.num_kept > 0) {
+    hipLaunchKernelGGL(bal_point_step_kernel, dim3(gp + 1), dim3(kBlock), 0, s, d, gp);
+  } else {
+    hipLaunchKernelGGL(bal_point_backsub_kernel, dim3(gp), dim3(kBlock), 0, s, d);
+    if (d.num_kept > 0) hipLaunchKernelGGL(bal_kept_step_kernel, dim3(1), dim3(kBlock), 0, s, d, gp);
+  }
   ReduceRows rows;
   rows.n = 2;
   rows.row[0] = 0; rows.count[0] = gc; rows.out[0] = out;
diff --git a/skeres_amd/csrc/bal_kernels.hpp b/skeres_amd/csrc/bal_kernels.hpp
--- a/skeres_amd/csrc/bal_kernels.hpp
+++ b/skeres_amd/csrc/bal_kernels.hpp
@@ -44,6 +44,7 @@
   double* r;  double* F;  double* E;  double* What;  double* u;
   double* Fcam;  const int* obs_slot;
   double* M;  double* q;
+  double* tsum;  const unsigned char* pt_kept;
   struct Front { double* S; int ld; int interior; int rhs_row; const int* border_row; };
   Front front[3];
   int seg_lo, cam_a, cam_b;
@@ -63,6 +64,9 @@
 int bal_partial_blocks(int N);
 int bal_point_blocks(int P);
 void launch_zero_envelope(double* S, int ld, const int* col0, int nblk, hipStream_t s);
+struct ZeroReset { double* S[3] = {nullptr, nullptr, nullptr}; int ld[3] = {0, 0, 0}; const int* col0[3] = {nullptr, nullptr, nullptr}; int nblk[3] = {0, 0, 0};
+                   double* flags = nullptr; int num_flags = 0; double* y = nullptr; size_t ny = 0; };
+void launch_zero_reset(const ZeroReset& a, hipStream_t s);
 size_t tri_packed_elems(int nblk);
 void launch_tri_pack(double* S, int ld, double* packed, int nblk, const int* col0, const long long* off, bool to_packed, hipStream_t s);
 void launch_bal_eval_jac(const BalDev& d, hipStream_t s);
@@ -73,7 +77,8 @@
 int launch_bal_host_cost(const BalDev& d, int partial_off, hipStream_t s);
 void launch_bal_scale_jac(const BalDev& d, hipStream_t s);
 void launch_bal_cam_records(const BalDev& d, hipStream_t s);
-void launch_bal_reduce(const BalDev& d, hipStream_t s);
+void launch_bal_reduce(const BalDev& d, bool point_sums, hipStream_t s);
+void launch_bal_point_sums(const BalDev& d, hipStream_t s);
 void launch_jacobi_scale(const double* colsq, double* scale, int n, hipStream_t s);
 void launch_apply_scale_to_reductions(double* colsq, double* gs, const double* scale, int n, hipStream_t s);
 void launch_lm_diagonal(const double* colsq, double* D, int n, double lo, double hi, double radius, hipStream_t s);
@@ -84,6 +89,7 @@
 void launch_final_reduce_rows(const double* partial, int stride, const ReduceRows& rows, hipStream_t s);
 void launch_bal_point_block(const BalDev& d, hipStream_t s);
 void launch_bal_kept_points(const BalDev& d, hipStream_t s);
+void launch_bal_points(const BalDev& d, hipStream_t s);
 void launch_bal_kept_sums(const BalDev& d, double* buf, int K, bool gather, hipStream_t s);
 void launch_bal_obs_precompute(const BalDev& d, hipStream_t s);
 void launch_bal_cam_diag(const BalDev& d, hipStream_t s);
@@ -93,7 +99,7 @@
 struct BalFinishRanges { double* S[4] = {nullptr, nullptr, nullptr, nullptr}; int ld[4] = {0, 0, 0, 0}, from[4] = {0, 0, 0, 0}, to[4] = {0, 0, 0, 0}; double value[4] = {0, 0, 0, 0}; };
 void launch_bal_finish_all(const BalDev& d, const BalFinishRanges& r, hipStream_t s);
 void launch_set_diagonal(double* S, int ld, int from, int to, double value, hipStream_t s);
-void launch_bal_backsub(const BalDev& d, double* out, int norm_lo, int norm_hi, int norm_lo2, int norm_hi2, hipStream_t s);
+void launch_bal_backsub(const BalDev& d, double* out, int norm_lo, int norm_hi, int norm_lo2, int norm_hi2, bool one_point_launch, hipStream_t s);
 
 struct DoglegDev { double* s; double* g; double* partial; int stride; double* scal; };
 int dogleg_partial_stride(const BalDev& d);
diff --git a/skeres_amd/csrc/bal_solver.hip b/skeres_amd/csrc/bal_solver.hip
--- a/skeres_amd/csrc/bal_solver.hip
+++ b/skeres_amd/csrc/bal_solver.hip
@@ -195,6 +195,9 @@
   std::vector<int> struct_ocam_, struct_opt_;
   int struct_P_ = 0;
   DevBuf<int> b_kept_pt_, b_kept_cam_, b_kept_obs_, b_kept_obs_slot_;
+  DevBuf<double> b_tsum_;
+  DevBuf<unsigned char> b_pt_kept_;
+  bool merged_launches_ = true;
   int P_own_ = 0;
   DevBuf<int> b_kept_home_, b_kept_global_;
   DevBuf<int> b_dup_a_, b_dup_b_, b_dup_cam_;
@@ -626,7 +629,12 @@
     SK_HIP_TRY(b_r_.zero(s)); SK_HIP_TRY(b_F_.zero(s)); SK_HIP_TRY(b_E_.zero(s));
   }
   SK_HIP_TRY(b_M_.alloc(6 * (size_t)P_)); SK_HIP_TRY(b_q_.alloc(3 * (size_t)P_));
+  merged_launches_ = dev_knobs().schedule_plain == 0;
+  if (merged_launches_) SK_HIP_TRY(b_tsum_.alloc(6 * (size_t)P_));
   if (pseudo_cams_ > 0) {
+    std::vector<unsigned char> kept(P_, 0);
+    for (int q : ls.kept_pt) kept[q] = 1;
+    SK_HIP_TRY(b_pt_kept_.upload(kept, s));
     std::vector<unsigned char> pseudo(C_, 0);
     for (int i = 0; i < C_; ++i) pseudo[i] = cam_block_[i] < 0 ? 1 : 0;
     SK_HIP_TRY(b_pseudo_.upload(pseudo, s));
@@ -706,6 +714,7 @@
   d_.scale_c = b_scale_.p; d_.scale_p = b_scale_.p + nc; d_.colsq_c = b_colsq_.p; d_.colsq_p = b_colsq_.p + nc;
   d_.gs_c = b_gs_.p; d_.gs_p = b_gs_.p + nc; d_.step_c = b_step_.p; d_.step_p = b_step_.p + nc;
   d_.y_c = b_y_.p; d_.r = b_r_.p; d_.F = b_F_.p; d_.Fcam = b_Fcam_.p; d_.E = b_E_.p; d_.What = b_W_.p; d_.u = b_rt_.p; d_.M = b_M_.p; d_.q = b_q_.p;
+  d_.tsum = b_tsum_.p; d_.pt_kept = d_.num_kept > 0 ? b_pt_kept_.p : nullptr;
   for (int f = 0; f < 3; ++f) {
     d_.front[f].S = fr_[f].nblk > 0 ? b_S_.p + fr_[f].s_off : nullptr; d_.front[f].ld = (int)fr_[f].dim; d_.front[f].interior = fr_[f].ncols * 128;
     d_.front[f].rhs_row = fr_[f].rhs_row; d_.front[f].border_row = f < 2 ? b_border_row_[f].p : nullptr;
@@ -865,7 +874,7 @@
     nb += launch_bal_host_jac(d_, nb, s);
   }
   kt_.begin("bal_cam_records", s); launch_bal_cam_records(d_, s); kt_.end("bal_cam_records", s);
-  kt_.begin("bal_reduce", s); launch_bal_reduce(d_, s); kt_.end("bal_reduce", s);
+  kt_.begin("bal_reduce", s); launch_bal_reduce(d_, merged_launches_, s); kt_.end("bal_reduce", s);
   if (opt_.allreduce) {
     double* buf = b_small_.p;
     const size_t nk = segmented_ && pseudo_cams_ > 0 ? 6 * retained_pts_.size() : 0;
@@ -887,6 +896,7 @@
     launch_jacobi_scale(b_colsq_.p, b_scale_.p, (int)(nc + np), s);
     launch_bal_scale_jac(d_, s);
     launch_bal_cam_records(d_, s);
+    if (merged_launches_) launch_bal_point_sums(d_, s);
     launch_apply_scale_to_reductions(b_colsq_.p, b_gs_.p, b_scale_.p, (int)(nc + np), s);
   }
   if (!opt_.allreduce) {
@@ -1024,12 +1034,28 @@
 int BalSolver::enqueue_schur_assembly(const Backsolve& bs, bool graph) {
   hipStream_t s = stream_;
   kt_.begin("memset_S", s);
-  for (int f = 0; f < 3; ++f)
-    if (fr_[f].nblk > 0) launch_zero_envelope(d_.front[f].S, (int)fr_[f].dim, (zero_by_backsolve_ && !need_full_zero_) ? b_zero_min_f_[f].p : b_zero_col0_f_[f].p, fr_[f].nblk, s);
+  if (merged_launches_) {
+    ZeroReset z;
+    for (int f = 0; f < 3; ++f) {
+      if (fr_[f].nblk <= 0) continue;
+      z.S[f] = d_.front[f].S; z.ld[f] = (int)fr_[f].dim; z.nblk[f] = fr_[f].nblk;
+      z.col0[f] = (zero_by_backsolve_ && !need_full_zero_) ? b_zero_min_f_[f].p : b_zero_col0_f_[f].p;
+    }
+    z.flags = b_scal_.p + kFail; z.num_flags = kInfo + 1 - kFail;
+    if (bs.resident) { z.y = b_yf_.p; z.ny = fr_[0].dim + fr_[1].dim + fr_[2].dim; }
+    launch_zero_reset(z, s);
+  } else {
+    for (int f = 0; f < 3; ++f)
+      if (fr_[f].nblk > 0) launch_zero_envelope(d_.front[f].S, (int)fr_[f].dim, (zero_by_backsolve_ && !need_full_zero_) ? b_zero_min_f_[f].p : b_zero_col0_f_[f].p, fr_[f].nblk, s);
+  }
   kt_.end("memset_S", s);
   need_full_zero_ = !bs.zero_after;
-  SK_HIP_TRY(hipMemsetAsync(b_scal_.p + kFail, 0, (kInfo + 1 - kFail) * sizeof(double), s));
-  launch_bal_point_block(d_, s);
+  if (merged_launches_) {
+    launch_bal_points(d_, s);
+  } else {
+    SK_HIP_TRY(hipMemsetAsync(b_scal_.p + kFail, 0, (kInfo + 1 - kFail) * sizeof(double), s));
+    launch_bal_point_block(d_, s);
+  }
   launch_bal_kept_points(d_, s);
   launch_bal_obs_precompute(d_, s);
   kt_.begin("bal_cam_diag", s); launch_bal_cam_diag(d_, s); kt_.end("bal_cam_diag", s);
@@ -1064,7 +1090,7 @@
   double* yf[3] = {b_yf_.p + fr_[0].y_off, b_yf_.p + fr_[1].y_off, b_yf_.p + fr_[2].y_off};
   double* wf[3] = {b_wf_.p + fr_[0].y_off, b_wf_.p + fr_[1].y_off, b_wf_.p + fr_[2].y_off};
   const bool prefilled = bs.resident != 0;
-  if (prefilled) SK_HIP_TRY(hipMemsetAsync(b_yf_.p, 0xff, (fr_[0].dim + fr_[1].dim + fr_[2].dim) * sizeof(double), s));
+  if (prefilled && !merged_launches_) SK_HIP_TRY(hipMemsetAsync(b_yf_.p, 0xff, (fr_[0].dim + fr_[1].dim + fr_[2].dim) * sizeof(double), s));
   if (segmented_) {
     const FrontView& L = leaf_;
     const FrontHost& R = fr_[2];
@@ -1107,7 +1133,7 @@
     lo = 9 * my_lo_; hi = 9 * my_hi_;
     if (role_ == 0) { lo2 = 9 * cam_b_; hi2 = 9 * C_; }
   }
-  launch_bal_backsub(d_, b_scal_.p + kStepSqCam, lo, hi, lo2, hi2, s);
+  launch_bal_backsub(d_, b_scal_.p + kStepSqCam, lo, hi, lo2, hi2, merged_launches_, s);
   if (dogleg()) {
     kt_.begin("dogleg_vector_norms", s); launch_dogleg_vector_norms(d_, dl_, s); kt_.end("dogleg_vector_norms", s);
     kt_.begin("bal_dogleg_products", s); launch_bal_dogleg_products(d_, dl_, s); kt_.end("bal_dogleg_products", s);
diff --git a/skeres_amd/csrc/chol_kernels.hip b/skeres_amd/csrc/chol_kernels.hip
--- a/skeres_amd/csrc/chol_kernels.hip
+++ b/skeres_amd/csrc/chol_kernels.hip
@@ -2351,6 +2351,18 @@
   if (!c->join_ev) (void)hipEventCreateWithFlags(&c->join_ev, g_event_flags);
 }
 
+static void cholesky_dissected_border_add(const DissectedSystem& d, bool one_launch, hipStream_t s) {
+  if (one_launch && d.A.ncols > 0 && d.B.ncols > 0 && d.mapB && d.mapB_involution) {
+    const int m = d.border_blocks * 128;
+    hipLaunchKernelGGL(border_add2_kernel, dim3((unsigned)(((long)m * m + 255) / 256)), dim3(256), 0, s, d.R.S, d.R.ld,
+                       (const double*)(d.A.S + (long)d.A.ncols * 128 * d.A.ld + (long)d.A.ncols * 128), d.A.ld,
+                       (const double*)(d.B.S + (long)d.B.ncols * 128 * d.B.ld + (long)d.B.ncols * 128), d.B.ld, m, d.mapB);
+  } else {
+    if (d.A.ncols > 0) cholesky_border_add(d.R.S, d.R.ld, d.A.S, d.A.ld, d.A.ncols, d.border_blocks, nullptr, s);
+    if (d.B.ncols > 0) cholesky_border_add(d.R.S, d.R.ld, d.B.S, d.B.ld, d.B.ncols, d.border_blocks, d.mapB, s);
+  }
+}
+
 void cholesky_dissected_factor(const DissectedSystem& d, int* info, int group, hipStream_t s, CholeskyContext* ctxA, CholeskyContext* ctxB,
                                KernelTimer* kt, KernelTimer* ktB, bool allow_chain) {
   if (d.A.ncols > 0 && d.B.ncols > 0 && ctxA && ctxB && allow_chain) {
@@ -2358,8 +2370,7 @@
     cholesky_factor(d.A.S, d.A.ld, d.A.nblk * 128, d.A.Linv, info, group, s, ctxA, kt, d.A.last, allow_chain, d.A.ncols, 1, &pt, d.A.tail);
     if (!pt.taken)
       cholesky_factor(d.B.S, d.B.ld, d.B.nblk * 128, d.B.Linv, info, group, s, ctxA, kt, d.B.last, allow_chain, d.B.ncols, 1, nullptr, d.B.tail);
-    cholesky_border_add(d.R.S, d.R.ld, d.A.S, d.A.ld, d.A.ncols, d.border_blocks, nullptr, s);
-    cholesky_border_add(d.R.S, d.R.ld, d.B.S, d.B.ld, d.B.ncols, d.border_blocks, d.mapB, s);
+    cholesky_dissected_border_add(d, dev_knobs().schedule_plain == 0, s);
     cholesky_factor(d.R.S, d.R.ld, d.R.nblk * 128, d.R.Linv, info, group, s, ctxA, kt, d.R.last, allow_chain);
     return;
   }
@@ -2383,15 +2394,7 @@
     ctxB->runner->wait();
     (void)hipStreamWaitEvent(s, ctxB->join_ev, 0);
   }
-  if (d.A.ncols > 0 && d.B.ncols > 0 && d.mapB && d.mapB_involution) {
-    const int m = d.border_blocks * 128;
-    hipLaunchKernelGGL(border_add2_kernel, dim3((unsigned)(((long)m * m + 255) / 256)), dim3(256), 0, s, d.R.S, d.R.ld,
-                       (const double*)(d.A.S + (long)d.A.ncols * 128 * d.A.ld + (long)d.A.ncols * 128), d.A.ld,
-                       (const double*)(d.B.S + (long)d.B.ncols * 128 * d.B.ld + (long)d.B.ncols * 128), d.B.ld, m, d.mapB);
-  } else {
-    if (d.A.ncols > 0) cholesky_border_add(d.R.S, d.R.ld, d.A.S, d.A.ld, d.A.ncols, d.border_blocks, nullptr, s);
-    if (d.B.ncols > 0) cholesky_border_add(d.R.S, d.R.ld, d.B.S, d.B.ld, d.B.ncols, d.border_blocks, d.mapB, s);
-  }
+  cholesky_dissected_border_add(d, true, s);
   cholesky_factor(d.R.S, d.R.ld, d.R.nblk * 128, d.R.Linv, info, group, s, ctxA, kt, d.R.last, allow_chain);
 }
 
```

After: 260.0 (median of 6 runs). +1.1%, better.
